# tbuckworth/train-procgen-pytorch

Hardware: AMD Instinct MI355X
Metric: env steps/sec (whole node), coinrun hard-500 IMPALA-CNN PPO (higher is better)
Workload: dtype bf16

## Files before the change

### scratch/ro_timeline4.py

```python
import csv, glob, sys, collections
f = glob.glob(sys.argv[1] + "/**/*kernel_trace.csv", recursive=True)[0]
rows = list(csv.DictReader(open(f)))
key = "Stream_Id" if "Stream_Id" in rows[0] else "Queue_Id"
by = collections.defaultdict(list)
for r in rows:
    by[r[key]].append(r)
streams = [(k, v) for k, v in by.items() if sum(1 for r in v if "heads_sample" in r["Kernel_Name"]) > 200]
print("streams with a rollout chain:", [(k, len(v)) for k, v in streams], "key", key)
k, v = streams[0]
v.sort(key=lambda r: int(r["Start_Timestamp"]))
idx = [i for i, r in enumerate(v) if "heads_sample" in r["Kernel_Name"]]
a, b = idx[-150], idx[-149]
base = int(v[a]["End_Timestamp"])
for r in v[a + 1:b + 1]:
    s, e = int(r["Start_Timestamp"]), int(r["End_Timestamp"])
    print(f"{(s - base) / 1e3:8.1f} us +{(e - s) / 1e3:7.1f}  {r['Kernel_Name'][:70]}")
dur, gap, cnt = collections.Counter(), collections.Counter(), collections.Counter()
for i in range(idx[-201] + 1, idx[-1] + 1):
    r, p = v[i], v[i - 1]
    n = r["Kernel_Name"][:40]
    dur[n] += (int(r["End_Timestamp"]) - int(r["Start_Timestamp"])) / 1e3
    gap[n] += (int(r["Start_Timestamp"]) - int(p["End_Timestamp"])) / 1e3
    cnt[n] += 1
print("kernel                                     n    avg_us   avg_gap_before_us")
for n in cnt:
    print(f"{n:40s} {cnt[n]:5d} {dur[n] / cnt[n]:8.1f} {gap[n] / cnt[n]:8.1f}")
print("step period us", (int(v[idx[-1]]["End_Timestamp"]) - int(v[idx[-201]]["End_Timestamp"])) / 200 / 1e3)
```

### train-procgen-pytorch_amd/csrc/common.h

```cpp
#pragma once
#include <hip/hip_runtime.h>
#include <stdint.h>
#include <stddef.h>

typedef float f32x4 __attribute__((ext_vector_type(4)));

struct ConvArgs {
    const void*    in;
    const int32_t* idx;
    long long      in_base;
    const float*   w;
    const float*   bias;
    const void*    res;
    const void*    mask;
    void*          out;
    const float*   lut;
    int            n;
    int            relu_in;
    int            bf16;
    const unsigned short* wbank;
    const unsigned short* lut16;
    const uint8_t* pool_arg;
    const void*    wg_in;
    float*         wg_partial;
};

struct WgradArgs {
    const void*    in;
    const int32_t* idx;
    long long      in_base;
    const void*    dout;
    float*         partial;
    const float*   lut;
    int            n;
    int            relu_in;
    int            bf16;
    const unsigned short* lut16;
    const uint8_t* pool_arg;
};

enum ConvShape {
    CS_3_16_64 = 0,
    CS_16_16_32,
    CS_16_32_32,
    CS_32_32_16,
    CS_32_32_8,
    CS_COUNT
};

void conv_shape_dims(ConvShape s, int* cin, int* cout, int* hw);
void launch_conv_fwd(ConvShape s, const ConvArgs& a, hipStream_t st);
void launch_conv_dgrad(ConvShape s, const ConvArgs& a, hipStream_t st);
int  wgrad_grid(ConvShape s, int n);
int  wgrad_grid_for(ConvShape s, int n, int bf16);
void launch_conv_wgrad(ConvShape s, const WgradArgs& a, hipStream_t st);

struct BankDesc { long long w_off, out_off; int rows, cin_pass, co_f, ci_f, transw, ws, nk; };
int  bank_ws(int cin_pass);
void launch_pack_banks(const float* params, unsigned short* banks, const BankDesc* d_desc, int n_desc, hipStream_t st);
int  wgrad_grid_bf16(ConvShape s, int n);
void launch_conv_wgrad_bf16(ConvShape s, const WgradArgs& a, hipStream_t st);
int  conv1_bank_elems();
void launch_repack_all(const float* params, unsigned short* banks, const BankDesc* d_desc, int n_desc, const float* c1_w, unsigned short* c1_bank ,
                       const float* fc_w, unsigned short* fc_wp, unsigned short* fc_wt, int H , hipStream_t st);
void launch_conv1_pool_fwd_bf16(const ConvArgs& a, const unsigned short* lut16, void* p_out, uint8_t* p_arg, hipStream_t st);
void launch_conv1_fwd_bf16(const ConvArgs& a, const unsigned short* lut16, hipStream_t st);
void launch_conv1_wgrad_bf16(const WgradArgs& a, const unsigned short* lut16, hipStream_t st);
void launch_conv_fwd_bf16(ConvShape s, const ConvArgs& a, hipStream_t st);
void launch_conv_dgrad_bf16(ConvShape s, const ConvArgs& a, hipStream_t st);
int  conv_bwd_fused_grid(ConvShape s, int n);

bool launch_conv_pool_fwd_bf16(ConvShape s, const ConvArgs& a, void* p_out, uint8_t* p_arg, hipStream_t st);

void launch_resblock_bf16(ConvShape s, const void* x, const float* b1, const float* b2, void* a_out, void* y_out, int n,
                          const unsigned short* bank1, const unsigned short* bank2, hipStream_t st);
void launch_resblock_bwd_bf16(ConvShape s, const void* dy, const void* a_fwd, const void* x_fwd, void* da_out, void* dx_out, int n,
                              const unsigned short* bank2_t, const unsigned short* bank1_t, hipStream_t st);
int  resblock_bwd_full_grid(int n);
void launch_resblock_bwd_full_bf16(const void* dy, const void* a_fwd, const void* x_fwd, void* dx_out, void* da_out, int n,
                                   const unsigned short* bank2_t, const unsigned short* bank1_t, float* slab2, float* slab1, hipStream_t st, hipEvent_t done_ev = nullptr );
int  resblock_bwd_full32_grid(ConvShape s, int n);
void launch_resblock_bwd_full32_bf16(ConvShape s, const void* dy, const void* a_fwd, const void* x_fwd, void* dx_out, void* da_out, int n,
                                     const unsigned short* bank2_t, const unsigned short* bank1_t, float* slab2, float* slab1, hipStream_t st);
void launch_resblock_pair_bf16(ConvShape s, const void* x, const float* const* b, void* a1_out, void* y1_out, void* a2_out, void* y2_out, int n,
                               const unsigned short* const* bank, hipStream_t st);

void launch_rollout_tail_bf16(const void* x, void* y, int n, const unsigned short* const* bank, const float* const* bias, hipStream_t st);

template <template <int> class F, typename... Args>
static inline bool fc_dispatch_width(int D, Args... args) {
    switch (D) {
    case 64: F<64>::run(args...); return true;
    case 128: F<128>::run(args...); return true;
    case 192: F<192>::run(args...); return true;
    case 256: F<256>::run(args...); return true;
    case 320: F<320>::run(args...); return true;
    case 384: F<384>::run(args...); return true;
    case 448: F<448>::run(args...); return true;
    case 512: F<512>::run(args...); return true;
    default: return false;
    }
}
void launch_fc_pack(const float* w, unsigned short* wp, unsigned short* wt, int N, int K, hipStream_t st);
void launch_fc_tn(const float* A, const unsigned short* B, float* gW, float* ws, size_t ws_floats, int M, int N, int K, hipStream_t st);
void launch_fc_fwd_bf16(const void* x_bf16, const unsigned short* wp, const float* bias, float* y, int n, int D, hipStream_t st);
void launch_fc_dgrad_bf16(const float* dy, const unsigned short* wt, const void* mask_bf16, void* dx_bf16, int n, int D, hipStream_t st);
void launch_fc_fwd_small_bf16(const void* X, const unsigned short* Wp, const float* bias, float* feat, int n, int D, hipStream_t st);

struct GemmArgs {
    const float* A; const float* B; float* C;
    int M, N, K;
    long long sam, sak, sbk, sbn, ldc;
    const float* bias;
    const float* mask;
    int relu_a, relu_b;
    int relu_out;
    int accumulate;
    int a_bf16, b_bf16, mask_bf16, c_bf16;
    float* ws; size_t ws_floats;
};
void launch_gemm(const GemmArgs& g, hipStream_t st);

void launch_maxpool_fwd(const float* in, float* out, uint8_t* arg, int n, int hw, int c, hipStream_t st);
void launch_maxpool_bwd(const float* dout, const uint8_t* arg, float* din, int n, int hw, int c, hipStream_t st);
void launch_maxpool_fwd_bf16(const void* in, void* out, uint8_t* arg, int n, int hw, int c, hipStream_t st);
void launch_maxpool_bwd_bf16(const void* dout, const uint8_t* arg, void* din, int n, int hw, int c, hipStream_t st);

struct SlabDesc { long long src_off, w_off, b_off; int nslab, slab_len, n_w; };
void launch_reduce_all_slabs(const float* ws, float* grads, const SlabDesc* d_desc, int n_desc, int max_slab_len, hipStream_t st);
void launch_reduce_slabs(const float* partial, int nslab, int slab_len, float* dst_w, int n_w, float* dst_b, int n_b,
                         hipStream_t st);
void launch_colsum_acc(const float* dY, int M, int N, int ld, float* db, float* col_ws , hipStream_t st);

void launch_heads_fwd(const float* feat, const float* Wh, const float* bh, float* hout, int n, int O , hipStream_t st);
void launch_heads_bwd(const float* dY, const float* feat, const float* Wh, int relu_mask, float* dfeat, float* gW, float* gb, float* ws ,
                      int n, int H, int O, hipStream_t st, bool with_reduce = true, hipEvent_t done_ev = nullptr);
void launch_heads_bwd_reduce(const float* ws, float* gW, float* gb, int n, int H, int O, hipStream_t st);
void launch_logp_all(const float* hout, int n, int A, float* lp_out, float* value_out, hipStream_t st, int value_from_logits = 0);
void launch_philox_debug(const uint32_t* in6, int n, uint32_t* out4, float* u_out, hipStream_t st);
void launch_heads_sample(const float* feat, const float* Wh, const float* bh, int n, int H, int A, const float* u,
                         unsigned long long seed, unsigned long long ctr, int32_t* act, float* logp, float* value, float* pack,
                         float* hout, const float* rd, float* rew_dst, float* done_dst, hipStream_t st,
                         unsigned* done_ctr = nullptr, unsigned* host_flag = nullptr, unsigned ticket = 0, int value_from_logits = 0);
void launch_sample(const float* hout, int n, int A, const float* u, unsigned long long seed, unsigned long long ctr,
                   int32_t* act, float* logp, float* value, hipStream_t st, int value_from_logits = 0);

struct LossHP { float eps_clip, value_coef, entropy_coef, x_entropy_coef, entropy_mult, fs_coef; };
struct LossArgs {
    const float* hout;
    const int32_t* idx;
    const int32_t* act; const float* old_logp; const float* old_value; const float* ret; const float* adv;
    float* dY;
    float* partial;
    float* stats;
    int n, A;
    float inv_n_global;
    LossHP hp;
    int value_from_logits;
};
constexpr int MI_MAX_SEG = 16;
constexpr int FS_PARTS = 8;
struct SegTab { int n_seg; int start[MI_MAX_SEG + 1]; };
int  loss_blocks(int n);
int  loss_blocks_seg(const SegTab& st);
void launch_loss_fwd_seg(const LossArgs& a, const SegTab& st, bool with_bwd, hipStream_t stream);
void launch_loss_fwd(const LossArgs& a, hipStream_t st);
void launch_loss_finalize_records(const LossArgs& a, int n_rec, float* stats_base, const float* fs_base, float* log_base, hipStream_t stream);
void launch_loss_finalize_seg(const LossArgs& a, const SegTab& st, int phase, float* stats_base, const double* fs_parts, int fs_d, float* fs_out,
                              float* log_base, hipStream_t stream);
void launch_loss_finalize(const LossArgs& a, int nblk, int phase, const float* fs_ptr, float* log_slot, hipStream_t st);
void launch_loss_bwd(const LossArgs& a, hipStream_t st);
int  fs_groups_per_segment(int n_seg);
void launch_fs_metric_seg(const void* flat_pre, int bf16, const SegTab& st, int d, float* colmax_scratch, double* fs_parts, hipStream_t stream);
int  fs_metric_groups();
void launch_fs_metric(const void* flat_pre, int bf16, int n, int d, float* colmax_scratch, float* fs_out, hipStream_t st);
void launch_fs_keys(const void* x, int bf16, int n, int d, const float* part, int G, const int32_t* gpos, float* colmax, int* arg,
                    long long* keys, long long* keys_local, hipStream_t st);
void launch_fs_apply_keys(void* Gd, int bf16, int d, const long long* keys, const long long* keys_local, const int* arg, float fs_coef, hipStream_t st);
void launch_fs_from_keys(const long long* keys, int d, float* fs_out, hipStream_t st);
void launch_fs_grad(const void* x, int bf16, int n, int d, const float* part, int G, void* Gd, float fs_coef, float* colmax, int* arg, hipStream_t st);

constexpr int IPL_SUMS = 8;
struct IplArgs {
    const float* hout;
    const int32_t* idx;
    const int32_t* act; const float* rew; const float* done;
    float* nv;
    float* dY;
    float* g_next;
    float *pred, *rew_out;
    double* partial;
    int n, A;
    float inv_n_global, gamma, alpha, entropy_coef;
    int entropy_modified, reward_incentive, adv_incentive, zero_obs_seed;
};
int  ipl_blocks(int n);
int  ipl_partial_cols(int A);
void launch_ipl_next_value(const IplArgs& a, const float* v_src, int v_stride, int v_off, hipStream_t st);
void launch_ipl_loss(const IplArgs& a, float* rec8, hipStream_t st);
void launch_ipl_next_seed(const float* g_next, float* dY, int n, int A, hipStream_t st);
void launch_ipl_shift_idx(const int32_t* idx, int32_t* idx2, int n, int shift, hipStream_t st);
void launch_ipl_greedy(const float* hout, int n, int A, int32_t* act, float* logp, float* value, hipStream_t st);

void launch_gae(const float* rew, const float* done, const float* value, float* adv, float* ret, int T, int E,
                float gamma, float lmbda, int use_gae, hipStream_t st);
void launch_advnorm_merge(const double* all, int R, double* stats3, hipStream_t st);
void launch_advnorm_stats(const float* adv, int n, double* stats3, hipStream_t st);
void launch_advnorm_apply(float* adv, int n, const double* stats3, hipStream_t st);

void launch_adam(float* p, float* g, float* m, float* v, long long n, const double* sumsq , int npart, float max_norm, float lr,
                 float beta1, float beta2, float eps, float step_size_scale, float bc2_sqrt, float* gnorm_out,
                 hipStream_t st);
void launch_sumsq_partials(const float* g, long long n, double* part , hipStream_t st);

void launch_mask_rows(const float* h, const float* done, float* out, int n, int H, hipStream_t st);
void launch_gru_value_bwd(const float* gi, const float* gh, const float* hm, const float* wv , float* dgates, int n, int H, hipStream_t st,
                          int row_seed = 0);
void launch_gru_gates(const float* gi, const float* gh, const float* hm, float* h_out, float* feat_out, int n, int H, hipStream_t st);
void launch_gru_step(const float* x, const float* h_in, const float* done, const float* w_ih, const float* w_hh, const float* b_ih,
                     const float* b_hh, float* h_out, float* h_copy, int n, int H, hipStream_t st);

void launch_gru_seq_mask(const float* done, const int32_t* idx, float* mask, int N, hipStream_t st);
bool gru_seq_width_ok(int H);
void launch_gru_seq_fwd(const float* gi, const float* h0, const float* mask, const float* w_hh, const float* b_hh, float* out_h, float* sv, int T, int n, int H,
                        hipStream_t st);
void launch_gru_seq_bwd(const float* dout, const float* out_h, const float* h0, const float* mask, const float* sv, const float* w_hh, float* dgi, float* dgh,
                        float* hm_out, int T, int n, int H, hipStream_t st);

void launch_value_seed(float* dY, int n, int A, hipStream_t st);
void launch_lse_value_seed(const float* hout, float* dY, int n, int A, hipStream_t st);
void launch_lse_hidden_seed(const float* hout, const float* Wh, float* seed, int n, int H, int A, hipStream_t st);
void launch_conv1_input_grad(const void* dC, int bf16, const float* W, float* dX, int n, hipStream_t st);

void mi_launch_fail(const char* msg);
const char* mi_launch_failed_take();
void launch_pull_bytes(const void* host_src , void* dst, size_t bytes , hipStream_t st);
void launch_pull_i32(const int32_t* host_src , int32_t* dst, int n, hipStream_t st);
void launch_gather_rows(const float* src, const int32_t* idx, long long base, float* dst, int n, int d, hipStream_t st);
void launch_fill(float* p, long long n, float v, hipStream_t st);
```

### train-procgen-pytorch_amd/csrc/conv_bf16.hip

```cpp
#include "common.h"
#include "device_util.h"
#include <mutex>
#include <type_traits>

static int c1_grid(int n);


template <int CH, int HO, int NPR>
struct PoolStage {
    static constexpr int NW = NPR * HO * (CH / 8), K = (NW + 255) / 256;
    static constexpr int PD_ELEMS = NPR * HO * CH;
    static constexpr size_t BYTES = (size_t)PD_ELEMS * 3;
    uint4 rd[K]; uint2 ra[K];
    __device__ __forceinline__ void load(const unsigned short* g_dp, const uint8_t* g_arg, long long img, int oyb) {
#pragma unroll
        for (int k = 0; k < K; ++k) {
            const int e = threadIdx.x + k * 256;
            rd[k] = (uint4){0u, 0u, 0u, 0u}; ra[k] = (uint2){0xffffffffu, 0xffffffffu};
            if (e < NW) {
                const int c8 = e % (CH / 8), ox = (e / (CH / 8)) % HO, oy = oyb + e / ((CH / 8) * HO);
                if (oy >= 0 && oy < HO) {
                    const long long o = ((img * HO + oy) * HO + ox) * CH + c8 * 8;
                    rd[k] = *(const uint4*)(g_dp + o); ra[k] = *(const uint2*)(g_arg + o);
                }
// ... 953 lines not shown
            for (int r = 0; r < 4; ++r) redb[wave * C::COUT + cb * 16 + kq * 4 + r] = accb[cb][r];
    }
    __syncthreads();
    float* slab = a.partial + (long long)blockIdx.x * C::SLAB;
    for (int e = tid; e < C::WLEN; e += 256) slab[e] = red[e];
    if (tid < C::COUT) slab[C::WLEN + tid] = (redb[tid] + redb[C::COUT + tid]) + (redb[2 * C::COUT + tid] + redb[3 * C::COUT + tid]);
}

using WT_16_16_32 = WbCfg<16, 16, 32,  8, 32, 1>;
using WT_16_32_32 = WbCfg<16, 32, 32,  8, 32, 1>;
using WT_32_32_16 = WbCfg<32, 32, 16, WG16_TH, 16, 1>;
using WT_32_32_8  = WbCfg<32, 32,  8,  8,  8, WG8_NIMG>;

template <class C>
static int wb_grid(int n) {
    int bpc = (int)((160 * 1024) / C::LDS_BYTES);
    bpc = bpc < 1 ? 1 : (bpc > 4 ? 4 : bpc);
    const int w = (C::NIMG > 1) ? (n + C::NIMG - 1) / C::NIMG : n * C::TPI;
    return w > 256 * bpc ? 256 * bpc : w;
}
template <class C, bool POOLED = false>
static void launch_wb_t(const WgradArgs& a, hipStream_t st) {
    static std::once_flag attr;
    constexpr size_t TILE = C::TILE_BYTES + (POOLED ? PoolStage<C::COUT, C::HW / 2, C::TH / 2 + 1>::BYTES : 0);
    constexpr size_t LDS = TILE > C::RED_BYTES ? TILE : C::RED_BYTES;
    std::call_once(attr, [] { hipFuncSetAttribute((const void*)conv3x3_wgrad_bf16_kernel<C, POOLED>, hipFuncAttributeMaxDynamicSharedMemorySize, (int)LDS); });
    const int grid = wb_grid<C>(a.n);
    if (grid < 1) return;
    hipLaunchKernelGGL((conv3x3_wgrad_bf16_kernel<C, POOLED>), dim3(grid), dim3(256), LDS, st, a);
}
int wgrad_grid_bf16(ConvShape s, int n) {
    switch (s) {
        case CS_16_16_32: return wb_grid<WT_16_16_32>(n);
        case CS_16_32_32: return wb_grid<WT_16_32_32>(n);
        case CS_32_32_16: return wb_grid<WT_32_32_16>(n);
        case CS_32_32_8:  return wb_grid<WT_32_32_8>(n);
        case CS_3_16_64:  return c1_grid(n);
        default: return -1;
    }
}
void launch_conv_wgrad_bf16(ConvShape s, const WgradArgs& a, hipStream_t st) {
    switch (s) {
        case CS_16_16_32: launch_wb_t<WT_16_16_32>(a, st); break;
        case CS_16_32_32: if (a.pool_arg) launch_wb_t<WT_16_32_32, true>(a, st); else launch_wb_t<WT_16_32_32>(a, st); break;
        case CS_32_32_16: if (a.pool_arg) launch_wb_t<WT_32_32_16, true>(a, st); else launch_wb_t<WT_32_32_16>(a, st); break;
        case CS_32_32_8:  launch_wb_t<WT_32_32_8>(a, st); break;
        default: break;
    }
}

template <int TH_>
struct C1T {
    static constexpr int HW = 64, TH = TH_, TW = 64, PH = TH + 2, PW = 66, NPIX = PH * PW, NT = TH * TW;
    static constexpr int NTASK = PH * 16, NLD = 3;
    static constexpr int TPI = HW / TH;
    static_assert(NTASK <= 256, "one staging task per thread");
};
using C1 = C1T<8>;
using C1W = C1T<4>;
__device__ __forceinline__ long long c1_frame(const int32_t* idx, long long in_base, int img) { return idx ? (long long)idx[img] : in_base + img; }
typedef const __attribute__((address_space(4))) int32_t* c1_const_i32p;
__device__ __forceinline__ int c1_frame_fetch(const int32_t* idx, const void* any_valid, int img) {
    const int32_t* p = idx ? idx + img : (const int32_t*)any_valid;
    return *(c1_const_i32p)p;
}
__device__ __forceinline__ long long c1_frame_of(const int32_t* idx, long long in_base, int fetched, int img) {
    return idx ? (long long)fetched : in_base + img;
}
template <class C1>
__device__ __forceinline__ void c1_load(uint32_t (&r)[C1::NLD], const uint8_t* frames, long long frame, int ty0) {
    const int e = threadIdx.x, row = (e >> 4) < C1::PH ? (e >> 4) : C1::PH - 1, g = e & 15, gy = ty0 + row - 1;
    const int gyc = gy < 0 ? 0 : (gy > C1::HW - 1 ? C1::HW - 1 : gy);
    const uint32_t* p = (const uint32_t*)(frames + frame * (C1::HW * C1::HW * 3) + gyc * (C1::HW * 3) + g * 12);
    r[0] = p[0]; r[1] = p[1]; r[2] = p[2];
}
template <class C1, bool ONE4 = false>
__device__ __forceinline__ void c1_store(const uint32_t (&r)[C1::NLD], unsigned short* s_in, int ty0) {
    const int e = threadIdx.x, row = e >> 4, g = e & 15, gy = ty0 + row - 1;
    if (e < C1::NTASK) {
        const bool in = gy >= 0 && gy < C1::HW;
        const uint32_t px[3] = {in ? r[0] : 0u, in ? r[1] : 0u, in ? r[2] : 0u};
        mi_f32x2 f[6];
#pragma unroll
        for (int b = 0; b < 6; ++b)
            f[b] = (mi_f32x2){(float)((px[(2 * b) >> 2] >> (8 * ((2 * b) & 3))) & 0xffu), (float)((px[(2 * b + 1) >> 2] >> (8 * ((2 * b + 1) & 3))) & 0xffu)}
                   * (mi_f32x2){1.0f / 255.0f, 1.0f / 255.0f};
        auto fv = [&](int b) { return (b & 1) ? f[b >> 1].y : f[b >> 1].x; };
#pragma unroll
        for (int j = 0; j < 4; ++j)
            *(uint2*)(s_in + (row * C1::PW + 1 + g * 4 + j) * 4) =
                (uint2){mi_pk_bf16(fv(3 * j), fv(3 * j + 1)), mi_pk_bf16(fv(3 * j + 2), ONE4 ? 1.f : 0.f)};
    }
}

constexpr int C1_WS = 80;
__global__ __launch_bounds__(256) void conv1_fwd_bf16_kernel(ConvArgs a, const unsigned short* lut16) {
    __shared__ __attribute__((aligned(16))) unsigned short s_in[C1::NPIX * 4];
    __shared__ __attribute__((aligned(16))) unsigned short s_w[16 * C1_WS];
    const int tid = threadIdx.x, lane = tid & 63, wave = tid >> 6, i = lane & 15, kq = lane >> 4;
    unsigned short* g_out = (unsigned short*)a.out;
    for (int e = tid; e < 16 * C1_WS; e += 256) {
        const int j = e / C1_WS, k = e % C1_WS, tap = k / 4, ci = k % 4;
        s_w[e] = f2bf((k < 36 && ci < 3) ? a.w[(j * 9 + tap) * 3 + ci] : 0.f);
    }
    for (int e = tid; e < C1::NPIX * 4; e += 256) s_in[e] = 0;
    const float bias = a.bias ? a.bias[i] : 0.f;
    int off0, off1;
    { const int t0 = 2 * kq, t1 = 2 * kq + 1; off0 = ((t0 / 3) * C1::PW + t0 % 3) * 4; off1 = ((t1 / 3) * C1::PW + t1 % 3) * 4; }
    constexpr int off8 = (2 * C1::PW + 2) * 4;
    const int nwork = a.n * C1::TPI;
    uint32_t regs[C1::NLD];
    auto item = [&](int w) { return w < nwork ? w : nwork - 1; };
    int frame_next = 0;
    if ((int)blockIdx.x < nwork) {
        c1_load<C1>(regs, (const uint8_t*)a.in, c1_frame(a.idx, a.in_base, blockIdx.x / C1::TPI), (blockIdx.x % C1::TPI) * C1::TH);
        frame_next = c1_frame_fetch(a.idx, a.in, item(blockIdx.x + gridDim.x) / C1::TPI);
    }
    for (int work = blockIdx.x; work < nwork; work += gridDim.x) {
        const int img = work / C1::TPI, ty0 = (work % C1::TPI) * C1::TH;
        __syncthreads();
        c1_store<C1>(regs, s_in, ty0);
        __syncthreads();
        { const int w2 = item(work + gridDim.x); c1_load<C1>(regs, (const uint8_t*)a.in, c1_frame_of(a.idx, a.in_base, frame_next, w2 / C1::TPI), (w2 % C1::TPI) * C1::TH);
          frame_next = c1_frame_fetch(a.idx, a.in, item(work + 2 * gridDim.x) / C1::TPI); }
        const bf16x8 bw1 = *(const bf16x8*)(s_w + i * C1_WS + kq * 8);
        const bf16x8 bw2 = *(const bf16x8*)(s_w + i * C1_WS + 32 + kq * 8);
#pragma unroll
        for (int mt = 0; mt < 8; ++mt) {
            const int pl = (wave * 8 + mt) * 16 + i, y = pl / C1::TW, x = pl % C1::TW;
            const unsigned short* p = s_in + (y * C1::PW + x) * 4;
            const uint2 lo = *(const uint2*)(p + off0), hi = *(const uint2*)(p + off1), t8 = *(const uint2*)(p + off8);
            const bf16x8 a1 = __builtin_bit_cast(bf16x8, (uint4){lo.x, lo.y, hi.x, hi.y});
            const bf16x8 a2 = __builtin_bit_cast(bf16x8, (uint4){t8.x, t8.y, 0u, 0u});
            f32x4 acc = {bias, bias, bias, bias};
            acc = MFMA_BF16(a1, bw1, acc);
            acc = MFMA_BF16(a2, bw2, acc);
#pragma unroll
            for (int r = 0; r < 4; ++r) {
                const int po = (wave * 8 + mt) * 16 + kq * 4 + r;
                g_out[(((long long)img * C1::HW + ty0 + po / C1::TW) * C1::HW + po % C1::TW) * 16 + i] = f2bf(acc[r]);
            }
        }
    }
}

using C1P = C1T<9>;
#ifndef C1P_SC
#define C1P_SC 24
#endif
int conv1_bank_elems() { return 16 * C1_WS; }
template <int D>
__global__ void repack_all_kernel(const float* __restrict__ params, unsigned short* __restrict__ banks, const BankDesc* __restrict__ desc, int n_desc,
                                  const float* __restrict__ c1_w, unsigned short* __restrict__ c1_bank,
                                  const float* __restrict__ fc_w, unsigned short* __restrict__ fc_wp, unsigned short* __restrict__ fc_wt) {
    constexpr int C1B = (16 * C1_WS + 255) / 256;
    int b = blockIdx.x;
    if (b < 8 * n_desc) {
        const BankDesc d = desc[b >> 3];
        const float* w = params + d.w_off;
        unsigned short* out = banks + d.out_off;
        for (int e = (b & 7) * 256 + threadIdx.x; e < d.rows * d.ws; e += 8 * 256) {
            const int j = e / d.ws, k = e % d.ws, tap = k / d.cin_pass, ci = k % d.cin_pass;
            float v = 0.f;
            if (k < d.nk * 32 && tap < 9) v = d.transw ? w[(ci * 9 + (8 - tap)) * d.ci_f + j] : w[(j * 9 + tap) * d.ci_f + ci];
            out[e] = f2bf(v);
        }
        return;
    }
    b -= 8 * n_desc;
    if (b < C1B) {
        const int e = b * 256 + threadIdx.x;
        if (c1_bank && e < 16 * C1_WS) {
            const int j = e / C1_WS, k = e % C1_WS, tap = k / 4, ci = k % 4;
            c1_bank[e] = f2bf((k < 36 && ci < 3) ? c1_w[(j * 9 + tap) * 3 + ci] : 0.f);
        }
        return;
    }
    b -= C1B;
    const int e = b * 256 + threadIdx.x;
    if (e < D * 2048) {
        const unsigned short h = f2bf(fc_w[e]);
        fc_wp[e] = h;
        fc_wt[(long long)(e % 2048) * D + e / 2048] = h;
    }
}
template <int D> struct RepackAll {
    static void run(const float* params, unsigned short* banks, const BankDesc* d_desc, int n_desc, const float* c1_w, unsigned short* c1_bank,
                    const float* fc_w, unsigned short* fc_wp, unsigned short* fc_wt, hipStream_t st) {
        const int blocks = 8 * n_desc + (16 * C1_WS + 255) / 256 + D * 2048 / 256;
        hipLaunchKernelGGL(repack_all_kernel<D>, dim3(blocks), dim3(256), 0, st, params, banks, d_desc, n_desc, c1_w, c1_bank, fc_w, fc_wp, fc_wt);
    }
};
void launch_repack_all(const float* params, unsigned short* banks, const BankDesc* d_desc, int n_desc, const float* c1_w, unsigned short* c1_bank,
                       const float* fc_w, unsigned short* fc_wp, unsigned short* fc_wt, int H, hipStream_t st) {
    if (!fc_dispatch_width<RepackAll>(H, params, banks, d_desc, n_desc, c1_w, c1_bank, fc_w, fc_wp, fc_wt, st))
        mi_launch_fail("repack_all: no fc image kernel for this output_dim");
}
__global__ __launch_bounds__(256, 4) void conv1_pool_fwd_bf16_kernel(ConvArgs a, const unsigned short* lut16, unsigned short* p_out, uint8_t* p_arg) {
    __shared__ __attribute__((aligned(16))) unsigned short s_in[C1P::NPIX * 4];
    __shared__ __attribute__((aligned(16))) unsigned short s_w[16 * C1_WS];
    __shared__ __attribute__((aligned(16))) unsigned short s_c[9 * 65 * C1P_SC];
    const int tid = threadIdx.x, lane = tid & 63, wave = tid >> 6, i = lane & 15, kq = lane >> 4;
#ifdef WG_TIMING
    long long tacc_[8] = {0, 0, 0, 0, 0, 0, 0, 0}, tlast_ = clock64();
#endif
    if (a.wbank) {
        if (tid < 16 * C1_WS / 8) ((uint4*)s_w)[tid] = ((const uint4*)a.wbank)[tid];
    } else {
        for (int e = tid; e < 16 * C1_WS; e += 256) {
            const int j = e / C1_WS, k = e % C1_WS, tap = k / 4, ci = k % 4;
            s_w[e] = f2bf((k < 36 && ci < 3) ? a.w[(j * 9 + tap) * 3 + ci] : 0.f);
        }
    }
    static_assert((C1P::NPIX * 4) % 8 == 0, "16-byte zero fill");
    for (int e = tid; e < C1P::NPIX * 4 / 8; e += 256) ((uint4*)s_in)[e] = (uint4){0u, 0u, 0u, 0u};
    if (tid < 9 * 8) ((unsigned*)s_c)[(tid >> 3) * 65 * (C1P_SC / 2) + (tid & 7)] = MI_KEY_MIN2;
    f32x4 bias4;
#pragma unroll
    for (int r = 0; r < 4; ++r) bias4[r] = a.bias ? a.bias[kq * 4 + r] : 0.f;
    int off0, off1;
    { const int t0 = 2 * kq, t1 = 2 * kq + 1; off0 = ((t0 / 3) * C1P::PW + t0 % 3) * 4; off1 = ((t1 / 3) * C1P::PW + t1 % 3) * 4; }
    constexpr int off8 = (2 * C1P::PW + 2) * 4;
    const int nwork = a.n * 8;
    uint32_t regs0[C1P::NLD], regs1[C1P::NLD];
    auto item = [&](int w) { return w < nwork ? w : nwork - 1; };
    const int G = gridDim.x;
    int frame_next = 0;
    if ((int)blockIdx.x < nwork) {
        const int w0 = blockIdx.x, w1 = item(w0 + G);
        c1_load<C1P>(regs0, (const uint8_t*)a.in, c1_frame(a.idx, a.in_base, w0 / 8), (w0 % 8) * 8 - 1);
        c1_load<C1P>(regs1, (const uint8_t*)a.in, c1_frame(a.idx, a.in_base, w1 / 8), (w1 % 8) * 8 - 1);
        frame_next = c1_frame_fetch(a.idx, a.in, item(w0 + 2 * G) / 8);
        asm volatile("s_waitcnt vmcnt(0)" ::: "memory");
    }
    auto step = [&](int work_, uint32_t (&regs)[C1P::NLD]) {
        const int work = __builtin_amdgcn_readfirstlane(work_);
        const int img = work / 8, oy0 = (work % 8) * 4, cy0 = 2 * oy0 - 1;
        TCK(0);
        __syncthreads();
        TCK(1);
        c1_store<C1P>(regs, s_in, cy0);
        TCK(2);
        __syncthreads();
        TCK(3);
        { const int w2 = item(work + 2 * G); c1_load<C1P>(regs, (const uint8_t*)a.in, c1_frame_of(a.idx, a.in_base, frame_next, w2 / 8), (w2 % 8) * 8 - 1);
          frame_next = c1_frame_fetch(a.idx, a.in, item(work + 3 * G) / 8); }
        TCK(4);
        const bf16x8 bw1 = *(const bf16x8*)(s_w + i * C1_WS + kq * 8);
        const bf16x8 bw2 = *(const bf16x8*)(s_w + i * C1_WS + 32 + kq * 8);
#ifndef C1P_GROUP
#define C1P_GROUP 3
#endif
#pragma unroll
        for (int g0 = 0; g0 < 9; g0 += C1P_GROUP) {
            f32x4 acc[C1P_GROUP];
#pragma unroll
            for (int m = 0; m < C1P_GROUP; ++m) {
                const int mt = g0 + m;
                const int pl = (wave * 9 + mt) * 16 + i, y = pl / 64, x = pl % 64;
                const unsigned short* p = s_in + (y * C1P::PW + x) * 4;
                const uint2 lo = *(const uint2*)(p + off0), hi = *(const uint2*)(p + off1), t8 = *(const uint2*)(p + off8);
                acc[m] = MFMA_BF16(bw1, __builtin_bit_cast(bf16x8, (uint4){lo.x, lo.y, hi.x, hi.y}), bias4);
                acc[m] = MFMA_BF16(bw2, __builtin_bit_cast(bf16x8, (uint4){t8.x, t8.y, 0u, 0u}), acc[m]);
            }
#pragma unroll
            for (int m = 0; m < C1P_GROUP; ++m) {
                const int t = wave * 9 + g0 + m;
                const unsigned k0 = mi_bf16x2_to_keys(mi_pk_bf16(acc[m][0], acc[m][1]));
                const unsigned k1 = mi_bf16x2_to_keys(mi_pk_bf16(acc[m][2], acc[m][3]));
                *(uint2*)(s_c + (t * 16 + i + (t >> 2) + 1) * C1P_SC + kq * 4) = (uint2){k0, k1};
            }
        }
        if (cy0 < 0 && wave == 0) {
            unsigned* q = (unsigned*)(s_c + (lane + 1) * C1P_SC);
#pragma unroll
            for (int w = 0; w < 8; ++w) q[w] = MI_KEY_MIN2;
        }
        TCK(5);
        __syncthreads();
        TCK(6);
        {
            const int c8 = tid & 1, ox = (tid >> 1) & 31, oyl = tid >> 6;
            uint4 u[9];
#pragma unroll
            for (int ky = 0; ky < 3; ++ky)
#pragma unroll
                for (int kx = 0; kx < 3; ++kx)
                    u[ky * 3 + kx] = *(const uint4*)(s_c + ((2 * oyl + ky) * 65 + 2 * ox + kx) * C1P_SC + c8 * 8);
            const size_t o = ((((size_t)img * 32 + oy0 + oyl) * 32 + ox) * 2 + c8) * 8;
            uint4 pk;
            uint2 ar;
            mi_pool9_keys(u, pk, ar);
            *(uint4*)(p_out + o) = pk;
            *(uint2*)(p_arg + o) = ar;
        }
        TCK(7);
    };
    int work = blockIdx.x;
    for (; work + G < nwork; work += 2 * G) { step(work, regs0); step(work + G, regs1); }
    if (work < nwork) step(work, regs0);
#ifdef WG_TIMING
    if (tid == 0) for (int k = 0; k < 8; ++k) atomicAdd(&g_wg_timing[k], (unsigned long long)tacc_[k]);
#endif
}
void launch_conv1_pool_fwd_bf16(const ConvArgs& a, const unsigned short* lut16, void* p_out, uint8_t* p_arg, hipStream_t st) {
    const int w = a.n * 8, grid = w > 1024 ? 1024 : w;
    if (grid < 1) return;
    hipLaunchKernelGGL(conv1_pool_fwd_bf16_kernel, dim3(grid), dim3(256), 0, st, a, lut16, (unsigned short*)p_out, p_arg);
}

__global__ __launch_bounds__(256) void conv1_wgrad_bf16_kernel(WgradArgs a, const unsigned short* lut16) {
    extern __shared__ __attribute__((aligned(16))) unsigned short smem_h[];
    unsigned short* s_in = smem_h;
    unsigned short* s_do = smem_h + ((C1W::NPIX * 4 + 7) / 8) * 8;
    const int tid = threadIdx.x, lane = tid & 63, wave = tid >> 6, i = lane & 15, kq = lane >> 4, rq = (lane & 15) >> 2, cp = lane & 3;
    const unsigned short* g_do = (const unsigned short*)a.dout;
#ifdef WG_TIMING
    long long tacc_[8] = {0, 0, 0, 0, 0, 0, 0, 0}, tlast_ = clock64();
#endif
    f32x4 acc[3] = {{0.f, 0.f, 0.f, 0.f}, {0.f, 0.f, 0.f, 0.f}, {0.f, 0.f, 0.f, 0.f}};
    for (int e = tid; e < C1W::NPIX * 4; e += 256) s_in[e] = 0;
    const int nwork = a.n * C1W::TPI;
    constexpr int NDO = C1W::NT * 2 / 256;
    struct Stage { uint32_t regs[C1W::NLD]; uint4 rdo[NDO]; };
    Stage S0, S1;
    auto load_do = [&](Stage& S, int img, int ty0) {
#pragma unroll
        for (int k = 0; k < NDO; ++k) {
            const int e = tid + k * 256, pl = e >> 1, c8 = e & 1;
            S.rdo[k] = *(const uint4*)(g_do + (((long long)img * C1W::HW + ty0 + pl / C1W::TW) * C1W::HW + pl % C1W::TW) * 16 + c8 * 8);
        }
    };
    auto item = [&](int w) { return w < nwork ? w : nwork - 1; };
    const int G = gridDim.x;
    int frame_next = 0;
    {
        const int w0 = blockIdx.x, w1 = item(w0 + G);
        c1_load<C1W>(S0.regs, (const uint8_t*)a.in, c1_frame(a.idx, a.in_base, w0 / C1W::TPI), (w0 % C1W::TPI) * C1W::TH); load_do(S0, w0 / C1W::TPI, (w0 % C1W::TPI) * C1W::TH);
        c1_load<C1W>(S1.regs, (const uint8_t*)a.in, c1_frame(a.idx, a.in_base, w1 / C1W::TPI), (w1 % C1W::TPI) * C1W::TH); load_do(S1, w1 / C1W::TPI, (w1 % C1W::TPI) * C1W::TH);
        frame_next = c1_frame_fetch(a.idx, a.in, item(w0 + 2 * G) / C1W::TPI);
        asm volatile("s_waitcnt vmcnt(0)" ::: "memory");
    }
    auto step = [&](int work, Stage& S) {
        TCK(0);
        __syncthreads();
        TCK(1);
        c1_store<C1W, true>(S.regs, s_in, (work % C1W::TPI) * C1W::TH);
#pragma unroll
// ... 312 lines not shown
```

### train-procgen-pytorch_amd/csrc/engine.hip

```cpp
#include "engine_ctx.h"
#include "lanes.h"

thread_local std::string g_err;
thread_local hipStream_t tl_stream = nullptr;
thread_local float* tl_ws = nullptr;
thread_local size_t tl_ws_floats = 0;
const char* mi_last_error(void) { return g_err.c_str(); }

static std::atomic<int64_t> g_live[3];
static int hip_dev_alloc(void** p, size_t bytes, bool zero) {
    hipError_t e = hipMalloc(p, bytes);
    if (e != hipSuccess) return e;
    if (zero && ((e = hipMemset(*p, 0, bytes)) != hipSuccess || (e = hipDeviceSynchronize()) != hipSuccess)) { hipFree(*p); return e; }
    ++g_live[0];
    return 0;
}
static void hip_dev_free(void* p) { hipFree(p); --g_live[0]; }
static int hip_pinned_alloc(void** p, size_t bytes, unsigned flags) { const hipError_t e = hipHostMalloc(p, bytes, flags); g_live[1] += e == hipSuccess; return e; }
static void hip_pinned_free(void* p) { hipHostFree(p); --g_live[1]; }
static int hip_event_create(void** ev, unsigned flags) { const hipError_t e = hipEventCreateWithFlags((hipEvent_t*)ev, flags); g_live[2] += e == hipSuccess; return e; }
static void hip_event_destroy(void* ev) { hipEventDestroy((hipEvent_t)ev); --g_live[2]; }
const DevPool::Backend* hip_pool() {
    static const DevPool::Backend be = {hip_dev_alloc, hip_dev_free, hip_pinned_alloc, hip_pinned_free, hip_event_create, hip_event_destroy};
    return &be;
// ... 128 lines not shown
        for (int o = 0; o < t.co; ++o)
            for (int ch = 0; ch < 32; ++ch)
                for (int p = 0; p < 64; ++p) dev[(int64_t)o * 2048 + p * 32 + ch] = ref[(int64_t)o * 2048 + ch * 64 + p];
    } else memcpy(dev, ref, t.n * sizeof(float));
}
void to_ref_layout(const TensorDesc& t, const float* dev, float* ref) {
    if (t.kind == K_CONVW) {
        for (int co = 0; co < t.co; ++co)
            for (int ci = 0; ci < t.ci; ++ci)
                for (int tap = 0; tap < 9; ++tap) ref[((int64_t)co * t.ci + ci) * 9 + tap] = dev[((int64_t)co * 9 + tap) * t.ci + ci];
    } else if (t.kind == K_FCW) {
        for (int o = 0; o < t.co; ++o)
            for (int ch = 0; ch < 32; ++ch)
                for (int p = 0; p < 64; ++p) ref[(int64_t)o * 2048 + ch * 64 + p] = dev[(int64_t)o * 2048 + p * 32 + ch];
    } else memcpy(ref, dev, t.n * sizeof(float));
}

static int upload_flat(mi_ctx* c, float* dbuf, const float* flat, int64_t n) {
    ARG(n == c->n_params, "flat vector length != mi_param_count"); JOIN(c);
    std::vector<float> tmp(n);
    for (auto& t : c->tensors) to_device_layout(t, flat + t.ref_off, tmp.data() + t.dev_off);
    HIPC(hipMemcpyAsync(dbuf, tmp.data(), n * sizeof(float), hipMemcpyHostToDevice, c->stream));
    HIPC(hipStreamSynchronize(c->stream));
    return 0;
}
static int download_flat(mi_ctx* c, const float* dbuf, float* flat, int64_t n) {
    ARG(n == c->n_params, "flat vector length != mi_param_count"); JOIN(c);
    std::vector<float> tmp(n);
    HIPC(hipMemcpyAsync(tmp.data(), dbuf, n * sizeof(float), hipMemcpyDeviceToHost, c->stream));
    HIPC(hipStreamSynchronize(c->stream));
    for (auto& t : c->tensors) to_ref_layout(t, tmp.data() + t.dev_off, flat + t.ref_off);
    return 0;
}

static int ctx_build(mi_ctx* c);
static void ctx_release(mi_ctx* c);
int mi_create(const mi_config* cfg, mi_ctx** out) {
    ARG(cfg && out, "null cfg/out");
    ARG(cfg->arch == MI_ARCH_IMPALA || cfg->arch == MI_ARCH_MLP, "arch");
    ARG(cfg->n_actions >= 1 && cfg->n_actions <= 16, "n_actions must be in [1,16]");
    ARG(cfg->n_steps >= 1 && cfg->n_envs >= 1 && cfg->max_batch >= 1, "n_steps/n_envs/max_batch");
    ARG(cfg->precision == 0 || cfg->precision == 1, "precision must be 0 (fp32) or 1 (bf16 activations)");
    ARG(cfg->value_from_logits == 0 || cfg->value_from_logits == 1, "value_from_logits must be 0 (fc_value head) or 1 (logsumexp of the logits)");
    if (cfg->arch == MI_ARCH_MLP) ARG(cfg->obs_dim >= 1 && cfg->mlp_depth >= 2 && cfg->mlp_width >= 1 && cfg->out_dim >= 1, "mlp dims");
    if (cfg->arch == MI_ARCH_IMPALA)
        ARG(cfg->out_dim == 0 || (cfg->out_dim >= 64 && cfg->out_dim <= 512 && cfg->out_dim % 64 == 0),
            "impala out_dim (output_dim) must be a multiple of 64 in [64, 512]");
    int ndev = 0;
    if (hipGetDeviceCount(&ndev) != hipSuccess || ndev == 0) return fail(-3, "no HIP device: the MI355X library has no CPU fallback");
    ARG(cfg->device >= 0 && cfg->device < ndev && cfg->device < MAX_LANE_DEVICES, "device");
    HIPC(hipSetDevice(cfg->device));
    mi_ctx* c = new mi_ctx();
    c->cfg = *cfg;
    if (int r = ctx_build(c)) { const std::string why = g_err; ctx_release(c); return fail(r, why); }
    *out = c;
    return 0;
}
static int ctx_build(mi_ctx* c) {
    const mi_config* cfg = &c->cfg;
    DevPool& m = c->pool;
    c->T = cfg->n_steps; c->E = cfg->n_envs; c->A = cfg->n_actions;
    c->H = (cfg->arch == MI_ARCH_IMPALA && cfg->out_dim == 0) ? 256 : cfg->out_dim;
    c->NB = cfg->max_batch < cfg->n_envs ? cfg->n_envs : cfg->max_batch;
    c->bf = (cfg->arch == MI_ARCH_IMPALA) && cfg->precision == 1;
    c->lse = cfg->value_from_logits;
    c->es = c->bf ? 2.0 : 4.0;
    if (cfg->stream) c->stream = (hipStream_t)cfg->stream;
    else { HIPC(hipStreamCreateWithFlags(&c->stream, hipStreamNonBlocking)); c->own_stream = true; }
    c->main_stream = c->stream;
    HIPC(m.event(&c->ev_side_fork, hipEventDisableTiming)); HIPC(m.event(&c->ev_side_join, hipEventDisableTiming));
    if (cfg->arch == MI_ARCH_IMPALA) build_impala_layout(c); else build_mlp_layout(c);
    if (cfg->arch == MI_ARCH_IMPALA && !impala_regions_ok(c)) return fail(-1, "internal: parameter layout does not split at embedder.fc.weight");

    const int64_t P = c->n_params, T = c->T, E = c->E, NB = c->NB;
    HIPC(m.dev(&c->params, P)); HIPC(m.dev(&c->grads, P)); HIPC(m.dev(&c->adam_m, P)); HIPC(m.dev(&c->adam_v, P));
    HIPC(m.dev(&c->rew, T * E)); HIPC(m.dev(&c->done, T * E)); HIPC(m.dev(&c->logp, T * E));
    HIPC(m.dev(&c->adv, T * E)); HIPC(m.dev(&c->ret, T * E)); HIPC(m.dev(&c->value, (T + 1) * E));
    HIPC(m.dev(&c->act, T * E)); HIPC(m.dev(&c->adv_stats, 4));
    if (cfg->arch == MI_ARCH_IMPALA) {
        c->obs_bytes_per_env = 64 * 64 * 3;
        HIPC(m.dev(&c->frames, (size_t)(T + 1) * E * c->obs_bytes_per_env));
        HIPC(m.dev(&c->stage_frames, (size_t)NB * c->obs_bytes_per_env));
        const int chan[4] = {3, 16, 32, 32};
        int hin = 64;
        for (int b = 0; b < 3; ++b) {
            Block& k = c->blk[b];
            k.cin = chan[b]; k.cout = chan[b + 1]; k.hin = hin;
            const size_t X = (size_t)NB * hin * hin * k.cout, p = X / 4;
            if (!c->bf) HIPC(m.dev(&k.C, X));
            HIPC(m.dev(&k.PI, p));
            HIPC(m.dev(&k.P0, p)); HIPC(m.dev(&k.A1, p)); HIPC(m.dev(&k.P1, p)); HIPC(m.dev(&k.A2, p)); HIPC(m.dev(&k.P2, p));
            hin /= 2;
        }
        if (!c->bf) HIPC(m.dev(&c->GC, (size_t)NB * 64 * 64 * 16));
        for (int k = 0; k < 3; ++k) HIPC(m.dev(&c->GP[k], (size_t)NB * 32 * 32 * 16));
        for (size_t l = 0; l < c->convs.size() && l < 15; ++l) {
            c->slab_off[l] = (long long)c->slab_floats;
            c->slab_floats += (size_t)1024 * (size_t)(c->convs[l].cout * 9 * c->convs[l].cin + c->convs[l].cout);
        }
        HIPC(m.dev(&c->slabs, c->slab_floats));
        HIPC(m.dev_raw(&c->d_slab_desc, sizeof(SlabDesc) * 15));
        HIPC(m.dev(&c->fs_scratch, (size_t)MI_MAX_SEG * 128 * 2048));
        HIPC(m.dev(&c->fs_colmax, (size_t)2048)); HIPC(m.dev(&c->fs_arg, (size_t)2048));
        HIPC(m.dev(&c->fs_keys, (size_t)2048)); HIPC(m.dev(&c->fs_keys_local, (size_t)2048)); HIPC(m.dev(&c->d_gpos, (size_t)NB));
        HIPC(m.pinned(&c->h_gpos, (size_t)NB * 4, hipHostMallocDefault));
    } else {
        c->obs_bytes_per_env = (size_t)cfg->obs_dim * sizeof(float);
        HIPC(m.dev(&c->obsf, (size_t)(T + 1) * E * cfg->obs_dim));
        HIPC(m.dev(&c->stage_obs, (size_t)NB * cfg->obs_dim));
        c->mlp_act.resize(c->mlp.size() + 1);
        HIPC(m.dev(&c->mlp_act[0], (size_t)NB * cfg->obs_dim));
        for (size_t l = 0; l < c->mlp.size(); ++l) HIPC(m.dev(&c->mlp_act[l + 1], (size_t)NB * c->mlp[l].out));
        const int wmax = cfg->mlp_width > c->H ? cfg->mlp_width : c->H;
        for (int k = 0; k < 2; ++k) HIPC(m.dev(&c->GP[k], (size_t)NB * wmax));
    }
    HIPC(m.dev(&c->feat, (size_t)NB * c->H)); HIPC(m.dev(&c->dfeat, (size_t)NB * c->H));
    HIPC(m.dev(&c->hout, (size_t)NB * (c->A + 1))); HIPC(m.dev(&c->dY, (size_t)NB * (c->A + 1)));
    if (c->lse) HIPC(m.dev(&c->d_val, (size_t)NB));
    HIPC(m.dev(&c->d_lp, (size_t)NB * c->A));
    const size_t gws = (size_t)8 << 20;
    HIPC(m.dev(&c->gemm_ws, gws)); c->gemm_ws_floats = gws;
    HIPC(m.dev(&c->col_ws, (size_t)64 * 4096));
    HIPC(m.dev(&c->fs_val, 4));
    {
        float h[256];
        for (int k = 0; k < 256; ++k) h[k] = (float)((double)k / 255.0);
        HIPC(m.dev(&c->lut, 256));
        HIPC(hipMemcpy(c->lut, h, sizeof(h), hipMemcpyHostToDevice));
        std::vector<uint16_t> b = host_to_bf16(h, 256);
        HIPC(m.dev(&c->lut16, 256));
        HIPC(hipMemcpy(c->lut16, b.data(), 512, hipMemcpyHostToDevice));
    }
    HIPC(m.dev(&c->d_idx, (size_t)NB));
    HIPC(m.dev(&c->loss_partial, (size_t)(loss_blocks(NB) + 1 + MI_MAX_SEG) * 32));
    HIPC(m.dev(&c->loss_stats, 64));
    HIPC(m.dev(&c->loss_log, (size_t)c->log_cap * 8));
    HIPC(m.dev(&c->stats_ring, (size_t)c->log_cap * 32)); HIPC(m.dev(&c->fs_ring, (size_t)c->log_cap)); HIPC(m.dev(&c->fs_parts, (size_t)MI_MAX_SEG * 8));
    HIPC(m.dev(&c->sumsq, 2 + 128)); HIPC(m.dev(&c->gnorm, 2));
    HIPC(m.dev(&c->d_u, (size_t)E));
    HIPC(m.dev(&c->d_pack, (size_t)3 * E)); HIPC(m.dev(&c->d_rd, (size_t)2 * E));
    const unsigned hflags = hipHostMallocCoherent | hipHostMallocMapped;
    HIPC(m.pinned(&c->h_pack, (size_t)3 * E * 4, hflags)); HIPC(m.pinned(&c->h_rd, (size_t)2 * E * 4, hflags));
    HIPC(m.dev(&c->d_done_ctr, (size_t)16)); HIPC(m.pinned(&c->h_flag, 64, hflags)); memset(c->h_flag, 0, 64);
    HIPC(m.dev(&c->s_act, (size_t)E)); HIPC(m.dev(&c->s_logp, (size_t)E)); HIPC(m.dev(&c->s_val, (size_t)E));
    for (int k = 0; k < mi_ctx::IDX_RING; ++k) {
        HIPC(m.pinned(&c->h_idx_ring[k], (size_t)NB * sizeof(int32_t), hflags));
        HIPC(m.event(&c->idx_ev[k], hipEventDisableTiming));
    }
    c->h_f_floats = (size_t)4 * (E > 64 ? E : 64);
    HIPC(m.pinned(&c->h_f, c->h_f_floats * sizeof(float), hipHostMallocDefault));
    HIPC(m.pinned(&c->h_i, (size_t)E * sizeof(int32_t), hipHostMallocDefault));
    if (getenv("MI355_COPY_GBPS")) c->copy_rate_bytes_per_us = atof(getenv("MI355_COPY_GBPS")) * 1000.0;
    if (c->bf) {
        HIPC(m.dev(&c->fc_wp, (size_t)c->H * 2048)); HIPC(m.dev(&c->fc_wt, (size_t)c->H * 2048));
        HIPC(m.dev(&c->c1_bank, (size_t)conv1_bank_elems()));
        std::vector<BankDesc> desc;
        long long off = 0;
        for (auto& L : c->convs) {
            if (L.cin == 3) continue;
            BankDesc f{L.w_off, off, L.cout, L.cin, L.cout, L.cin, 0, bank_ws(L.cin), L.cin == 32 ? 9 : 5};
            L.bank_f = off; off += (long long)f.rows * f.ws; desc.push_back(f);
            BankDesc d{L.w_off, off, L.cin, L.cout, L.cout, L.cin, 1, bank_ws(L.cout), L.cout == 32 ? 9 : 5};
            L.bank_d = off; off += (long long)d.rows * d.ws; desc.push_back(d);
        }
        c->n_banks = (int)desc.size();
        HIPC(m.dev(&c->banks, (size_t)off));
        HIPC(m.dev_raw(&c->d_bank_desc, desc.size() * sizeof(BankDesc)));
        HIPC(hipMemcpy(c->d_bank_desc, desc.data(), desc.size() * sizeof(BankDesc), hipMemcpyHostToDevice));
    }
    HIPC(hipDeviceSynchronize());
    return 0;
}

static void ctx_release(mi_ctx* c) {
    for (int g = 0; g < mi_ctx::MAX_GROUPS; ++g)
        if (c->gw[g]) {
            GroupWorker* w = c->gw[g];
            w->quit.store(true); { std::lock_guard<std::mutex> lk(w->mu); } w->cv.notify_one();
            w->th.join(); delete w; c->gw[g] = nullptr;
        }
    for (int g = 0; g < mi_ctx::MAX_GROUPS; ++g) if (c->gs[g]) hipStreamSynchronize(c->gs[g]);
    if (c->stream) hipStreamSynchronize(c->stream);
    prof_harvest(c);
    g_lanes[c->cfg.device].give_back(c, lane_drop);
    mi_comm_destroy(c);
    hipDeviceSynchronize();
    sae_release(c);
    c->pool.release_all();
    if (c->side_stream) hipStreamDestroy(c->side_stream);
    if (c->own_stream) hipStreamDestroy(c->stream);
    delete c;
}
int mi_destroy(mi_ctx* c) { if (c) ctx_release(c); return 0; }

void* mi_host_alloc(size_t bytes) {
    void* p = nullptr;
    if (hipHostMalloc(&p, bytes ? bytes : 1) != hipSuccess) { g_err = "hipHostMalloc failed"; return nullptr; }
    return p;
}
void mi_host_free(void* p) { if (p) hipHostFree(p); }
int mi_host_register(void* p, size_t bytes) {
    ARG(p && bytes, "null");
    if (hipHostRegister(p, bytes, hipHostRegisterDefault) != hipSuccess) { (void)hipGetLastError(); return fail(-2, "hipHostRegister refused the range"); }
    return 0;
}
int mi_host_unregister(void* p) {
    ARG(p, "null");
    if (hipHostUnregister(p) != hipSuccess) { (void)hipGetLastError(); return fail(-2, "hipHostUnregister failed"); }
    return 0;
}

int mi_sync(mi_ctx* c) { ARG(c, "ctx"); JOIN(c); HIPC(hipStreamSynchronize(c->stream)); return 0; }

int64_t mi_param_count(mi_ctx* c) { return c ? c->n_params : -1; }
int mi_set_params(mi_ctx* c, const float* flat, int64_t n) { ARG(c && flat, "null"); c->fc_packed_valid = false; return upload_flat(c, c->params, flat, n); }
int mi_get_params(mi_ctx* c, float* flat, int64_t n) { ARG(c && flat, "null"); return download_flat(c, c->params, flat, n); }
int mi_copy_params(mi_ctx* dst, mi_ctx* src) {
    ARG(dst && src && dst != src, "null / same context"); JOIN(src); JOIN(dst);
    ARG(dst->cfg.arch == src->cfg.arch && dst->n_params == src->n_params && dst->A == src->A && dst->H == src->H && dst->cfg.device == src->cfg.device,
        "contexts of different architecture / size / device");
    hipEvent_t ready = nullptr, done = nullptr;
    DevPool evs(hip_pool());
    HIPC(evs.event(&ready, hipEventDisableTiming)); HIPC(evs.event(&done, hipEventDisableTiming));
    HIPC(hipEventRecord(ready, src->stream));
    HIPC(hipStreamWaitEvent(dst->stream, ready, 0));
    HIPC(hipMemcpyAsync(dst->params, src->params, (size_t)src->n_params * 4, hipMemcpyDeviceToDevice, dst->stream));
    if (src->gru_train) {
        if (!dst->gru_on) return fail(-1, "invalid argument: the source trains its GRU but the destination has none (mi_set_gru)");
        const GruTensors from = gru_tensors(src), to = gru_tensors(dst);
        for (int k = 0; k < 4; ++k) HIPC(hipMemcpyAsync(to.t[k].p, from.t[k].p, from.t[k].len * 4, hipMemcpyDeviceToDevice, dst->stream));
    }
    HIPC(hipEventRecord(done, dst->stream));
    HIPC(hipStreamWaitEvent(src->stream, done, 0));
    dst->fc_packed_valid = false;
    return 0;
}
int mi_get_grads(mi_ctx* c, float* flat, int64_t n) { ARG(c && flat, "null"); return download_flat(c, c->grads, flat, n); }
int mi_set_adam_state(mi_ctx* c, const float* m, const float* v, int64_t n) {
    ARG(c && m && v, "null");
    int r = upload_flat(c, c->adam_m, m, n);
    return r ? r : upload_flat(c, c->adam_v, v, n);
}
int mi_get_adam_state(mi_ctx* c, float* m, float* v, int64_t n) {
    ARG(c && m && v, "null");
    int r = download_flat(c, c->adam_m, m, n);
    return r ? r : download_flat(c, c->adam_v, v, n);
}

int mi_put_obs(mi_ctx* c, int32_t t, const void* obs, size_t bytes) {
    ARG(c && obs, "null"); JOIN(c); ARG(t >= 0 && t <= c->T, "t out of range");
    const size_t want = (size_t)c->E * c->obs_bytes_per_env;
    ARG(bytes == want, "obs byte count != E * bytes_per_env");
    HIPC(hipMemcpyAsync(obs_ring(c) + (size_t)t * want, obs, bytes, hipMemcpyHostToDevice, c->stream));
    return 0;
}
int mi_get_obs(mi_ctx* c, int32_t t, void* obs, size_t bytes) {
    ARG(c && obs, "null"); JOIN(c); ARG(t >= 0 && t <= c->T, "t out of range");
    const size_t want = (size_t)c->E * c->obs_bytes_per_env;
    ARG(bytes == want, "obs byte count != E * bytes_per_env");
    HIPC(hipMemcpyAsync(obs, obs_ring(c) + (size_t)t * want, bytes, hipMemcpyDeviceToHost, c->stream));
    HIPC(hipStreamSynchronize(c->stream));
    return 0;
}
int mi_put_step(mi_ctx* c, int32_t t, const float* rew, const float* done) {
    ARG(c && rew && done, "null"); JOIN(c); ARG(t >= 0 && t < c->T, "t out of range");
    const size_t b = (size_t)c->E * sizeof(float);
    HIPC(hipMemcpyAsync(c->rew + (size_t)t * c->E, rew, b, hipMemcpyHostToDevice, c->stream));
    HIPC(hipMemcpyAsync(c->done + (size_t)t * c->E, done, b, hipMemcpyHostToDevice, c->stream));
    return 0;
}
int mi_put_policy_outputs(mi_ctx* c, int32_t t, const int32_t* act, const float* logp, const float* value) {
    ARG(c, "null"); JOIN(c); ARG(t >= 0 && t <= c->T, "t out of range");
    const size_t E = c->E;
    if (act) { ARG(t < c->T, "act at t==T"); HIPC(hipMemcpyAsync(c->act + t * E, act, E * 4, hipMemcpyHostToDevice, c->stream)); }
    if (logp) { ARG(t < c->T, "logp at t==T"); HIPC(hipMemcpyAsync(c->logp + t * E, logp, E * 4, hipMemcpyHostToDevice, c->stream)); }
    if (value) HIPC(hipMemcpyAsync(c->value + t * E, value, E * 4, hipMemcpyHostToDevice, c->stream));
    HIPC(hipStreamSynchronize(c->stream));
    return 0;
}
static float* field_ptr(mi_ctx* c, int f, int64_t* n) {
    const int64_t TE = (int64_t)c->T * c->E;
    *n = TE;
    switch (f) {
        case MI_F_REW: return c->rew; case MI_F_DONE: return c->done; case MI_F_LOGP: return c->logp;
        case MI_F_ADV: return c->adv; case MI_F_RET: return c->ret;
        case MI_F_VALUE: *n = TE + c->E; return c->value;
        default: return nullptr;
    }
}
int mi_read_field(mi_ctx* c, int32_t f, float* out, int64_t n) {
    ARG(c && out, "null"); JOIN(c);
    if (f == MI_F_ACT) {
        ARG(n == (int64_t)c->T * c->E, "length");
        std::vector<int32_t> tmp(n);
        HIPC(hipMemcpyAsync(tmp.data(), c->act, n * 4, hipMemcpyDeviceToHost, c->stream));
        HIPC(hipStreamSynchronize(c->stream));
        for (int64_t k = 0; k < n; ++k) out[k] = (float)tmp[k];
        return 0;
    }
    int64_t want; float* p = field_ptr(c, f, &want);
    ARG(p, "field"); ARG(n == want, "length");
    HIPC(hipMemcpyAsync(out, p, n * 4, hipMemcpyDeviceToHost, c->stream));
    HIPC(hipStreamSynchronize(c->stream));
    return 0;
}
int mi_write_field(mi_ctx* c, int32_t f, const float* in, int64_t n) {
    ARG(c && in, "null"); JOIN(c);
// ... 40 lines not shown
        p.a = prof_event(c); p.b = prof_event(c); p.cls = cls; p.phase = c->prof.phase; p.units = units; p.bytes = bytes; p.flops = flops;
        hipEventRecord(p.a, c->stream);
    }
    ~ProfScope() {
        if (!live) return;
        hipEventRecord(p.b, c->stream);
        c->prof.pend.push_back(p);
        if (c->prof.pend.size() >= 4096) prof_harvest(c);
    }
};
int mi_profile_enable(mi_ctx* c, int32_t enabled) {
    ARG(c, "null");
    if (!enabled) prof_harvest(c);
    c->prof.on = (enabled & 0xff) != 0; c->prof.all_phases = (enabled & 0xff) == 2;
    c->prof.period = (enabled >> 8) > 0 ? (enabled >> 8) : 1; c->prof.mb_count = 0; c->prof.sample_now = true;
    return 0;
}
const char* mi_profile_class_name(int32_t id) { return (id >= 0 && id < PC_COUNT) ? kProfNames[id] : ""; }
int mi_profile_read(mi_ctx* c, double* rows, int32_t max_rows, int32_t* n_rows, int32_t reset) {
    ARG(c && rows && n_rows, "null"); JOIN(c);
    prof_harvest(c);
    int n = 0;
    for (int ph = 0; ph < 2; ++ph)
        for (int k = 0; k < PC_COUNT; ++k)
            if (c->prof.launches[ph][k] > 0 && n < max_rows) {
                double* r = rows + (size_t)n * 7;
                r[0] = k; r[1] = ph; r[2] = (double)c->prof.launches[ph][k]; r[3] = c->prof.ms[ph][k]; r[4] = (double)c->prof.units[ph][k];
                r[5] = c->prof.bytes[ph][k]; r[6] = c->prof.flops[ph][k];
                ++n;
            }
    *n_rows = n;
    if (reset) { memset(c->prof.ms, 0, sizeof(c->prof.ms)); memset(c->prof.launches, 0, sizeof(c->prof.launches)); memset(c->prof.units, 0, sizeof(c->prof.units));
                 memset(c->prof.bytes, 0, sizeof(c->prof.bytes)); memset(c->prof.flops, 0, sizeof(c->prof.flops)); }
    return 0;
}

static void conv_fwd(mi_ctx* c, const ConvLayer& L, const void* in, const InputSrc* src, int relu_in, const float* res, float* out, int n) {
    ConvArgs a{};
    a.in = src ? src->base : in; a.idx = src ? src->idx : nullptr; a.in_base = src ? src->first : 0;
    a.w = c->params + L.w_off; a.bias = c->params + L.b_off; a.res = res; a.mask = nullptr; a.out = out;
    a.lut = c->lut; a.n = n; a.relu_in = relu_in; a.bf16 = c->bf;
    a.wbank = (c->bf && L.bank_f >= 0) ? c->banks + L.bank_f : nullptr;
    a.lut16 = c->bf ? c->lut16 : nullptr;
    const double px = (double)n * L.hw * L.hw, es = c->es;
    ProfScope ps(c, PC_CONV_FWD + (int)L.shape, n, px * ((L.cin == 3 ? 3.0 : es * L.cin) + es * L.cout * (res ? 2 : 1)), px * 18.0 * L.cin * L.cout);
    launch_conv_fwd(L.shape, a, CUR(c));
}
static void conv_dgrad(mi_ctx* c, const ConvLayer& L, const float* dout, const float* mask, const float* res, float* din, int n, const uint8_t* pool_arg = nullptr) {
    ConvArgs a{};
    a.pool_arg = pool_arg;
    a.in = dout; a.w = c->params + L.w_off; a.bias = nullptr; a.res = res; a.mask = mask; a.out = din;
    a.lut = c->lut; a.n = n; a.relu_in = 0; a.bf16 = c->bf;
    a.wbank = (c->bf && L.bank_d >= 0) ? c->banks + L.bank_d : nullptr;
    const double px = (double)n * L.hw * L.hw;
    const double pool_b = pool_arg ? c->es * (px / 4 * L.cout + 2.0 * px * L.cout) : 0.0;
    ProfScope ps(c, PC_CONV_DGRAD + (int)L.shape, n, px * c->es * (L.cout + L.cin * (1 + (mask ? 1 : 0) + (res ? 1 : 0))) + pool_b, px * 18.0 * L.cin * L.cout);
    launch_conv_dgrad(L.shape, a, CUR(c));
}
static inline void push_slab(mi_ctx* c, int layer, int grid) {
    const ConvLayer& L = c->convs[layer];
    const int wlen = L.cout * 9 * L.cin;
    c->h_slab_desc[c->slab_desc_n++] = SlabDesc{c->slab_off[layer], (long long)L.w_off, (long long)L.b_off, grid, wlen + L.cout, wlen};
}
static void conv_wgrad(mi_ctx* c, const ConvLayer& L, const void* in, const InputSrc* src, int relu_in, const float* dout, int n, const uint8_t* pool_arg = nullptr) {
    WgradArgs a{};
    a.pool_arg = pool_arg;
    a.in = src ? src->base : in; a.idx = src ? src->idx : nullptr; a.in_base = src ? src->first : 0;
    const int layer = (int)(&L - c->convs.data());
    a.dout = dout; a.partial = c->slabs + c->slab_off[layer]; a.lut = c->lut; a.n = n; a.relu_in = relu_in; a.bf16 = c->bf;
    a.lut16 = c->bf ? c->lut16 : nullptr;
    const int grid = wgrad_grid_for(L.shape, n, c->bf);
    if (grid < 1) return;
    if (grid > 1024) { net_err_set(c, "weight-gradient launch needs more than the 1024 slabs a layer owns"); return; }
    const double px = (double)n * L.hw * L.hw;
    {
      const double pool_b = (pool_arg && L.cin == 3) ? c->es * (px / 4 * L.cout + 2.0 * px * L.cout) : 0.0;
      ProfScope ps(c, PC_CONV_WGRAD + (int)L.shape, n, px * ((L.cin == 3 ? 3.0 : c->es * L.cin) + c->es * L.cout) + pool_b, px * 18.0 * L.cin * L.cout);
      launch_conv_wgrad(L.shape, a, CUR(c)); }
    push_slab(c, layer, grid);
}
static void issue_grad_allreduce(mi_ctx* c, int64_t off, int64_t n, bool last) {
    if (!c->ar_armed || !c->comm || n <= 0) return;
    hipEventRecord(c->ev_ar_ready, CUR(c));
    hipStreamWaitEvent(c->comm_stream, c->ev_ar_ready, 0);
    ncclResult_t r = ncclAllReduce(c->grads + off, c->grads + off, (size_t)n, ncclFloat, ncclSum, c->comm_grad, c->comm_stream);
    if (r != ncclSuccess) { net_err_set(c, std::string("ncclAllReduce (gradients): ") + ncclGetErrorString(r)); return; }
    if (last) { hipEventRecord(c->ev_ar_done, c->comm_stream); c->ar_armed = false; c->ar_issued = true; c->ar_inflight = true; }
}

static void conv_wgrad_reduce_all(mi_ctx* c, int n, int first = 0) {
    if (c->slab_desc_n <= 0) return;
    int max_len = 0; double bytes = 0;
    for (int k = first; k < c->slab_desc_n; ++k) { max_len = std::max(max_len, c->h_slab_desc[k].slab_len); bytes += 4.0 * c->h_slab_desc[k].nslab * c->h_slab_desc[k].slab_len; }
    if (c->slab_desc_cached_n != n) {
        hipMemcpyAsync(c->d_slab_desc, c->h_slab_desc, sizeof(SlabDesc) * c->slab_desc_n, hipMemcpyHostToDevice, CUR(c));
        c->slab_desc_cached_n = n;
    }
    { ProfScope ps(c, PC_SLAB_REDUCE, n, bytes, 0.0);
      launch_reduce_all_slabs(c->slabs, c->grads, c->d_slab_desc + first, c->slab_desc_n - first, max_len, CUR(c)); }
    c->slab_desc_n = 0;
}

void linear_fwd(mi_ctx* c, const float* X, int relu_x, const float* W, const float* b, float* Y, int n, int in, int out, int relu_out, int x_bf16) {
    GemmArgs g{};
    const GemmWs ws = gemm_ws(c); g.ws = ws.p; g.ws_floats = ws.floats;
    g.a_bf16 = x_bf16;
    g.A = X; g.B = W; g.C = Y; g.M = n; g.N = out; g.K = in;
    g.sam = in; g.sak = 1; g.sbk = 1; g.sbn = in; g.ldc = out;
    g.bias = b; g.relu_a = relu_x; g.relu_out = relu_out;
    ProfScope ps(c, PC_GEMM, n, 4.0 * ((double)n * in + (double)in * out + (double)n * out), 2.0 * n * in * out);
    launch_gemm(g, CUR(c));
}
void linear_dgrad(mi_ctx* c, const float* dY, const float* W, const float* mask, float* dX, int n, int in, int out, int x_bf16) {
    GemmArgs g{};
    const GemmWs ws = gemm_ws(c); g.ws = ws.p; g.ws_floats = ws.floats;
    g.mask_bf16 = x_bf16; g.c_bf16 = x_bf16;
    g.A = dY; g.B = W; g.C = dX; g.M = n; g.N = in; g.K = out;
    g.sam = out; g.sak = 1; g.sbk = in; g.sbn = 1; g.ldc = in; g.mask = mask;
    ProfScope ps(c, PC_GEMM, n, 4.0 * ((double)n * out + (double)in * out + (double)n * in * (mask ? 2 : 1)), 2.0 * n * in * out);
    launch_gemm(g, CUR(c));
}
void linear_wgrad(mi_ctx* c, const float* dY, const float* X, int relu_x, float* gW, float* gb, int n, int in, int out, int x_bf16) {
    GemmArgs g{};
    const GemmWs ws = gemm_ws(c); g.ws = ws.p; g.ws_floats = ws.floats;
    g.b_bf16 = x_bf16;
    g.A = dY; g.B = X; g.C = gW; g.M = out; g.N = in; g.K = n;
    g.sam = 1; g.sak = out; g.sbk = in; g.sbn = 1; g.ldc = in; g.relu_b = relu_x; g.accumulate = 1;
    ProfScope ps(c, PC_GEMM, n, 4.0 * ((double)n * out + (double)n * in + (double)in * out), 2.0 * n * in * out);
    launch_gemm(g, CUR(c));
    launch_colsum_acc(dY, n, out, out, gb, c->col_ws, CUR(c));
}

static void net_heads(mi_ctx* c, int n, int soff = 0) {
    if (c->H == 256 && c->A + 1 <= 16 && n >= 1024) {
        ProfScope ps(c, PC_GEMM, n, 4.0 * ((double)n * c->H + (double)n * (c->A + 1) + (double)c->H * (c->A + 1)), 2.0 * n * c->H * (c->A + 1));
        launch_heads_fwd(c->feat + (size_t)soff * c->H, c->params + c->wh_off, c->params + c->bh_off, c->hout + (size_t)soff * (c->A + 1), n, c->A + 1, CUR(c));
        return;
    }
    linear_fwd(c, c->feat + (size_t)soff * c->H, 0, c->params + c->wh_off, c->params + c->bh_off, c->hout + (size_t)soff * (c->A + 1), n, c->H, c->A + 1, 0);
}
static void net_gru(mi_ctx* c, int n, int soff = 0) {
    const int H = c->H;
    const size_t o = (size_t)soff * H;
    launch_mask_rows(c->h_state + o, c->d_done + soff, c->h_masked + o, n, H, CUR(c));
    linear_fwd(c, c->feat + o, 0, c->gru_wih, c->gru_bih, c->gru_gi + 3 * o, n, H, 3 * H, 0);
    linear_fwd(c, c->h_masked + o, 0, c->gru_whh, c->gru_bhh, c->gru_gh + 3 * o, n, H, 3 * H, 0);
    if (c->sal_keep_x) hipMemcpyAsync(c->gru_x + o, c->feat + o, (size_t)n * H * 4, hipMemcpyDeviceToDevice, CUR(c));
    launch_gru_gates(c->gru_gi + 3 * o, c->gru_gh + 3 * o, c->h_masked + o, c->h_state + o, c->feat + o, n, H, CUR(c));
}

static void fc_refresh(mi_ctx* c) {
    if (c->bf && !c->fc_packed_valid) {
        launch_repack_all(c->params, c->banks, c->d_bank_desc, c->n_banks, c->convs.empty() ? nullptr : c->params + c->convs[0].w_off,
                          c->convs.empty() ? nullptr : c->c1_bank, c->params + c->fc.w_off, c->fc_wp, c->fc_wt, c->H, CUR(c));
        c->fc_packed_valid = true;
    }
}

static Block block_view(const mi_ctx* c, int b, int soff) {
    Block k = c->blk[b];
    if (soff) {
        const size_t pe = (size_t)(k.hin / 2) * (k.hin / 2) * k.cout, po = (size_t)soff * pe * (size_t)c->es;
        auto sh = [&](float* q, size_t bytes) { return q ? (float*)((char*)q + bytes) : q; };
        k.C = sh(k.C, po * 4); k.P0 = sh(k.P0, po); k.A1 = sh(k.A1, po); k.P1 = sh(k.P1, po); k.A2 = sh(k.A2, po); k.P2 = sh(k.P2, po);
        k.PI += (size_t)soff * pe;
    }
    return k;
}

static void forward_mlp(mi_ctx* c, const InputSrc& src, int n, int soff, float* feat) {
    float* x0 = c->mlp_act[0] + (size_t)soff * c->cfg.obs_dim;
    launch_gather_rows((const float*)src.base, src.idx, src.first, x0, n, c->cfg.obs_dim, CUR(c));
    const size_t L = c->mlp.size();
    const float* x = x0;
    for (size_t l = 0; l < L; ++l) {
        float* y = (l + 1 == L) ? feat : c->mlp_act[l + 1] + (size_t)soff * c->mlp[l].out;
        linear_fwd(c, x, 0, c->params + c->mlp[l].w_off, c->params + c->mlp[l].b_off, y, n, c->mlp[l].in, c->mlp[l].out, l + 1 < L);
        x = y;
    }
}

static void forward_impala_fp32(mi_ctx* c, const InputSrc& src, int n, int soff, float* feat) {
    const float* prev = nullptr;
    for (int b = 0; b < 3; ++b) {
        const Block k = block_view(c, b, soff);
        const ConvLayer* L = &c->convs[b * 5];
        if (b == 0) conv_fwd(c, L[0], nullptr, &src, 0, nullptr, k.C, n);
        else conv_fwd(c, L[0], prev, nullptr, 0, nullptr, k.C, n);
        { ProfScope ps(c, PC_POOL_FWD, n, (double)n * k.hin * k.hin * k.cout * (c->es * 1.25 + 0.25), 0.0);
          launch_maxpool_fwd(k.C, k.P0, k.PI, n, k.hin, k.cout, CUR(c)); }
        conv_fwd(c, L[1], k.P0, nullptr, 1, nullptr, k.A1, n);
        conv_fwd(c, L[2], k.A1, nullptr, 1, k.P0, k.P1, n);
        conv_fwd(c, L[3], k.P1, nullptr, 1, nullptr, k.A2, n);
        conv_fwd(c, L[4], k.A2, nullptr, 1, k.P1, k.P2, n);
        prev = k.P2;
    }
    linear_fwd(c, prev, 1, c->params + c->fc.w_off, c->params + c->fc.b_off, feat, n, 2048, c->H, 1, 0);
}

static bool forward_impala_bf16(mi_ctx* c, const InputSrc& src, int n, int soff, float* feat, bool train) {
    const bool fused_tail = !train && n <= 256 && c->rollout_tail;
    const float* prev = nullptr;
    for (int b = 0; b < 3; ++b) {
        const Block k = block_view(c, b, soff);
        const ConvLayer* L = &c->convs[b * 5];
        if (fused_tail && b == 1) {
            const unsigned short* bk[10]; const float* bb[10];
            for (int q = 0; q < 10; ++q) { bk[q] = c->banks + c->convs[5 + q].bank_f; bb[q] = c->params + c->convs[5 + q].b_off; }
            const Block k3 = block_view(c, 2, soff);
            { const double px2 = (double)n * 32 * 32, px3 = (double)n * 16 * 16;
              ProfScope ps(c, PC_RESBLOCK + (int)CS_32_32_16, n, 2.0 * (px2 * 16 + px3 / 4 * 32), px2 * 18.0 * 16 * 32 + 5.0 * px3 * 18.0 * 32 * 32 + 4.0 * (px3 / 4) * 18.0 * 32 * 32);
              launch_rollout_tail_bf16(prev, k3.P2, n, bk, bb, CUR(c)); }
            prev = k3.P2;
            break;
        }
        if (b == 0) {
            ConvArgs a{};
            a.in = src.base; a.idx = src.idx; a.in_base = src.first; a.w = c->params + L[0].w_off; a.bias = c->params + L[0].b_off;
            a.n = n; a.bf16 = 1; a.lut16 = c->lut16; a.wbank = c->c1_bank;
            const double px = (double)n * 64 * 64;
            ProfScope ps(c, PC_CONV_FWD + (int)L[0].shape, n, px * 3.0 + 2.0 * (2.0 * px * 16 + px / 4 * 16), px * 18.0 * 3 * 16);
            launch_conv1_pool_fwd_bf16(a, c->lut16, k.P0, k.PI, CUR(c));
        } else {
            ConvArgs a{};
            a.in = prev; a.bias = c->params + L[0].b_off; a.n = n; a.bf16 = 1; a.wbank = c->banks + L[0].bank_f;
            const double px = (double)n * L[0].hw * L[0].hw;
            ProfScope ps(c, PC_CONV_FWD + (int)L[0].shape, n, 2.0 * (px * L[0].cin + 2.0 * px * L[0].cout + px / 4 * L[0].cout), px * 18.0 * L[0].cin * L[0].cout);
            if (!launch_conv_pool_fwd_bf16(L[0].shape, a, k.P0, k.PI, CUR(c))) { net_err_set(c, "no fused conv+pool kernel for this conv shape"); return false; }
        }
        {
            const double px = (double)n * L[1].hw * L[1].hw, ch = L[1].cout;
            const float* bb[4] = {c->params + L[1].b_off, c->params + L[2].b_off, c->params + L[3].b_off, c->params + L[4].b_off};
            const unsigned short* bk[4] = {c->banks + L[1].bank_f, c->banks + L[2].bank_f, c->banks + L[3].bank_f, c->banks + L[4].bank_f};
            ProfScope ps(c, PC_RESBLOCK + (int)L[1].shape, n, px * ch * 2.0 * 10, 4.0 * px * 18.0 * ch * ch);
            launch_resblock_pair_bf16(L[1].shape, k.P0, bb, train ? k.A1 : nullptr, train ? k.P1 : nullptr, train ? k.A2 : nullptr, k.P2, n, bk, CUR(c));
        }
        prev = k.P2;
    }
    {
        const double H = c->H;
        ProfScope ps(c, PC_GEMM, n, 2.0 * n * 2048 + 2.0 * 2048 * H + 4.0 * n * H, 2.0 * n * 2048 * H);
        if (n >= 1024) launch_fc_fwd_bf16(prev, c->fc_wp, c->params + c->fc.b_off, feat, n, c->H, CUR(c));
        else launch_fc_fwd_small_bf16(prev, c->fc_wp, c->params + c->fc.b_off, feat, n, c->H, CUR(c));
    }
    return true;
}

void net_forward(mi_ctx* c, const InputSrc& src, int n, const FwdOpts& o) {
    fc_refresh(c);
    float* const feat = c->feat + (size_t)o.soff * c->H;
    if (c->cfg.arch != MI_ARCH_IMPALA) forward_mlp(c, src, n, o.soff, feat);
    else if (!c->bf) forward_impala_fp32(c, src, n, o.soff, feat);
    else if (!forward_impala_bf16(c, src, n, o.soff, feat, o.train)) return;
    if (o.recurrent && c->gru_on) net_gru(c, n, o.soff);
    if (o.heads) net_heads(c, n, o.soff);
}

static void heads_backward(mi_ctx* c, int n, int relu_mask, bool fused, bool prof, hipStream_t st, bool with_reduce = true, hipEvent_t done_ev = nullptr) {
    if (fused) {
        ProfScope ps(c, PC_GEMM, n, 4.0 * ((double)n * (c->A + 1) + 2.0 * n * c->H + (double)c->H * (c->A + 1)), 4.0 * n * c->H * (c->A + 1), prof);
        launch_heads_bwd(c->dY, c->feat, c->params + c->wh_off, relu_mask, c->dfeat, c->grads + c->wh_off, c->grads + c->bh_off, c->gemm_ws, n, c->H, c->A + 1, st, with_reduce, done_ev);
        return;
    }
    linear_wgrad(c, c->dY, c->feat, 0, c->grads + c->wh_off, c->grads + c->bh_off, n, c->H, c->A + 1);
    linear_dgrad(c, c->dY, c->params + c->wh_off, relu_mask ? c->feat : nullptr, c->dfeat, n, c->H, c->A + 1);
}

static void backward_mlp(mi_ctx* c, int n) {
    const size_t L = c->mlp.size();
    const float* dy = c->dfeat;
    for (size_t l = L; l-- > 0;) {
        linear_wgrad(c, dy, c->mlp_act[l], 0, c->grads + c->mlp[l].w_off, c->grads + c->mlp[l].b_off, n, c->mlp[l].in, c->mlp[l].out);
        if (l == 0) { c->sal_src = dy; break; }
        float* dx = c->GP[l & 1];
        linear_dgrad(c, dy, c->params + c->mlp[l].w_off, c->mlp_act[l], dx, n, c->mlp[l].in, c->mlp[l].out);
        dy = dx;
    }
    issue_grad_allreduce(c, 0, c->n_params, true);
}

static void fs_gradient(mi_ctx* c, int n, float* G) {
    if (c->fs_grad_coef == 0.f) return;
    if (c->fs_global_apply) { if (n > 0) launch_fs_apply_keys(G, c->bf, 2048, c->fs_keys, c->fs_keys_local, c->fs_arg, c->fs_grad_coef, CUR(c)); }
    else launch_fs_grad(c->blk[2].P2, c->bf, n, 2048, c->fs_scratch, c->fs_G, G, c->fs_grad_coef, c->fs_colmax, c->fs_arg, CUR(c));
}

static void backward_impala_fp32(mi_ctx* c, const InputSrc& src, int n) {
    linear_wgrad(c, c->dfeat, c->blk[2].P2, 1, c->grads + c->fc.w_off, c->grads + c->fc.b_off, n, 2048, c->H, 0);
    issue_grad_allreduce(c, c->fc.w_off, c->n_params - c->fc.w_off, false);
    float *Gout = c->GP[0], *Ga = c->GP[1], *Gb = c->GP[2];
    linear_dgrad(c, c->dfeat, c->params + c->fc.w_off, c->blk[2].P2, Gout, n, 2048, c->H, 0);
    fs_gradient(c, n, Gout);
    for (int b = 2; b >= 0; --b) {
        Block& k = c->blk[b];
        const ConvLayer* L = &c->convs[b * 5];
        conv_wgrad(c, L[4], k.A2, nullptr, 1, Gout, n);
        conv_dgrad(c, L[4], Gout, k.A2, nullptr, Ga, n);
        conv_wgrad(c, L[3], k.P1, nullptr, 1, Ga, n);
        conv_dgrad(c, L[3], Ga, k.P1, Gout, Gb, n);
        conv_wgrad(c, L[2], k.A1, nullptr, 1, Gb, n);
        conv_dgrad(c, L[2], Gb, k.A1, nullptr, Ga, n);
        conv_wgrad(c, L[1], k.P0, nullptr, 1, Ga, n);
        conv_dgrad(c, L[1], Ga, k.P0, Gb, Gout, n);
        { ProfScope ps(c, PC_POOL_BWD, n, (double)n * k.hin * k.hin * k.cout * (c->es * 1.25 + 0.25), 0.0);
          launch_maxpool_bwd(Gout, k.PI, c->GC, n, k.hin, k.cout, CUR(c)); }
        if (b == 0) { c->sal_src = c->GC; conv_wgrad(c, L[0], nullptr, &src, 0, c->GC, n); }
        else {
            conv_wgrad(c, L[0], c->blk[b - 1].P2, nullptr, 0, c->GC, n);
            conv_dgrad(c, L[0], c->GC, nullptr, nullptr, Gout, n);
        }
    }
    conv_wgrad_reduce_all(c, n);
    issue_grad_allreduce(c, 0, c->fc.w_off, true);
}

static void fork_stats_and_fc(mi_ctx* c, int n) {
    fc_refresh(c);
    const mi_ctx::SideJob& j = c->side;
    hipStream_t ss = side_stream(c);
    hipStreamWaitEvent(ss, c->ev_side_fork, 0);
    if (c->idx_ev_deferred >= 0) { hipEventRecord(c->idx_ev[c->idx_ev_deferred], ss); c->idx_ev_deferred = -1; }
    tl_stream = ss;
    launch_heads_bwd_reduce(c->gemm_ws, c->grads + c->wh_off, c->grads + c->bh_off, n, c->H, c->A + 1, ss);
    launch_fs_metric_seg(c->blk[2].P2, c->bf, j.st, 2048, c->fs_scratch, c->fs_parts, ss);
    launch_loss_finalize_seg(j.a, j.st, j.mode, j.ring, c->fs_parts, 2048, j.fsr, j.log, ss);
    launch_fc_tn(c->dfeat, (const unsigned short*)c->blk[2].P2, c->grads + c->fc.w_off, c->gemm_ws, (size_t)8 << 20, c->H, 2048, n, ss);
    launch_colsum_acc(c->dfeat, n, c->H, c->H, c->grads + c->fc.b_off, c->col_ws, ss);
    tl_stream = nullptr;
    hipEventRecord(c->ev_side_join, ss);
    c->side.armed = false;
}
static int fork_slab_sums(mi_ctx* c, bool fork_recorded) {
    hipStream_t ss = side_stream(c);
    int max_len = 0;
    for (int q = 0; q < c->slab_desc_n; ++q) max_len = std::max(max_len, c->h_slab_desc[q].slab_len);
    if (!fork_recorded) hipEventRecord(c->ev_side_fork, c->stream);
    hipStreamWaitEvent(ss, c->ev_side_fork, 0);
    launch_reduce_all_slabs(c->slabs, c->grads, c->d_slab_desc, c->slab_desc_n, max_len, ss);
    hipEventRecord(c->ev_side_join, ss);
    return c->slab_desc_n;
}

static bool backward_residual_pair(mi_ctx* c, int b, int n, float* G, float* Ga, float* Gb, hipEvent_t done_ev) {
    const Block& k = c->blk[b];
    const ConvShape s = c->convs[b * 5 + 1].shape;
    const double px = (double)n * c->convs[b * 5 + 1].hw * c->convs[b * 5 + 1].hw, ch = c->convs[b * 5 + 1].cout;
    bool ev_taken = false;
    auto residual = [&](int i1, const float* dy, const float* a_fwd, const float* x_fwd, float* dx, hipEvent_t ev) {
        const int i2 = i1 + 1;
        const ConvLayer &l1 = c->convs[i1], &l2 = c->convs[i2];
        const unsigned short *bank2 = c->banks + l2.bank_d, *bank1 = c->banks + l1.bank_d;
        if (s == CS_16_16_32 || s == CS_32_32_16 || s == CS_32_32_8) {
            const bool c16 = s == CS_16_16_32;
            const int grid = c16 ? resblock_bwd_full_grid(n) : resblock_bwd_full32_grid(s, n);
            float *slab2 = c->slabs + c->slab_off[i2], *slab1 = c->slabs + c->slab_off[i1];
            { ProfScope ps(c, PC_RESBLOCK_BWD + (int)s, n, px * ch * 2.0 * 7, 4.0 * px * 18.0 * ch * ch);
              if (c16) launch_resblock_bwd_full_bf16(dy, a_fwd, x_fwd, dx, nullptr, n, bank2, bank1, slab2, slab1, CUR(c), ev);
              else launch_resblock_bwd_full32_bf16(s, dy, a_fwd, x_fwd, dx, nullptr, n, bank2, bank1, slab2, slab1, CUR(c)); }
            push_slab(c, i2, grid); push_slab(c, i1, grid);
            ev_taken = c16 && ev != nullptr;
        } else {
            { ProfScope ps(c, PC_RESBLOCK_BWD + (int)s, n, px * ch * 2.0 * 5, 2.0 * px * 18.0 * ch * ch);
              launch_resblock_bwd_bf16(s, dy, a_fwd, x_fwd, Ga, dx, n, bank2, bank1, CUR(c)); }
            conv_wgrad(c, l2, a_fwd, nullptr, 1, dy, n);
            conv_wgrad(c, l1, x_fwd, nullptr, 1, Ga, n);
        }
    };
    residual(b * 5 + 3, G, k.A2, k.P1, Gb, nullptr);
    residual(b * 5 + 1, Gb, k.A1, k.P0, G, done_ev);
    return ev_taken;
}
static void backward_conv_pool_bf16(mi_ctx* c, int b, int n, const float* G, float* Gin) {
    const Block& k = c->blk[b];
    const int layer = b * 5;
    const ConvLayer& L = c->convs[layer];
    const int fgrid = conv_bwd_fused_grid(L.shape, n);
    if (fgrid > 0) {
        ConvArgs a{};
        a.in = G; a.pool_arg = k.PI; a.out = Gin; a.n = n; a.bf16 = 1; a.wbank = c->banks + L.bank_d;
        a.wg_in = c->blk[b - 1].P2; a.wg_partial = c->slabs + c->slab_off[layer];
        const double px = (double)n * L.hw * L.hw;
        { ProfScope ps(c, PC_CONV_DGRAD + (int)L.shape, n, 2.0 * (px / 4 * L.cout + 3.0 * px * L.cout + 2.0 * px * L.cin), 2.0 * px * 18.0 * L.cin * L.cout);
          launch_conv_dgrad(L.shape, a, CUR(c)); }
        push_slab(c, layer, fgrid);
    } else {
        conv_wgrad(c, L, c->blk[b - 1].P2, nullptr, 0, G, n, k.PI);
        conv_dgrad(c, L, G, nullptr, nullptr, Gin, n, k.PI);
    }
}

static void backward_impala_bf16(mi_ctx* c, const InputSrc& src, int n) {
    const bool fc16 = n >= 1024;
    const bool fork1 = fc16 && c->side.armed && !tl_stream;
    const bool fork2 = c->side_on && !tl_stream && n >= 1024 && c->slab_desc_cached_n == n;
    float *Gout = c->GP[0], *Ga = c->GP[1], *Gb = c->GP[2];
    if (fork1) fork_stats_and_fc(c, n);
    else if (fc16) {
        fc_refresh(c);
        { const double H = c->H;
          ProfScope ps(c, PC_GEMM, n, 2.0 * n * 2048 + 4.0 * n * H + 4.0 * 2048 * H, 2.0 * n * 2048 * H);
          launch_fc_tn(c->dfeat, (const unsigned short*)c->blk[2].P2, c->grads + c->fc.w_off, c->gemm_ws, (size_t)8 << 20, c->H, 2048, n, CUR(c)); }
        launch_colsum_acc(c->dfeat, n, c->H, c->H, c->grads + c->fc.b_off, c->col_ws, CUR(c));
    } else
        linear_wgrad(c, c->dfeat, c->blk[2].P2, 1, c->grads + c->fc.w_off, c->grads + c->fc.b_off, n, 2048, c->H, 1);
    issue_grad_allreduce(c, c->fc.w_off, c->n_params - c->fc.w_off, false);
    if (fc16) {
        const double H = c->H;
        ProfScope ps(c, PC_GEMM, n, 4.0 * n * H + 2.0 * 2048 * H + 2.0 * 2.0 * n * 2048, 2.0 * n * 2048 * H);
        launch_fc_dgrad_bf16(c->dfeat, c->fc_wt, c->blk[2].P2, Gout, n, c->H, CUR(c));
    } else
        linear_dgrad(c, c->dfeat, c->params + c->fc.w_off, c->blk[2].P2, Gout, n, 2048, c->H, 1);
    fs_gradient(c, n, Gout);
    for (int b = 2; b >= 1; --b) {
        backward_residual_pair(c, b, n, Gout, Ga, Gb, nullptr);
        backward_conv_pool_bf16(c, b, n, Gout, Ga);
        std::swap(Gout, Ga);
    }
    const bool fork2_on_launch = backward_residual_pair(c, 0, n, Gout, Ga, Gb, fork2 ? c->ev_side_fork : nullptr);
    c->sal_src = Gout;
    int slabs_done = 0;
    if (fork2 && c->slab_desc_n >= 1) slabs_done = fork_slab_sums(c, fork2_on_launch);
    conv_wgrad(c, c->convs[0], nullptr, &src, 0, Gout, n, c->blk[0].PI);
    if (fork1 || slabs_done) hipStreamWaitEvent(c->stream, c->ev_side_join, 0);
    conv_wgrad_reduce_all(c, n, slabs_done);
    issue_grad_allreduce(c, 0, c->fc.w_off, true);
}

static void net_backward(mi_ctx* c, const InputSrc& src, int n) {
    const bool impala = c->cfg.arch == MI_ARCH_IMPALA;
    if (!c->bwd_from_dfeat) {
        const bool to_side = c->side.armed && !tl_stream;
        heads_backward(c, n, impala ? 1 : 0, c->H <= 256 && c->A + 1 <= 16 && !tl_ws, true, CUR(c), !to_side, to_side ? c->ev_side_fork : nullptr);
    }
    if (!impala) backward_mlp(c, n);
    else if (!c->bf) backward_impala_fp32(c, src, n);
    else backward_impala_bf16(c, src, n);
}

static int upload_u(mi_ctx* c, const float* u, hipStream_t st, int row0, int rows, const float** du) {
    *du = nullptr;
    if (u) { HIPC(hipMemcpyAsync(c->d_u + row0, u, (size_t)rows * 4, hipMemcpyHostToDevice, st)); *du = c->d_u + row0; }
    return 0;
}
static int read_back_staged(mi_ctx* c, const int32_t* d_act, const float* d_logp, const float* d_val, int64_t* act_out, float* logp_out, float* value_out, void* extra_out = nullptr, const void* d_extra = nullptr, size_t extra_bytes = 0) {
    const size_t E = c->E;
    if (d_act) HIPC(hipMemcpyAsync(c->h_i, d_act, E * 4, hipMemcpyDeviceToHost, c->stream));
    if (d_logp) HIPC(hipMemcpyAsync(c->h_f, d_logp, E * 4, hipMemcpyDeviceToHost, c->stream));
    if (d_val) HIPC(hipMemcpyAsync(c->h_f + E, d_val, E * 4, hipMemcpyDeviceToHost, c->stream));
    if (extra_out) HIPC(hipMemcpyAsync(extra_out, d_extra, extra_bytes, hipMemcpyDeviceToHost, c->stream));
    HIPC(hipStreamSynchronize(c->stream));
    if (d_act && act_out) for (size_t e = 0; e < E; ++e) act_out[e] = c->h_i[e];
    if (d_logp && logp_out) memcpy(logp_out, c->h_f, E * 4);
    if (d_val && value_out) memcpy(value_out, c->h_f + E, E * 4);
    return 0;
}
static inline void unpack_step(const float* pk, int n, bool last, int64_t* act_out, float* logp_out, float* value_out) {
    for (int e = 0; e < n; ++e) {
        if (act_out && !last) act_out[e] = (int64_t)pk[3 * e];
        if (logp_out && !last) logp_out[e] = pk[3 * e + 1];
        if (value_out) value_out[e] = pk[3 * e + 2];
    }
}
template <typename Gone>
static inline bool wait_ticket(const volatile unsigned* flag, unsigned want, Gone gone) {
    for (unsigned long long spin = 0; spin < (1ull << 34); ++spin) {
        if (__atomic_load_n(flag, __ATOMIC_ACQUIRE) == want) return true;
        __builtin_ia32_pause();
        if ((spin & 0xfffff) == 0xfffff && gone()) break;
    }
    return false;
}

int mi_policy_step(mi_ctx* c, int32_t t, uint64_t seed, const float* u, int64_t* act_out, float* logp_out, float* value_out) {
    ARG(c, "null"); JOIN(c); ARG(t >= 0 && t <= c->T, "t out of range");
    const int E = c->E;
    InputSrc src{obs_ring(c), nullptr, (long long)t * E};
    const float* du;
    if (int r = upload_u(c, u, c->stream, 0, E, &du)) return r;
    c->prof.phase = 0;
    net_forward(c, src, E, {.recurrent = true});
    const bool last = (t == c->T);
    launch_sample(c->hout, E, c->A, du, seed, (unsigned long long)t * E, last ? nullptr : c->act + (size_t)t * E,
                  last ? nullptr : c->logp + (size_t)t * E, c->value + (size_t)t * E, c->stream, c->lse);
    HIPC(hipGetLastError()); NETCHK(c);
    if (!act_out && !logp_out && !value_out) { if (u) HIPC(hipStreamSynchronize(c->stream)); return 0; }
    const size_t o = (size_t)t * E;
    return read_back_staged(c, (act_out && !last) ? c->act + o : nullptr, (logp_out && !last) ? c->logp + o : nullptr, value_out ? c->value + o : nullptr, act_out, logp_out, value_out);
}

int mi_rollout_step(mi_ctx* c, int32_t t, const float* rew_prev, const float* done_prev, uint64_t seed, const float* u,
                    int64_t* act_out, float* logp_out, float* value_out) {
    ARG(c, "null"); JOIN(c); ARG(t >= 0 && t <= c->T, "t out of range");
    const int E = c->E;
    if (rew_prev || done_prev) {
        ARG(rew_prev && done_prev && t >= 1, "rew_prev/done_prev come together and belong to step t-1");
        memcpy(c->h_rd, rew_prev, (size_t)E * 4); memcpy(c->h_rd + E, done_prev, (size_t)E * 4);
        if (c->gru_on) HIPC(hipMemcpyAsync(c->d_done, c->h_rd + E, (size_t)E * 4, hipMemcpyHostToDevice, c->stream));
    }
    const bool have_rd = rew_prev != nullptr;
    InputSrc src{obs_ring(c), nullptr, (long long)t * E};
    const float* du;
    if (int r = upload_u(c, u, c->stream, 0, E, &du)) return r;
    c->prof.phase = 0;
    net_forward(c, src, E, {.recurrent = true, .heads = false});
    const bool last = (t == c->T);
    launch_heads_sample(c->feat, c->params + c->wh_off, c->params + c->bh_off, E, c->H, c->A, du, seed, (unsigned long long)t * E,
                        last ? nullptr : c->act + (size_t)t * E, last ? nullptr : c->logp + (size_t)t * E, c->value + (size_t)t * E,
                        c->h_pack, nullptr, have_rd ? c->h_rd : nullptr, have_rd ? c->rew + (size_t)(t - 1) * E : nullptr,
                        have_rd ? c->done + (size_t)(t - 1) * E : nullptr, c->stream, c->d_done_ctr, c->h_flag, ++c->roll_ticket, c->lse);
    HIPC(hipGetLastError()); NETCHK(c);
    if (!wait_ticket(c->h_flag, c->roll_ticket, [&] { return hipStreamQuery(c->stream) != hipErrorNotReady; })) HIPC(hipStreamSynchronize(c->stream));
    unpack_step(c->h_pack, E, last, act_out, logp_out, value_out);
    return 0;
}

static void worker_drain(GroupWorker* w) {
    if (!w) return;
    while (w->done.load(std::memory_order_acquire) != w->posted.load(std::memory_order_acquire)) __builtin_ia32_pause();
}
int join_groups(mi_ctx* c) {
    for (int g = 0; g < c->n_groups; ++g) {
        if (!c->gs[g]) continue;
        worker_drain(c->gw[g]);
        if (c->g_dirty[g]) {
            HIPC(hipEventRecord(c->ev_join[g], c->gs[g]));
            HIPC(hipStreamWaitEvent(c->main_stream, c->ev_join[g], 0));
            c->g_dirty[g] = false;
        }
        c->g_forked[g] = false;
    }
    c->groups_live = false;
    return 0;
}

static int group_issue(mi_ctx* c, int g, const GroupJob& j) {
    const int E = c->E, ng = E / c->n_groups, e0 = g * ng;
    hipStream_t st = tl_stream;
    if (j.frames) {
        char* dst = obs_ring(c) + ((size_t)j.t * E + e0) * c->obs_bytes_per_env;
        if (c->copy_rate_bytes_per_us > 0) {
            const int64_t gap = (int64_t)((double)j.bytes * 1000.0 / c->copy_rate_bytes_per_us);
            const auto clk = [] { return (int64_t)std::chrono::duration_cast<std::chrono::nanoseconds>(std::chrono::steady_clock::now().time_since_epoch()).count(); };
            int64_t slot = c->copy_slot_ns.load(), start;
            do { const int64_t now = clk(); start = now > slot ? now : slot; } while (!c->copy_slot_ns.compare_exchange_weak(slot, start + gap));
            while (clk() < start) __builtin_ia32_pause();
        }
        if (j.pull) launch_pull_bytes(j.frames, dst, j.bytes, st);
        else HIPC(hipMemcpyAsync(dst, j.frames, j.bytes, hipMemcpyHostToDevice, st));
    }
    float* h_rd = c->h_rd + 2 * e0;
    if (j.have_rd && c->gru_on) HIPC(hipMemcpyAsync(c->d_done + e0, h_rd + ng, (size_t)ng * 4, hipMemcpyHostToDevice, st));
    const float* du;
    if (int r = upload_u(c, j.u, st, e0, ng, &du)) return r;
    InputSrc src{obs_ring(c), nullptr, (long long)j.t * E + e0};
    net_forward(c, src, ng, {.heads = false, .soff = e0});
    const float* hin = c->feat + (size_t)e0 * c->H;
    if (c->gru_on) {
        const size_t H = c->H;
        float* slot = c->h_ring + ((size_t)j.t * E + e0) * H;
        launch_gru_step(c->feat + (size_t)e0 * H, slot, c->d_done + e0, c->gru_wih, c->gru_whh, c->gru_bih, c->gru_bhh, c->h_state + (size_t)e0 * H,
                        j.last ? nullptr : slot + (size_t)E * H, ng, c->H, st);
        hin = c->h_state + (size_t)e0 * H;
    }
    const size_t o = (size_t)j.t * E + e0;
    launch_heads_sample(hin, c->params + c->wh_off, c->params + c->bh_off, ng, c->H, c->A, du, j.seed, (unsigned long long)j.t * E + e0,
                        j.last ? nullptr : c->act + o, j.last ? nullptr : c->logp + o, c->value + o, c->h_pack + 3 * e0, nullptr,
                        j.have_rd ? h_rd : nullptr, j.have_rd ? c->rew + o - E : nullptr, j.have_rd ? c->done + o - E : nullptr, st,
                        c->d_done_ctr + 1 + g, c->h_flag + 1 + g, j.ticket, c->lse);
    HIPC(hipGetLastError());
    if (const char* lf = mi_launch_failed_take()) return fail(-4, lf);
    return 0;
}
static void group_worker_main(mi_ctx* c, int g) {
    GroupWorker* w = c->gw[g];
    hipSetDevice(c->cfg.device);
    tl_stream = c->gs[g];
    tl_ws_floats = c->gemm_ws_floats / mi_ctx::MAX_GROUPS; tl_ws = c->gemm_ws + (size_t)g * tl_ws_floats;
    unsigned seen = 0;
    for (;;) {
        int spins = 0;
        while (w->posted.load(std::memory_order_acquire) == seen && !w->quit.load()) {
            if (++spins < 40000) __builtin_ia32_pause();
            else {
                std::unique_lock<std::mutex> lk(w->mu);
                w->sleeping.store(true);
                w->cv.wait_for(lk, std::chrono::milliseconds(50), [&] { return w->posted.load() != seen || w->quit.load(); });
                w->sleeping.store(false);
                spins = 0;
            }
        }
        if (w->quit.load()) return;
        seen = w->posted.load(std::memory_order_acquire);
        w->rc = group_issue(c, g, w->job);
        if (w->rc) w->err = g_err;
        w->done.store(seen, std::memory_order_release);
    }
}

int mi_rollout_groups(mi_ctx* c, int32_t n_groups) {
    ARG(c, "null"); ARG(n_groups >= 1 && n_groups <= mi_ctx::MAX_GROUPS, "1 .. 4 groups");
    ARG(c->E % n_groups == 0, "n_envs must be divisible by the number of groups");
    for (int g = 0; g < c->n_groups; ++g) ARG(!c->g_busy[g], "a group step is still in flight: mi_rollout_wait it first");
    JOIN(c);
    void* lane[mi_ctx::MAX_GROUPS]; int prio[mi_ctx::MAX_GROUPS];
    const int have = [&] { int k = 0; while (k < mi_ctx::MAX_GROUPS && c->gs[k]) ++k; return k; }();
    if (n_groups > have && !g_lanes[c->cfg.device].borrow(c, n_groups, c->cfg.device, lane_make, lane, prio))
        return fail(-2, "no stream for an env group (hipStreamCreateWithPriority failed)");
    for (int g = 0; g < n_groups; ++g)
        if (!c->gs[g]) {
            DevPool::Group both(c->pool);
            HIPC(c->pool.event(&c->ev_fork[g], hipEventDisableTiming));
            HIPC(c->pool.event(&c->ev_join[g], hipEventDisableTiming));
            both.keep = true;
            c->gs[g] = (hipStream_t)lane[g]; c->gs_prio[g] = prio[g];
            c->gw[g] = new GroupWorker();
            c->gw[g]->th = std::thread(group_worker_main, c, g);
        }
    c->n_groups = n_groups;
    return 0;
}

int mi_rollout_lane_info(mi_ctx* c, int32_t* n, int32_t* prio, uint64_t* stream_id) {
    ARG(c && n && prio && stream_id, "null");
    *n = 0;
    for (int g = 0; g < c->n_groups && c->gs[g]; ++g) { prio[g] = c->gs_prio[g]; stream_id[g] = (uint64_t)(uintptr_t)c->gs[g]; *n = g + 1; }
    return 0;
}

int mi_rollout_submit(mi_ctx* c, int32_t t, int32_t g, const void* frames, size_t bytes, const float* rew_prev, const float* done_prev,
                      uint64_t seed, const float* u) {
    ARG(c, "null"); ARG(t >= 0 && t <= c->T, "t out of range"); ARG(g >= 0 && g < c->n_groups, "group out of range");
    ARG(c->gs[g], "call mi_rollout_groups first"); ARG(!c->g_busy[g], "this group's previous step has not been waited for");
    ARG(c->pending_n < 0, "a multirank minibatch is pending");
    const int E = c->E, ng = E / c->n_groups, e0 = g * ng;
    ARG(!frames || bytes == (size_t)ng * c->obs_bytes_per_env, "frames byte count != (E / groups) * bytes_per_env");
    if (rew_prev || done_prev) ARG(rew_prev && done_prev && t >= 1, "rew_prev/done_prev come together and belong to step t-1");
    if (c->gru_on) {
        ARG(c->h_ring && (t > 0 || c->g_rec_ok[g]), "recurrent rollout: call mi_rec_begin before the groups' first step (t == 0) of every rollout");
        if (t == 0) c->g_rec_ok[g] = false;
    }
    GroupWorker* w = c->gw[g];
    worker_drain(w);
    if (!c->g_forked[g]) {
        fc_refresh(c);
        HIPC(hipEventRecord(c->ev_fork[g], c->main_stream));
        HIPC(hipStreamWaitEvent(c->gs[g], c->ev_fork[g], 0));
        c->g_forked[g] = true;
    }
    c->groups_live = true; c->g_dirty[g] = true;
    const bool have_rd = rew_prev != nullptr;
    if (have_rd) { float* h_rd = c->h_rd + 2 * e0; memcpy(h_rd, rew_prev, (size_t)ng * 4); memcpy(h_rd + ng, done_prev, (size_t)ng * 4); }
    const bool last = (t == c->T);
    bool pull = false;
    if (frames && !c->no_pull && bytes <= (512u << 10) && (bytes & 15) == 0 && ((uintptr_t)frames & 15) == 0) {
        auto it = c->pull_ok.find(frames);
        if (it == c->pull_ok.end()) {
            hipPointerAttribute_t at{};
            const bool ok = hipPointerGetAttributes(&at, frames) == hipSuccess && at.type == hipMemoryTypeHost && at.devicePointer == frames;
            if (!ok) (void)hipGetLastError();
            if (c->pull_ok.size() > 64) c->pull_ok.clear();
            it = c->pull_ok.emplace(frames, ok).first;
        }
        pull = it->second;
    }
    w->job = GroupJob{t, frames, bytes, pull, have_rd, last, u, seed, ++c->g_ticket[g]};
    w->posted.fetch_add(1, std::memory_order_seq_cst);
    if (w->sleeping.load()) { { std::lock_guard<std::mutex> lk(w->mu); } w->cv.notify_one(); }
    c->g_busy[g] = true; c->g_last[g] = last;
    return 0;
}

int mi_rollout_wait(mi_ctx* c, int32_t g, int64_t* act_out, float* logp_out, float* value_out) {
    ARG(c, "null"); ARG(g >= 0 && g < c->n_groups, "group out of range"); ARG(c->g_busy[g], "nothing submitted for this group");
    const int ng = c->E / c->n_groups, e0 = g * ng;
    const unsigned want = c->g_ticket[g];
    GroupWorker* w = c->gw[g];
    const bool seen = wait_ticket(c->h_flag + 1 + g, want, [&] { return w->done.load() == w->posted.load() && hipStreamQuery(c->gs[g]) != hipErrorNotReady; });
    worker_drain(w);
    c->g_busy[g] = false;
    if (w->rc) { const int rc = w->rc; w->rc = 0; return fail(rc, "group worker: " + w->err); }
    if (!seen) HIPC(hipStreamSynchronize(c->gs[g]));
    NETCHK(c);
    unpack_step(c->h_pack + 3 * e0, ng, c->g_last[g], act_out, logp_out, value_out);
    return 0;
}

int mi_predict_staged(mi_ctx* c, const void* obs, size_t bytes, uint64_t seed, uint64_t counter, const float* u,
                      int64_t* act_out, float* logp_out, float* value_out) {
    ARG(c && obs, "null"); JOIN(c);
    const int E = c->E;
    ARG(bytes == (size_t)E * c->obs_bytes_per_env, "obs byte count != E * bytes_per_env");
    void* stage = obs_stage(c);
    HIPC(hipMemcpyAsync(stage, obs, bytes, hipMemcpyHostToDevice, c->stream));
    const float* du;
    if (int r = upload_u(c, u, c->stream, 0, E, &du)) return r;
    InputSrc src{stage, nullptr, 0};
    net_forward(c, src, E, {.recurrent = true});
    launch_sample(c->hout, E, c->A, du, seed, counter, c->s_act, c->s_logp, c->s_val, c->stream, c->lse);
    HIPC(hipGetLastError()); NETCHK(c);
    if (int r = read_back_staged(c, c->s_act, c->s_logp, c->s_val, act_out, logp_out, value_out)) return r;
    c->staged_valid = true;
    return 0;
}

int mi_predict_greedy(mi_ctx* c, const void* obs, size_t bytes, int64_t* act_out, float* logp_out, float* value_out) {
    ARG(c && obs, "null"); JOIN(c);
    ARG(!c->gru_on, "mi_predict_greedy: a recurrent context (mi_set_gru) is not supported"); ARG(!c->lse, "mi_predict_greedy: value_from_logits is not supported");
    const int E = c->E;
    ARG(bytes == (size_t)E * c->obs_bytes_per_env, "obs byte count != E * bytes_per_env");
    void* stage = obs_stage(c);
    HIPC(hipMemcpyAsync(stage, obs, bytes, hipMemcpyHostToDevice, c->stream));
    InputSrc src{stage, nullptr, 0};
    net_forward(c, src, E, {});
    launch_ipl_greedy(c->hout, E, c->A, c->s_act, c->s_logp, c->s_val, c->stream);
    HIPC(hipGetLastError()); NETCHK(c);
    if (int r = read_back_staged(c, c->s_act, c->s_logp, c->s_val, act_out, logp_out, value_out)) return r;
    c->staged_valid = true;
    return 0;
}

int mi_value_saliency(mi_ctx* c, const void* obs, size_t bytes, uint64_t seed, uint64_t counter, const float* u,
// ... 460 lines not shown
}

int mi_minibatch_rec(mi_ctx* c, const int64_t* env_idx, int32_t n_env, const float* h0, int32_t n_global, const mi_hparams* hp) {
    ARG(c && hp && env_idx && h0, "null"); JOIN(c);
    ARG(c->gru_train, "GRU training is off: call mi_gru_train first");
    ARG(!c->lse, "value_from_logits with a trained GRU (recurrent ppo-pure) is not supported");
    ARG(hp->fs_coef == 0.f, "algo ppo-pure has no feature-sparsity term: fs_coef must be 0");
    ARG(c->multirank == 0 && !c->ar_armed && !c->comm, "GRU training runs on a single rank: multirank modes 1 / 2 and the in-library gradient exchange are refused");
    ARG(n_env >= 1 && n_global >= 1, "n_env / n_global");
    ARG((int64_t)n_env * c->T <= c->NB, "n_env * T must not exceed max_batch");
    ARG(c->log_count + 1 <= c->log_cap, "loss log full: call mi_loss_log_read(reset=1)");
    ARG(c->pending_n < 0, "previous multirank minibatch not finished");
    for (int i = 0; i < n_env; ++i) ARG(env_idx[i] >= 0 && env_idx[i] < c->E, "env index out of range");
    const int T = c->T, E = c->E, H = c->H, n = n_env, N = n_env * T;
    if (int r = stage_indices(c, N, [&](int32_t* h) { for (int t = 0; t < T; ++t) for (int i = 0; i < n; ++i) h[t * n + i] = (int32_t)(t * E + env_idx[i]); }, false)) return r;
    HIPC(hipMemcpyAsync(c->rec_h0, h0, (size_t)n * H * 4, hipMemcpyHostToDevice, c->stream));
    InputSrc src = minibatch_src(c);
    c->prof.phase = 1;
    c->prof.sample_now = (c->prof.mb_count++ % c->prof.period) == 0;
    const bool impala = c->cfg.arch == MI_ARCH_IMPALA;
    net_forward(c, src, N, {.heads = false, .train = true});
    HIPC(hipMemcpyAsync(c->rec_x, c->feat, (size_t)N * H * 4, hipMemcpyDeviceToDevice, c->stream));
    launch_gru_seq_mask(c->done, c->d_idx, c->rec_mask, N, c->stream);
    linear_fwd(c, c->rec_x, 0, c->gru_wih, c->gru_bih, c->rec_gi, N, H, 3 * H, 0);
    launch_gru_seq_fwd(c->rec_gi, c->rec_h0, c->rec_mask, c->gru_whh, c->gru_bhh, c->feat, c->rec_sv, T, n, H, c->stream);
    net_heads(c, N);
    LossArgs a = loss_args(c, N, n_global, hp);
    a.hp.fs_coef = 0.f;
    const bool batch_terms = hp->x_entropy_coef != 0.f;
    SegTab st{};
    st.n_seg = 1; st.start[1] = N;
    float* ring = c->stats_ring + (size_t)c->log_count * 32;
    a.stats = ring;
    loss_and_records(c, a, st, !batch_terms, 3, ring, c->fs_ring + c->log_count, c->loss_log + (size_t)c->log_count * 8);
    c->ring_args = a;
    c->log_count += 1;
    if (batch_terms) launch_loss_bwd(a, c->stream);
    heads_backward(c, N, 0, H <= 256 && c->A + 1 <= 16, false, c->stream);
    launch_gru_seq_bwd(c->dfeat, c->feat, c->rec_h0, c->rec_mask, c->rec_sv, c->gru_whh, c->rec_dgi, c->rec_dgh, c->rec_hm, T, n, H, c->stream);
    const size_t W = (size_t)3 * H * H, B = (size_t)3 * H;
    linear_wgrad(c, c->rec_dgi, c->rec_x, 0, c->gru_g, c->gru_g + 2 * W, N, H, 3 * H);
    linear_wgrad(c, c->rec_dgh, c->rec_hm, 0, c->gru_g + W, c->gru_g + 2 * W + B, N, H, 3 * H);
    linear_dgrad(c, c->rec_dgi, c->gru_wih, impala ? c->rec_x : nullptr, c->dfeat, N, H, 3 * H);
    c->bwd_from_dfeat = true;
    net_backward(c, src, N);
    c->bwd_from_dfeat = false;
    c->rec_last = true;
    HIPC(hipGetLastError()); NETCHK(c);
    return 0;
}

int mi_loss_log_read(mi_ctx* c, float* out, int32_t max_records, int32_t* n_records, int32_t reset) {
    ARG(c && n_records, "null"); JOIN(c);
    const int n = c->log_count < max_records ? c->log_count : max_records;
    if (out && n > 0) {
        HIPC(hipMemcpyAsync(out, c->loss_log, (size_t)n * 8 * 4, hipMemcpyDeviceToHost, c->stream));
        HIPC(hipStreamSynchronize(c->stream));
    }
    *n_records = n;
    if (reset) c->log_count = 0;
    return 0;
}

int mi_comm_unique_id(void* out, size_t bytes) {
    ARG(out && bytes >= sizeof(ncclUniqueId), "need a 128-byte buffer");
    ncclUniqueId id;
    NCCLC(ncclGetUniqueId(&id));
    memcpy(out, &id, sizeof id);
    return 0;
}
int mi_comm_init(mi_ctx* c, const void* id_bytes, size_t bytes, int32_t rank, int32_t world) {
    ARG(c && id_bytes && bytes >= sizeof(ncclUniqueId), "null / short id"); ARG(world >= 1 && rank >= 0 && rank < world, "rank / world");
    ARG(!c->comm, "communicator already initialised");
    JOIN(c);
    HIPC(hipSetDevice(c->cfg.device));
    ncclUniqueId id;
    memcpy(&id, id_bytes, sizeof id);
    struct Undo { mi_ctx* c; bool keep = false; ~Undo() { if (!keep) mi_comm_destroy(c); } } undo{c};
    NCCLC(ncclCommInitRank(&c->comm, world, id, rank));
    NCCLC(ncclCommSplit(c->comm, 0, rank, &c->comm_grad, nullptr));
    c->comm_world = world; c->comm_rank = rank;
    HIPC(hipStreamCreateWithFlags(&c->comm_stream, hipStreamNonBlocking));
    HIPC(c->comm_pool.event(&c->ev_ar_ready, hipEventDisableTiming));
    HIPC(c->comm_pool.event(&c->ev_ar_done, hipEventDisableTiming));
    HIPC(c->comm_pool.dev(&c->adv_all, (size_t)3 * world + 4));
    undo.keep = true;
    return 0;
}
int mi_comm_destroy(mi_ctx* c) {
    if (!c || !c->comm) return 0;
    if (c->comm_stream) hipStreamSynchronize(c->comm_stream);
    hipStreamSynchronize(c->stream);
    if (c->comm_grad) { ncclCommDestroy(c->comm_grad); c->comm_grad = nullptr; }
    ncclCommDestroy(c->comm); c->comm = nullptr;
    c->comm_pool.release_all();
    if (c->comm_stream) { hipStreamDestroy(c->comm_stream); c->comm_stream = nullptr; }
    c->comm_world = 1; c->comm_rank = 0;
    c->ar_armed = c->ar_issued = c->ar_inflight = false;
    return 0;
}
int mi_allreduce_arm(mi_ctx* c) {
    ARG(c, "null"); ARG(c->comm, "no communicator: call mi_comm_init first"); ARG(!c->ar_inflight, "a gradient all-reduce is already in flight");
    c->ar_armed = true;
    return 0;
}
int mi_allreduce_grads(mi_ctx* c) {
    ARG(c, "null"); ARG(c->comm, "no communicator: call mi_comm_init first"); JOIN(c);
    if (c->ar_issued) return 0;
    c->ar_armed = true;
    issue_grad_allreduce(c, 0, c->n_params, true);
    NETCHK(c);
    return 0;
}
int mi_allreduce_buffer(mi_ctx* c, int32_t which, int64_t n) {
    ARG(c, "null"); ARG(c->comm, "no communicator: call mi_comm_init first"); JOIN(c);
    if (which == MI_PTR_FS_KEYS) {
        ARG(c->fs_keys && n == 2048, "MI_PTR_FS_KEYS: the 2048 keys of an IMPALA context");
        NCCLC(ncclAllReduce(c->fs_keys, c->fs_keys, 2048, ncclInt64, ncclMax, c->comm, c->stream));
        return 0;
    }
    float* p = nullptr; int64_t cap = 0;
    switch (which) {
        case MI_PTR_LOSS_STATS: p = c->loss_stats; cap = 32; break;
        case MI_PTR_STATS_RING: p = c->stats_ring; cap = (int64_t)c->log_cap * 32; break;
        case MI_PTR_GRADS: p = c->grads; cap = c->n_params; break;
        default: return fail(-1, "mi_allreduce_buffer: unknown buffer id");
    }
    ARG(n >= 1 && n <= cap, "count");
    NCCLC(ncclAllReduce(p, p, (size_t)n, ncclFloat, ncclSum, c->comm, c->stream));
    return 0;
}
int mi_adv_normalize_global(mi_ctx* c) {
    ARG(c, "null"); ARG(c->comm, "no communicator: call mi_comm_init first"); JOIN(c);
    launch_advnorm_stats(c->adv, c->T * c->E, c->adv_stats, c->stream);
    NCCLC(ncclAllGather(c->adv_stats, c->adv_all, 3, ncclDouble, c->comm, c->stream));
    launch_advnorm_merge(c->adv_all, c->comm_world, c->adv_stats, c->stream);
    launch_advnorm_apply(c->adv, c->T * c->E, c->adv_stats, c->stream);
    HIPC(hipGetLastError());
    return 0;
}

int mi_device_ptr(mi_ctx* c, int32_t which, void** ptr, int64_t* n) {
    ARG(c && ptr && n, "null"); JOIN(c);
    switch (which) {
        case MI_PTR_GRADS: *ptr = c->grads; *n = c->n_params; return 0;
        case MI_PTR_LOSS_STATS: *ptr = c->loss_stats; *n = 32; return 0;
        case MI_PTR_PARAMS: *ptr = c->params; *n = c->n_params; return 0;
        case MI_PTR_STATS_RING: *ptr = c->stats_ring; *n = (int64_t)c->log_cap * 32; return 0;
        case MI_PTR_FS_KEYS: ARG(c->fs_keys, "IMPALA contexts only"); *ptr = c->fs_keys; *n = 2048; return 0;
        default: return fail(-1, "unknown pointer id");
    }
}

int mi_debug_flags(mi_ctx* c, int32_t flags) { ARG(c, "null"); JOIN(c); c->rollout_tail = !(flags & 1); c->no_pull = (flags & 4) != 0; c->side_on = !(flags & 16); return 0; }
```

### train-procgen-pytorch_amd/csrc/engine_ctx.h

```cpp
#pragma once
#include "common.h"
#include "devpool.h"
#include "../../include/mi355ppo.h"
#include <rccl/rccl.h>
#include <math.h>
#include <stdio.h>
#include <string.h>
#include <string>
#include <unordered_map>
#include <vector>
#include <atomic>
#include <chrono>
#include <condition_variable>
#include <deque>
#include <mutex>
#include <thread>

#pragma clang diagnostic ignored "-Wc++20-designator"
#define MI_INTERNAL __attribute__((visibility("hidden")))

MI_INTERNAL extern thread_local std::string g_err;
MI_INTERNAL extern thread_local hipStream_t tl_stream;
MI_INTERNAL extern thread_local float* tl_ws;
MI_INTERNAL extern thread_local size_t tl_ws_floats;
#define CUR(c) (tl_stream ? tl_stream : (c)->stream)
static inline int fail(int code, const std::string& msg) { g_err = msg; return code; }

#define HIPC(x)                                                                                          \
    do {                                                                                                 \
        hipError_t e_ = (hipError_t)(x);       \
        if (e_ != hipSuccess)                                                                            \
            return fail(-2, std::string(#x) + ": " + hipGetErrorString(e_) + " @" + std::to_string(__LINE__)); \
    } while (0)
#define ARG(c, msg) do { if (!(c)) return fail(-1, std::string("invalid argument: ") + msg); } while (0)
#define NETCHK(c) do { if (const char* lf_ = mi_launch_failed_take()) return fail(-4, lf_);                                   \
                       std::string m_ = net_err_take(c); if (!m_.empty()) return fail(-4, m_); } while (0)
#define JOIN(c) do { if ((c)->groups_live) { int r_ = join_groups(c); if (r_) return r_; } } while (0)


enum TKind { K_PLAIN = 0, K_CONVW, K_FCW };
struct TensorDesc {
    std::string name;
    int64_t ref_off, dev_off, n;
    int kind, co, ci;
};

struct ConvLayer { ConvShape shape; int64_t w_off, b_off; int cin, cout, hw; long long bank_f = -1, bank_d = -1; };
struct Block { float *C = nullptr, *P0 = nullptr, *A1 = nullptr, *P1 = nullptr, *A2 = nullptr, *P2 = nullptr; uint8_t* PI = nullptr; int cin = 0, cout = 0, hin = 0; };
struct Linear { int64_t w_off, b_off; int in, out; };

enum ProfClass { PC_CONV_FWD = 0, PC_CONV_DGRAD = 5, PC_CONV_WGRAD = 10, PC_POOL_FWD = 15, PC_POOL_BWD, PC_GEMM, PC_SLAB_REDUCE, PC_RESBLOCK, PC_RESBLOCK_BWD = PC_RESBLOCK + 5, PC_COUNT = PC_RESBLOCK_BWD + 5 };
struct ProfPending { hipEvent_t a, b; int cls, phase; long long units; double bytes, flops; };
struct Profiler {
    bool on = false;
    bool all_phases = false;
    int phase = 0;
    int period = 1, mb_count = 0;
    bool sample_now = true;
    std::vector<ProfPending> pend;
    std::vector<hipEvent_t> pool;
    std::deque<hipEvent_t> made;
    double ms[2][PC_COUNT] = {};
    long long launches[2][PC_COUNT] = {}, units[2][PC_COUNT] = {};
    double bytes[2][PC_COUNT] = {}, flops[2][PC_COUNT] = {};
};

MI_INTERNAL const DevPool::Backend* hip_pool();
struct mi_ctx {
    Profiler prof;
    mi_config cfg = {};
    hipStream_t stream = nullptr;
    bool own_stream = false;
    int T = 0, E = 0, A = 0, H = 0, NB = 0;
    bool bf = false;
    double es = 4.0;
    int64_t n_params = 0;
    std::vector<TensorDesc> tensors;
    float *params = nullptr, *grads = nullptr, *adam_m = nullptr, *adam_v = nullptr;
    uint8_t* frames = nullptr;
    float* obsf = nullptr;
    size_t obs_bytes_per_env = 0;
    float *rew = nullptr, *done = nullptr, *logp = nullptr, *adv = nullptr, *ret = nullptr, *value = nullptr;
    int32_t* act = nullptr;
    double* adv_stats = nullptr;
    std::vector<ConvLayer> convs;
    Block blk[3];
    Linear fc = {};
    std::vector<Linear> mlp;
    std::vector<float*> mlp_act;
    int64_t wh_off = 0, bh_off = 0;
    float *feat = nullptr, *hout = nullptr, *dY = nullptr, *dfeat = nullptr, *GC = nullptr, *GP[3] = {};
    int lse = 0; float* d_val = nullptr;
    float* slabs = nullptr; size_t slab_floats = 0;
    void* sal_dc = nullptr; float* sal_dx = nullptr; const float* sal_src = nullptr;
    long long slab_off[15] = {}; SlabDesc h_slab_desc[15] = {}; SlabDesc* d_slab_desc = nullptr; int slab_desc_n = 0, slab_desc_cached_n = -1;
    float *gemm_ws = nullptr, *col_ws = nullptr, *fs_scratch = nullptr, *fs_val = nullptr; size_t gemm_ws_floats = 0;
    float* lut = nullptr;
    unsigned short* lut16 = nullptr;
    uint8_t* stage_frames = nullptr; float* stage_obs = nullptr;
    int32_t* d_idx = nullptr;
    float *loss_partial = nullptr, *loss_stats = nullptr, *loss_log = nullptr; int log_count = 0, log_cap = 4096;
    double* fs_parts = nullptr;
    float *stats_ring = nullptr, *fs_ring = nullptr; LossArgs ring_args = {};
    double* sumsq = nullptr; float* gnorm = nullptr;
    float* d_u = nullptr; float* d_lp = nullptr;
    unsigned short* banks = nullptr; BankDesc* d_bank_desc = nullptr; int n_banks = 0;
    unsigned short* c1_bank = nullptr;
    unsigned short *fc_wp = nullptr, *fc_wt = nullptr;
    bool fc_packed_valid = false;
    float *d_pack = nullptr, *h_pack = nullptr, *h_rd = nullptr, *d_rd = nullptr;
    unsigned *d_done_ctr = nullptr, *h_flag = nullptr, roll_ticket = 0;
    int32_t* s_act = nullptr; float *s_logp = nullptr, *s_val = nullptr; bool staged_valid = false;
    bool gru_on = false; float *gru_wih = nullptr, *gru_whh = nullptr, *gru_bih = nullptr, *gru_bhh = nullptr, *h_state = nullptr, *h_masked = nullptr, *gru_gi = nullptr, *gru_gh = nullptr, *d_done = nullptr;
    float *gru_x = nullptr, *gru_dg = nullptr; bool sal_keep_x = false, bwd_from_dfeat = false;
    static constexpr int IDX_RING = 32;
    int32_t* h_idx_ring[IDX_RING] = {}; hipEvent_t idx_ev[IDX_RING] = {}; bool idx_used[IDX_RING] = {}; int idx_next = 0, idx_ev_deferred = -1;
    float* h_f = nullptr; int32_t* h_i = nullptr; size_t h_f_floats = 0;
    int multirank = 0;
    LossArgs pending = {}; int pending_n = -1;
    static constexpr int MAX_GROUPS = 4;
    int n_groups = 1; hipStream_t main_stream = nullptr, gs[MAX_GROUPS] = {}; int gs_prio[MAX_GROUPS] = {}; hipEvent_t ev_fork[MAX_GROUPS] = {}, ev_join[MAX_GROUPS] = {};
    bool g_forked[MAX_GROUPS] = {}, g_busy[MAX_GROUPS] = {}, g_last[MAX_GROUPS] = {}, g_dirty[MAX_GROUPS] = {}; unsigned g_ticket[MAX_GROUPS] = {}; bool groups_live = false;
    struct GroupWorker* gw[MAX_GROUPS] = {};
    std::atomic<int64_t> copy_slot_ns{0}; double copy_rate_bytes_per_us = 40000.0;
    std::unordered_map<const void*, bool> pull_ok; bool no_pull = false;
    hipStream_t side_stream = nullptr; hipEvent_t ev_side_fork = nullptr, ev_side_join = nullptr;
    bool side_on = true;
    struct SideJob { bool armed; LossArgs a; SegTab st; int mode; float* ring; float* fsr; float* log; } side = {};
    bool rollout_tail = true;
    float *fs_colmax = nullptr, fs_grad_coef = 0.f; int *fs_arg = nullptr, fs_G = 0;
    long long *fs_keys = nullptr, *fs_keys_local = nullptr; int32_t *d_gpos = nullptr, *h_gpos = nullptr; int gpos_n = -1; bool fs_global_pending = false, fs_global_apply = false;
    ncclComm_t comm = nullptr, comm_grad = nullptr; int comm_world = 1, comm_rank = 0; hipStream_t comm_stream = nullptr; hipEvent_t ev_ar_ready = nullptr, ev_ar_done = nullptr;
    bool ar_armed = false, ar_issued = false, ar_inflight = false; double* adv_all = nullptr;
    std::string net_err; std::mutex net_err_mu;
    float *h_ring = nullptr, *h_rec_stage = nullptr; hipEvent_t ev_rec = nullptr; bool g_rec_ok[MAX_GROUPS] = {};
    bool gru_train = false, rec_last = false; float *gru_g = nullptr, *gru_m = nullptr, *gru_v = nullptr; double* gru_sumsq = nullptr;
    float *rec_x = nullptr, *rec_gi = nullptr, *rec_sv = nullptr, *rec_dgi = nullptr, *rec_dgh = nullptr, *rec_hm = nullptr, *rec_mask = nullptr, *rec_h0 = nullptr;
    int32_t* ipl_idx2 = nullptr; float *ipl_nv = nullptr, *ipl_gnext = nullptr, *ipl_pred = nullptr, *ipl_rew = nullptr; double* ipl_partial = nullptr;
    int ipl_last_n = 0;
    struct mi_sae* sae = nullptr;
    DevPool pool{hip_pool()}, comm_pool{hip_pool()};
};

static inline char* obs_ring(mi_ctx* c) { return c->frames ? (char*)c->frames : (char*)c->obsf; }

MI_INTERNAL std::string net_err_take(mi_ctx* c);
MI_INTERNAL void net_err_set(mi_ctx* c, const std::string& m);
MI_INTERNAL void sae_release(mi_ctx* c);
MI_INTERNAL int join_groups(mi_ctx* c);
MI_INTERNAL void to_device_layout(const TensorDesc& t, const float* ref, float* dev);
MI_INTERNAL void to_ref_layout(const TensorDesc& t, const float* dev, float* ref);
MI_INTERNAL std::vector<uint16_t> host_to_bf16(const float* x, size_t n);
struct InputSrc { const void* base; const int32_t* idx; long long first; };
struct FwdOpts { bool recurrent = false; bool heads = true; bool train = false; int soff = 0; };
MI_INTERNAL void net_forward(mi_ctx* c, const InputSrc& src, int n, const FwdOpts& o);
MI_INTERNAL void linear_fwd(mi_ctx* c, const float* X, int relu_x, const float* W, const float* b, float* Y, int n, int in, int out, int relu_out, int x_bf16 = 0);
MI_INTERNAL void linear_dgrad(mi_ctx* c, const float* dY, const float* W, const float* mask, float* dX, int n, int in, int out, int x_bf16 = 0);
MI_INTERNAL void linear_wgrad(mi_ctx* c, const float* dY, const float* X, int relu_x, float* gW, float* gb, int n, int in, int out, int x_bf16 = 0);
```

### train-procgen-pytorch_amd/csrc/heads.hip

```cpp
#include "common.h"
#include "policy_math.h"
#include <hip/hip_ext.h>
#include <math.h>

__global__ __launch_bounds__(256) void heads_fwd_kernel(const float* __restrict__ feat, const float* __restrict__ Wh, const float* __restrict__ bh,
                                                        float* __restrict__ hout, int n, int O) {
    __shared__ __attribute__((aligned(16))) float s_f[16 * 260];
    __shared__ __attribute__((aligned(16))) float s_w[16 * 260];
    const int tid = threadIdx.x, e0 = blockIdx.x * 16, el = tid >> 4, o = tid & 15;
    f32x4 rf[4], rw[4];
#pragma unroll
    for (int j = 0; j < 4; ++j) {
        const int k = tid + j * 256, r = k >> 6, kk = (k & 63) * 4;
        const int rr = e0 + r < n ? e0 + r : n - 1;
        rf[j] = *(const f32x4*)(feat + (long long)rr * 256 + kk);
        rw[j] = *(const f32x4*)(Wh + (long long)(r < O ? r : O - 1) * 256 + kk);
    }
#pragma unroll
    for (int j = 0; j < 4; ++j) { const int k = tid + j * 256; *(f32x4*)(s_f + (k >> 6) * 260 + (k & 63) * 4) = rf[j]; *(f32x4*)(s_w + (k >> 6) * 260 + (k & 63) * 4) = rw[j]; }
    __syncthreads();
    const float* w = s_w + o * 260;
    const float* f = s_f + el * 260;
    float acc = 0.f;
#pragma unroll 8
// ... 54 lines not shown
    if (k < O) sl[(long long)O * H + k] = gb;
}
static int heads_bwd_grid(int n) { const int g = (n + 15) / 16; return g > 512 ? 512 : g; }
void launch_heads_bwd_reduce(const float* ws, float* gW, float* gb, int n, int H, int O, hipStream_t st) {
    if (n <= 0) return;
    launch_reduce_slabs(ws, heads_bwd_grid(n), O * H + O, gW, O * H, gb, O, st);
}
void launch_heads_bwd(const float* dY, const float* feat, const float* Wh, int relu_mask, float* dfeat, float* gW, float* gb, float* ws,
                      int n, int H, int O, hipStream_t st, bool with_reduce, hipEvent_t done_ev) {
    if (n <= 0) return;
    if (done_ev) hipExtLaunchKernelGGL(heads_bwd_kernel, dim3(heads_bwd_grid(n)), dim3(256), 0, st, nullptr, done_ev, 0, dY, feat, Wh, relu_mask, dfeat, ws, n, H, O);
    else
    hipLaunchKernelGGL(heads_bwd_kernel, dim3(heads_bwd_grid(n)), dim3(256), 0, st, dY, feat, Wh, relu_mask, dfeat, ws, n, H, O);
    if (with_reduce) launch_heads_bwd_reduce(ws, gW, gb, n, H, O, st);
}

template <bool LSE>
__global__ void sample_kernel(const float* hout, int n, int A, const float* u, unsigned long long seed,
                              unsigned long long ctr, int32_t* act, float* logp, float* value) {
    const int e = blockIdx.x * blockDim.x + threadIdx.x;
    if (e >= n) return;
    const float* h = hout + (long long)e * (A + 1);
    float z[MAXA], lp[MAXA], p[MAXA];
    for (int k = 0; k < A; ++k) z[k] = h[k];
    float lse = 0.f, q1[MAXA];
    log_softmax_twice_t<LSE>(z, A, lp, p, lse, q1);
    const float uu = u ? u[e] : philox_uniform(seed, ctr + e);
    float cdf = 0.f;
    int a_sel = 0;
    for (int k = 0; k < A; ++k) { cdf += expf(lp[k]); if (cdf <= uu) a_sel = k + 1; }
    if (a_sel > A - 1) a_sel = A - 1;
    if (act) act[e] = a_sel;
    if (logp) logp[e] = lp[a_sel];
    if (value) value[e] = LSE ? lse : h[A];
}
template <bool LSE>
__global__ void logp_all_kernel(const float* hout, int n, int A, float* lp_out, float* value_out) {
    const int e = blockIdx.x * blockDim.x + threadIdx.x;
    if (e >= n) return;
    const float* h = hout + (long long)e * (A + 1);
    float z[MAXA], lp[MAXA], p[MAXA];
    for (int k = 0; k < A; ++k) z[k] = h[k];
    float lse = 0.f, q1[MAXA];
    log_softmax_twice_t<LSE>(z, A, lp, p, lse, q1);
    if (lp_out) for (int k = 0; k < A; ++k) lp_out[(long long)e * A + k] = lp[k];
    if (value_out) value_out[e] = LSE ? lse : h[A];
}
void launch_logp_all(const float* hout, int n, int A, float* lp_out, float* value_out, hipStream_t st, int value_from_logits) {
    if (n <= 0) return;
    if (value_from_logits) hipLaunchKernelGGL(logp_all_kernel<true>, dim3((n + 63) / 64), dim3(64), 0, st, hout, n, A, lp_out, value_out);
    else hipLaunchKernelGGL(logp_all_kernel<false>, dim3((n + 63) / 64), dim3(64), 0, st, hout, n, A, lp_out, value_out);
}
__global__ void philox_debug_kernel(const uint32_t* in6, int n, uint32_t* out4, float* u_out) {
    const int i = blockIdx.x * blockDim.x + threadIdx.x;
    if (i >= n) return;
    uint32_t c[4] = {in6[6 * i], in6[6 * i + 1], in6[6 * i + 2], in6[6 * i + 3]};
    uint32_t k[2] = {in6[6 * i + 4], in6[6 * i + 5]};
    philox4x32_10(c, k);
    for (int j = 0; j < 4; ++j) out4[4 * i + j] = c[j];
    u_out[i] = philox_uniform((unsigned long long)in6[6 * i + 4] | ((unsigned long long)in6[6 * i + 5] << 32),
                              (unsigned long long)in6[6 * i] | ((unsigned long long)in6[6 * i + 1] << 32));
}
void launch_philox_debug(const uint32_t* in6, int n, uint32_t* out4, float* u_out, hipStream_t st) {
    if (n <= 0) return;
    hipLaunchKernelGGL(philox_debug_kernel, dim3((n + 255) / 256), dim3(256), 0, st, in6, n, out4, u_out);
}
template <bool WIDE, bool LSE>
__global__ __launch_bounds__(256) void heads_sample_kernel(const float* __restrict__ feat, const float* __restrict__ Wh,
                                                           const float* __restrict__ bh, int n, int H, int A, const float* u,
                                                           unsigned long long seed, unsigned long long ctr, int32_t* act,
                                                           float* logp, float* value, float* pack, float* hout,
                                                           const float* rd, float* rew_dst, float* done_dst,
                                                           unsigned* done_ctr, unsigned* host_flag, unsigned ticket) {
    __shared__ __attribute__((aligned(16))) float s_f[16 * 260];
    __shared__ __attribute__((aligned(16))) float s_w[17 * 260];
    __shared__ float s_z[16 * 17];
    const int tid = threadIdx.x, e0 = blockIdx.x * 16;
    const int el = tid >> 4, o = tid & 15, e = e0 + el;
    float rwd = 0.f, dn = 0.f;
    if (rd && o == 0 && e < n) { rwd = rd[e]; dn = rd[n + e]; }
    if constexpr (WIDE) {
        float acc0 = 0.f, acc1 = 0.f;
        for (int c0 = 0; c0 < H; c0 += 256) {
            const int HC = H - c0 < 256 ? H - c0 : 256;
            __syncthreads();
            if ((H & 3) == 0) {
                const int H4 = HC >> 2;
                for (int k = tid; k < 16 * H4; k += 256) {
                    const int r = k / H4, kk = (k % H4) * 4;
                    *(f32x4*)(s_f + r * 260 + kk) = (e0 + r < n) ? *(const f32x4*)(feat + (long long)(e0 + r) * H + c0 + kk) : (f32x4){0.f, 0.f, 0.f, 0.f};
                }
                for (int k = tid; k < (A + 1) * H4; k += 256) {
                    const int r = k / H4, kk = (k % H4) * 4;
                    *(f32x4*)(s_w + r * 260 + kk) = *(const f32x4*)(Wh + (long long)r * H + c0 + kk);
                }
            } else {
                for (int k = tid; k < 16 * HC; k += 256) { const int r = k / HC, kk = k % HC; s_f[r * 260 + kk] = (e0 + r < n) ? feat[(long long)(e0 + r) * H + c0 + kk] : 0.f; }
                for (int k = tid; k < (A + 1) * HC; k += 256) { const int r = k / HC, kk = k % HC; s_w[r * 260 + kk] = Wh[(long long)r * H + c0 + kk]; }
            }
            __syncthreads();
            auto dot = [&](int oo, float acc) {
                const float* w = s_w + oo * 260;
                const float* f = s_f + el * 260;
                int k = 0;
                for (; k + 4 <= HC; k += 4) {
                    const f32x4 fv = *(const f32x4*)(f + k), ww = *(const f32x4*)(w + k);
                    acc += fv.x * ww.x + fv.y * ww.y + fv.z * ww.z + fv.w * ww.w;
                }
                for (; k < HC; ++k) acc += f[k] * w[k];
                return acc;
            };
            if (o <= A) acc0 = dot(o, acc0);
            if (o + 16 <= A) acc1 = dot(o + 16, acc1);
        }
        if (o <= A) s_z[el * 17 + o] = acc0 + bh[o];
        if (o + 16 <= A) s_z[el * 17 + o + 16] = acc1 + bh[o + 16];
    } else {
    if (H == 256) {
        f32x4 rf[4], rw[5];
#pragma unroll
        for (int j = 0; j < 4; ++j) {
            const int k = tid + j * 256, r = k >> 6, kk = (k & 63) * 4;
            rf[j] = (e0 + r < n) ? *(const f32x4*)(feat + (long long)(e0 + r) * 256 + kk) : (f32x4){0.f, 0.f, 0.f, 0.f};
        }
#pragma unroll
        for (int j = 0; j < 5; ++j) {
            const int k = tid + j * 256, r = k >> 6, kk = (k & 63) * 4;
            rw[j] = (r <= A) ? *(const f32x4*)(Wh + (long long)r * 256 + kk) : (f32x4){0.f, 0.f, 0.f, 0.f};
        }
#pragma unroll
        for (int j = 0; j < 4; ++j) { const int k = tid + j * 256; *(f32x4*)(s_f + (k >> 6) * 260 + (k & 63) * 4) = rf[j]; }
#pragma unroll
        for (int j = 0; j < 5; ++j) { const int k = tid + j * 256; if ((k >> 6) <= A) *(f32x4*)(s_w + (k >> 6) * 260 + (k & 63) * 4) = rw[j]; }
    } else if ((H & 3) == 0) {
        const int H4 = H >> 2;
        for (int k = tid; k < 16 * H4; k += 256) {
            const int r = k / H4, kk = (k % H4) * 4;
            *(f32x4*)(s_f + r * 260 + kk) = (e0 + r < n) ? *(const f32x4*)(feat + (long long)(e0 + r) * H + kk) : (f32x4){0.f, 0.f, 0.f, 0.f};
        }
        for (int k = tid; k < (A + 1) * H4; k += 256) {
            const int r = k / H4, kk = (k % H4) * 4;
            *(f32x4*)(s_w + r * 260 + kk) = *(const f32x4*)(Wh + (long long)r * H + kk);
        }
    } else {
        for (int k = tid; k < 16 * H; k += 256) { const int r = k / H, kk = k % H; s_f[r * 260 + kk] = (e0 + r < n) ? feat[(long long)(e0 + r) * H + kk] : 0.f; }
        for (int k = tid; k < (A + 1) * H; k += 256) { const int r = k / H, kk = k % H; s_w[r * 260 + kk] = Wh[(long long)r * H + kk]; }
    }
    __syncthreads();
    for (int oo = o; oo <= A; oo += 16) {
        const float* w = s_w + oo * 260;
        const float* f = s_f + el * 260;
        float acc = 0.f;
        int k = 0;
        if (H == 256) {
#pragma unroll 8
            for (; k < 256; k += 4) {
                const f32x4 fv = *(const f32x4*)(f + k), ww = *(const f32x4*)(w + k);
                acc += fv.x * ww.x + fv.y * ww.y + fv.z * ww.z + fv.w * ww.w;
            }
        }
        for (; k + 4 <= H; k += 4) {
            const f32x4 fv = *(const f32x4*)(f + k), ww = *(const f32x4*)(w + k);
            acc += fv.x * ww.x + fv.y * ww.y + fv.z * ww.z + fv.w * ww.w;
        }
        for (; k < H; ++k) acc += f[k] * w[k];
        s_z[el * 17 + oo] = acc + bh[oo];
    }
    }
    __syncthreads();
    __shared__ __attribute__((aligned(16))) float s_t[16 * 16];
    const bool lane_on = o < A;
    auto row = [&](float term, float (&v)[16]) {
        __builtin_amdgcn_wave_barrier();
        s_t[el * 16 + o] = term;
        __builtin_amdgcn_wave_barrier();
        const f32x4 a0 = *(const f32x4*)(s_t + el * 16), a1 = *(const f32x4*)(s_t + el * 16 + 4);
        const f32x4 a2 = *(const f32x4*)(s_t + el * 16 + 8), a3 = *(const f32x4*)(s_t + el * 16 + 12);
        v[0] = a0.x; v[1] = a0.y; v[2] = a0.z; v[3] = a0.w; v[4] = a1.x; v[5] = a1.y; v[6] = a1.z; v[7] = a1.w;
        v[8] = a2.x; v[9] = a2.y; v[10] = a2.z; v[11] = a2.w; v[12] = a3.x; v[13] = a3.y; v[14] = a3.z; v[15] = a3.w;
    };
    auto group_sum = [&](float term) {
        float v[16];
        row(term, v);
        float t = 0.f;
#pragma unroll
        for (int k = 0; k < 16; ++k) if (k < A) t += v[k];
        return t;
    };
    const float z = lane_on ? s_z[el * 17 + o] : 0.f;
    float mx;
    {
        float v[16];
        row(z, v);
        mx = v[0];
#pragma unroll
        for (int k = 1; k < 16; ++k) if (k < A) mx = fmaxf(mx, v[k]);
    }
    const float s1 = group_sum(lane_on ? expf(z - mx) : 0.f);
    const float lse1 = mx + logf(s1);
    float lp = z - lse1;
    const float s2 = group_sum(lane_on ? expf(lp) : 0.f);
    lp -= logf(s2);
    const float pr = lane_on ? expf(lp) : 0.f;
    float cdf = 0.f;
    {
        float v[16];
        row(pr, v);
#pragma unroll
        for (int k = 0; k < 16; ++k) if (k < A) cdf += (k <= o) ? v[k] : 0.f;
    }
    const float uu = (e < n) ? (u ? u[e] : philox_uniform(seed, ctr + e)) : 0.f;
    const float mark = (lane_on && cdf <= uu) ? (float)(o + 1) : 0.f;
    float sel = 0.f;
    {
        float v[16];
        row(mark, v);
#pragma unroll
        for (int k = 0; k < 16; ++k) if (k < A) sel = fmaxf(sel, v[k]);
    }
    int a_sel = (int)sel;
    if (a_sel > A - 1) a_sel = A - 1;
    float lp_pick;
    {
        float v[16];
        row(lp, v);
        lp_pick = v[0];
#pragma unroll
        for (int k = 1; k < 16; ++k) lp_pick = (k == a_sel) ? v[k] : lp_pick;
    }
    if (o == 0 && e < n) {
        const float lp_sel = lp_pick, val = LSE ? lse1 : s_z[el * 17 + A];
        if (rd) { rew_dst[e] = rwd; done_dst[e] = dn; }
        if (act) act[e] = a_sel;
        if (logp) logp[e] = lp_sel;
        if (value) value[e] = val;
        if (pack) { pack[e * 3] = (float)a_sel; pack[e * 3 + 1] = lp_sel; pack[e * 3 + 2] = val; }
        if (hout) for (int k = 0; k <= A; ++k) hout[(long long)e * (A + 1) + k] = s_z[el * 17 + k];
    }
    if (host_flag) {
        __threadfence_system();
        __syncthreads();
        if (threadIdx.x == 0) {
            const unsigned old = atomicAdd(done_ctr, 1u);
            if (old == gridDim.x - 1) {
                *done_ctr = 0;
                __threadfence_system();
                __hip_atomic_store(host_flag, ticket, __ATOMIC_RELEASE, __HIP_MEMORY_SCOPE_SYSTEM);
            }
        }
    }
}
void launch_heads_sample(const float* feat, const float* Wh, const float* bh, int n, int H, int A, const float* u,
                         unsigned long long seed, unsigned long long ctr, int32_t* act, float* logp, float* value, float* pack,
                         float* hout, const float* rd, float* rew_dst, float* done_dst, hipStream_t st,
                         unsigned* done_ctr, unsigned* host_flag, unsigned ticket, int value_from_logits) {
    if (n <= 0) return;
    auto go = [&](auto kernel) {
        hipLaunchKernelGGL(kernel, dim3((n + 15) / 16), dim3(256), 0, st, feat, Wh, bh, n, H, A, u, seed, ctr, act, logp, value, pack, hout,
                           rd, rew_dst, done_dst, done_ctr, host_flag, ticket);
    };
    if (value_from_logits) { if (H > 256) go(heads_sample_kernel<true, true>); else go(heads_sample_kernel<false, true>); }
    else if (H > 256) go(heads_sample_kernel<true, false>);
    else go(heads_sample_kernel<false, false>);
}
void launch_sample(const float* hout, int n, int A, const float* u, unsigned long long seed, unsigned long long ctr,
                   int32_t* act, float* logp, float* value, hipStream_t st, int value_from_logits) {
    if (n <= 0) return;
    if (value_from_logits) hipLaunchKernelGGL(sample_kernel<true>, dim3((n + 63) / 64), dim3(64), 0, st, hout, n, A, u, seed, ctr, act, logp, value);
    else hipLaunchKernelGGL(sample_kernel<false>, dim3((n + 63) / 64), dim3(64), 0, st, hout, n, A, u, seed, ctr, act, logp, value);
}
```

### train-procgen-pytorch_amd/csrc/policy_math.h

```cpp
#pragma once
#include <hip/hip_runtime.h>
#include <stdint.h>
#include <math.h>

#define MAXA 16
template <bool LSE>
__device__ __forceinline__ void log_softmax_twice_t(const float* z, int A, float* lp, float* p, float& lse_out, float* q1) {
    float mx = z[0];
#pragma unroll
    for (int a = 1; a < MAXA; ++a) if (a < A) mx = fmaxf(mx, z[a]);
    float s = 0.f;
#pragma unroll
    for (int a = 0; a < MAXA; ++a) if (a < A) s += expf(z[a] - mx);
    const float lse = mx + logf(s);
    float s2 = 0.f;
#pragma unroll
    for (int a = 0; a < MAXA; ++a) if (a < A) { lp[a] = z[a] - lse; const float e1 = expf(lp[a]); s2 += e1; if (LSE) q1[a] = e1; }
    if (LSE) lse_out = lse;
    const float lse2 = logf(s2);
    float s3 = 0.f;
#pragma unroll
    for (int a = 0; a < MAXA; ++a) if (a < A) { lp[a] -= lse2; p[a] = expf(lp[a]); s3 += p[a]; }
#pragma unroll
    for (int a = 0; a < MAXA; ++a) if (a < A) p[a] /= s3;
}

__device__ __forceinline__ void philox_round(uint32_t* c, uint32_t* k) {
    const uint32_t M0 = 0xD2511F53u, M1 = 0xCD9E8D57u;
    const uint32_t hi0 = __umulhi(M0, c[0]), lo0 = M0 * c[0];
    const uint32_t hi1 = __umulhi(M1, c[2]), lo1 = M1 * c[2];
    const uint32_t n0 = hi1 ^ c[1] ^ k[0], n2 = hi0 ^ c[3] ^ k[1];
    c[0] = n0; c[1] = lo1; c[2] = n2; c[3] = lo0;
    k[0] += 0x9E3779B9u; k[1] += 0xBB67AE85u;
}
__device__ __forceinline__ void philox4x32_10(uint32_t* c, uint32_t* k) {
#pragma unroll
    for (int r = 0; r < 10; ++r) philox_round(c, k);
}
__device__ __forceinline__ float philox_uniform(unsigned long long seed, unsigned long long ctr) {
    uint32_t c[4] = {(uint32_t)ctr, (uint32_t)(ctr >> 32), 0u, 0u};
    uint32_t k[2] = {(uint32_t)seed, (uint32_t)(seed >> 32)};
    philox4x32_10(c, k);
    return (float)(c[0] >> 8) * (1.0f / 16777216.0f);
}
```

### train-procgen-pytorch_amd/csrc/rollout_bf16.hip

```cpp
#include "common.h"
#include "device_util.h"
#include <mutex>

__device__ __forceinline__ unsigned rt_relu2(unsigned w) { const unsigned neg = (w >> 15) & 0x00010001u; return w & ~(neg * 0xFFFFu); }

#ifndef RT_NT
#define RT_NT 512
#endif
namespace rt {
constexpr int NT = RT_NT, NW = NT / 64;
constexpr int S16 = 16, S32 = 48, SCS = 48;
constexpr int P32 = 34, P16 = 18, P8 = 10;
constexpr int IN_ELEMS = P32 * P32 * S16;
constexpr int X16_ELEMS = P16 * P16 * S32;
constexpr int X8_ELEMS = P8 * P8 * S32;
constexpr int KB2_ELEMS = 9 * 33 * SCS;
constexpr int KB3_ELEMS = 17 * 17 * SCS;
constexpr int WS16 = 5 * 32 + 16, WS32 = 9 * 32 + 16;
constexpr int W_ELEMS = 32 * WS32;
constexpr int R_IN = 0, R_X = R_IN + IN_ELEMS, R_Y = R_X + X16_ELEMS, R_W = R_Y + X16_ELEMS, R_B = R_W + 2 * W_ELEMS;
constexpr int LDS_ELEMS = R_B + 10 * 32 * 2;
static_assert(KB2_ELEMS <= X16_ELEMS && KB3_ELEMS <= IN_ELEMS && 2 * X8_ELEMS <= X16_ELEMS, "region reuse");
static_assert(LDS_ELEMS * 2 <= 160 * 1024, "LDS");
constexpr int KW = (W_ELEMS / 8 + NT - 1) / NT;
}

struct RolloutTailArgs {
    const unsigned short* x;
    unsigned short* y;
    int n;
    const unsigned short* bank[10];
    const float* bias[10];
};

struct KoffTab { int v[5]; __device__ __forceinline__ int operator()(int m) const { return v[m]; } };
template <int P> struct KoffC { __device__ __forceinline__ constexpr int operator()(int m) const { return ((m / 3) * P + (m % 3)) * 48; } };
template <int NK, int WS, bool RELU_A, int MTC, class KO>
__device__ __forceinline__ void rt_conv(const unsigned short* s_src, const unsigned short* s_w, const KO koff, const int (&abase)[MTC],
                                        int bbase, f32x4 (&acc)[MTC][2], int nmt = MTC) {
#pragma unroll
    for (int mt = 0; mt < MTC; ++mt) { acc[mt][0] = (f32x4){0.f, 0.f, 0.f, 0.f}; acc[mt][1] = (f32x4){0.f, 0.f, 0.f, 0.f}; }
#pragma unroll
    for (int m = 0; m < NK; ++m) {
        bf16x8 av[MTC];
#pragma unroll
        for (int mt = 0; mt < MTC; ++mt) {
            if (mt >= nmt) continue;
            av[mt] = *(const bf16x8*)(s_src + abase[mt] + koff(m));
            if (RELU_A) {
                const uint4 u = __builtin_bit_cast(uint4, av[mt]);
                av[mt] = __builtin_bit_cast(bf16x8, (uint4){mi_relu_bf16x2(u.x), mi_relu_bf16x2(u.y), mi_relu_bf16x2(u.z), mi_relu_bf16x2(u.w)});
            }
        }
        const bf16x8 b0 = *(const bf16x8*)(s_w + bbase + m * 32), b1 = *(const bf16x8*)(s_w + bbase + 16 * WS + m * 32);
#pragma unroll
        for (int mt = 0; mt < MTC; ++mt)
            if (mt < nmt) { acc[mt][0] = MFMA_BF16(b0, av[mt], acc[mt][0]); acc[mt][1] = MFMA_BF16(b1, av[mt], acc[mt][1]); }
    }
}
template <bool RELU_A>
__device__ __forceinline__ f32x4 rt_conv1(const unsigned short* s_src, const unsigned short* s_w, int abase, int bbase) {
    f32x4 acc = {0.f, 0.f, 0.f, 0.f};
    constexpr KoffC<10> koff;
#pragma unroll
    for (int m = 0; m < 9; ++m) {
        bf16x8 av = *(const bf16x8*)(s_src + abase + koff(m));
        if (RELU_A) {
            const uint4 u = __builtin_bit_cast(uint4, av);
            av = __builtin_bit_cast(bf16x8, (uint4){mi_relu_bf16x2(u.x), mi_relu_bf16x2(u.y), mi_relu_bf16x2(u.z), mi_relu_bf16x2(u.w)});
        }
        acc = MFMA_BF16(*(const bf16x8*)(s_w + bbase + m * 32), av, acc);
    }
    return acc;
}

__global__ __launch_bounds__(rt::NT) void rollout_tail_bf16_kernel(RolloutTailArgs a) {
    using namespace rt;
    extern __shared__ __attribute__((aligned(16))) unsigned short smem_h[];
    unsigned short* s_in = smem_h + R_IN;
    unsigned short* s_x = smem_h + R_X;
    unsigned short* s_y = smem_h + R_Y;
    unsigned short* s_w[2] = {smem_h + R_W, smem_h + R_W + W_ELEMS};
    float* s_b = (float*)(smem_h + R_B);
    const int tid = threadIdx.x, lane = tid & 63, wave = tid >> 6, i = lane & 15, kq = lane >> 4;

    KoffTab koff2;
#pragma unroll
    for (int m = 0; m < 5; ++m) { int tap = 2 * m + (kq >> 1); const int chunk = kq & 1; if (tap > 8) tap = 8; koff2.v[m] = ((tap / 3) * P32 + (tap % 3)) * S16 + chunk * 8; }
    static_assert(S32 == 48, "KoffC assumes the 32-channel pixel stride");
    const int bb16 = i * WS16 + kq * 8, bb32 = i * WS32 + kq * 8;

    typedef unsigned rt_u32x4 __attribute__((ext_vector_type(4)));
    rt_u32x4 wreg[2][KW];
    auto bank_fetch = [&](int k) {
        const int words = (k == 0 ? 32 * WS16 : W_ELEMS) / 8;
#pragma unroll
        for (int q = 0; q < KW; ++q) { const int e = tid + q * NT; wreg[k & 1][q] = e < words ? ((const rt_u32x4*)a.bank[k])[e] : (rt_u32x4){0u, 0u, 0u, 0u}; }
    };
    auto bank_commit = [&](int k) {
        const int words = (k == 0 ? 32 * WS16 : W_ELEMS) / 8;
#pragma unroll
        for (int q = 0; q < KW; ++q) { const int e = tid + q * NT; if (e < words) ((rt_u32x4*)s_w[k & 1])[e] = wreg[k & 1][q]; }
    };
    auto bank_step = [&](int c) { bank_commit(c + 1); if (c + 3 <= 9) bank_fetch(c + 3); };

    for (int img = blockIdx.x; img < a.n; img += gridDim.x) {
        rt_u32x4 xin[2048 / NT];
        {
            const rt_u32x4* g = (const rt_u32x4*)(a.x + (long long)img * 32 * 32 * 16);
#pragma unroll
            for (int q = 0; q < 2048 / NT; ++q) xin[q] = g[tid + q * NT];
        }
        bank_fetch(0); bank_fetch(1);
        const float bias_v = tid < 320 ? a.bias[tid >> 5][tid & 31] : 0.f;
        __syncthreads();
        for (int e = tid; e < (IN_ELEMS + X16_ELEMS) / 8; e += NT) ((uint4*)smem_h)[e] = (uint4){0u, 0u, 0u, 0u};
        for (int e = tid; e < 9 * 16; e += NT) ((unsigned*)s_y)[(e >> 4) * 33 * (SCS / 2) + (e & 15)] = MI_KEY_MIN2;
        if (tid < 320) s_b[tid] = bias_v;
        bank_commit(0);
        bank_fetch(2);
        __syncthreads();
#pragma unroll
        for (int q = 0; q < 2048 / NT; ++q) {
            const int e = tid + q * NT, c8 = e & 1, px = (e >> 1) & 31, r = e >> 6;
            *(rt_u32x4*)(s_in + ((r + 1) * P32 + px + 1) * S16 + c8 * 8) = xin[q];
        }
        __syncthreads();

        for (int band = 0; band < 4; ++band) {
            const int cy0 = 8 * band - 1;
            constexpr int MTB = (18 + NW - 1) / NW;
            const int nmtb = (18 - __builtin_amdgcn_readfirstlane(wave) + NW - 1) / NW;
            f32x4 acc[MTB][2];
            int abase[MTB], cbase[MTB];
            bool dead[MTB];
#pragma unroll
            for (int mt = 0; mt < MTB; ++mt) {
                int t = wave + NW * mt;
                const bool live = t < 18;
                t = live ? t : 17;
                const int pl = t * 16 + i, y = pl >> 5, x = pl & 31, cy = cy0 + y;
                dead[mt] = cy < 0;
                abase[mt] = ((cy < 0 ? 0 : cy) * P32 + x) * S16;
                cbase[mt] = live ? (y * 33 + x + 1) * SCS + kq * 4 : -1;
            }
            rt_conv<5, WS16, false, MTB, KoffTab>(s_in, s_w[0], koff2, abase, bb16, acc, nmtb);
#pragma unroll
            for (int mt = 0; mt < MTB; ++mt) {
                if (cbase[mt] < 0) continue;
#pragma unroll
                for (int nb = 0; nb < 2; ++nb) {
                    const f32x4 bq = *(const f32x4*)(s_b + nb * 16 + kq * 4);
                    const unsigned k0 = mi_bf16x2_to_keys(mi_pk_bf16(acc[mt][nb][0] + bq[0], acc[mt][nb][1] + bq[1]));
                    const unsigned k1 = mi_bf16x2_to_keys(mi_pk_bf16(acc[mt][nb][2] + bq[2], acc[mt][nb][3] + bq[3]));
                    *(uint2*)(s_y + cbase[mt] + nb * 16) = (uint2){dead[mt] ? MI_KEY_MIN2 : k0, dead[mt] ? MI_KEY_MIN2 : k1};
                }
            }
            if (band == 0) { bank_commit(1); bank_fetch(3); }
            __syncthreads();
            if (tid < 256) {
                const int c8 = tid & 3, ox = (tid >> 2) & 15, oyl = tid >> 6;
                uint4 u[9];
#pragma unroll
                for (int ky = 0; ky < 3; ++ky)
#pragma unroll
                    for (int kx = 0; kx < 3; ++kx) u[ky * 3 + kx] = *(const uint4*)(s_y + ((2 * oyl + ky) * 33 + 2 * ox + kx) * SCS + c8 * 8);
                uint4 pk; uint2 ar;
                mi_pool9_keys(u, pk, ar);
                *(uint4*)(s_x + ((4 * band + oyl + 1) * P16 + ox + 1) * S32 + c8 * 8) = pk;
            }
            __syncthreads();
        }
        for (int e = tid; e < X16_ELEMS / 8; e += NT) ((uint4*)s_y)[e] = (uint4){0u, 0u, 0u, 0u};
        __syncthreads();

        constexpr int MT16 = 16 / NW;
        {
            int abase[MT16], cen[MT16];
#pragma unroll
            for (int mt = 0; mt < MT16; ++mt) { const int pl = (wave + NW * mt) * 16 + i, y = pl >> 4, x = pl & 15; abase[mt] = (y * P16 + x) * S32 + kq * 8; cen[mt] = (y * P16 + x) * S32 + (P16 + 1) * S32 + kq * 4; }
#pragma unroll
            for (int st = 0; st < 2; ++st) {
                const int k1 = 1 + 2 * st, k2 = k1 + 1;
                f32x4 acc[MT16][2];
                rt_conv<9, WS32, true, MT16, KoffC<P16>>(s_x, s_w[k1 & 1], KoffC<P16>(), abase, bb32, acc);
#pragma unroll
                for (int mt = 0; mt < MT16; ++mt)
#pragma unroll
                    for (int nb = 0; nb < 2; ++nb) {
                        const f32x4 bq = *(const f32x4*)(s_b + k1 * 32 + nb * 16 + kq * 4);
                        float v[4];
#pragma unroll
                        for (int r = 0; r < 4; ++r) v[r] = acc[mt][nb][r] + bq[r];
                        const uint2 raw = mi_pk_bf16x4(v);
                        *(uint2*)(s_y + cen[mt] + nb * 16) = (uint2){rt_relu2(raw.x), rt_relu2(raw.y)};
                    }
                bank_step(k1);
                __syncthreads();
                rt_conv<9, WS32, false, MT16, KoffC<P16>>(s_y, s_w[k2 & 1], KoffC<P16>(), abase, bb32, acc);
#pragma unroll
                for (int mt = 0; mt < MT16; ++mt)
#pragma unroll
                    for (int nb = 0; nb < 2; ++nb) {
                        const f32x4 bq = *(const f32x4*)(s_b + k2 * 32 + nb * 16 + kq * 4);
                        const uint2 sk = *(const uint2*)(s_x + cen[mt] + nb * 16);
                        float v[4];
#pragma unroll
                        for (int r = 0; r < 4; ++r) v[r] = acc[mt][nb][r] + bq[r] + mi_bf16x4_lane(sk, r);
                        *(uint2*)(s_x + cen[mt] + nb * 16) = mi_pk_bf16x4(v);
                    }
                bank_step(k2);
                __syncthreads();
            }
        }

        unsigned short* s_k3 = s_in;
        unsigned short* s_x8 = s_y;
        unsigned short* s_y8 = s_x;
        {
            for (int e = tid; e < 17 * 16; e += NT) {
                const int cell = e >> 4, d = e & 15;
                ((unsigned*)s_k3)[cell * (SCS / 2) + d] = MI_KEY_MIN2;
                if (cell >= 1) ((unsigned*)s_k3)[cell * 17 * (SCS / 2) + d] = MI_KEY_MIN2;
            }
            for (int e = tid; e < X8_ELEMS / 8; e += NT) ((uint4*)s_x8)[e] = (uint4){0u, 0u, 0u, 0u};
            int abase[MT16], cbase[MT16];
#pragma unroll
            for (int mt = 0; mt < MT16; ++mt) { const int pl = (wave + NW * mt) * 16 + i, y = pl >> 4, x = pl & 15; abase[mt] = (y * P16 + x) * S32 + kq * 8; cbase[mt] = ((y + 1) * 17 + x + 1) * SCS + kq * 4; }
            f32x4 acc[MT16][2];
            rt_conv<9, WS32, false, MT16, KoffC<P16>>(s_x, s_w[5 & 1], KoffC<P16>(), abase, bb32, acc);
#pragma unroll
            for (int mt = 0; mt < MT16; ++mt)
#pragma unroll
                for (int nb = 0; nb < 2; ++nb) {
                    const f32x4 bq = *(const f32x4*)(s_b + 5 * 32 + nb * 16 + kq * 4);
                    const unsigned k0 = mi_bf16x2_to_keys(mi_pk_bf16(acc[mt][nb][0] + bq[0], acc[mt][nb][1] + bq[1]));
                    const unsigned k1 = mi_bf16x2_to_keys(mi_pk_bf16(acc[mt][nb][2] + bq[2], acc[mt][nb][3] + bq[3]));
                    *(uint2*)(s_k3 + cbase[mt] + nb * 16) = (uint2){k0, k1};
                }
            bank_step(5);
            __syncthreads();
            for (int e = tid; e < X8_ELEMS / 8; e += NT) ((uint4*)s_y8)[e] = (uint4){0u, 0u, 0u, 0u};
            if (tid < 256) {
                const int c8 = tid & 3, ox = (tid >> 2) & 7, oy = tid >> 5;
                uint4 u[9];
#pragma unroll
                for (int ky = 0; ky < 3; ++ky)
#pragma unroll
                    for (int kx = 0; kx < 3; ++kx) u[ky * 3 + kx] = *(const uint4*)(s_k3 + ((2 * oy + ky) * 17 + 2 * ox + kx) * SCS + c8 * 8);
                uint4 pk; uint2 ar;
                mi_pool9_keys(u, pk, ar);
                *(uint4*)(s_x8 + ((oy + 1) * P8 + ox + 1) * S32 + c8 * 8) = pk;
            }
            __syncthreads();
        }

        {
            const bool on = wave < 8;
            const int tile = (wave & 7) >> 1, nb = wave & 1;
            const int pl = tile * 16 + i, y = pl >> 3, x = pl & 7;
            const int abase = (y * P8 + x) * S32 + kq * 8, cen = (y * P8 + x) * S32 + (P8 + 1) * S32 + kq * 4 + nb * 16;
            const int bbn = bb32 + nb * 16 * WS32;
#pragma unroll
            for (int st = 0; st < 2; ++st) {
                const int k1 = 6 + 2 * st, k2 = k1 + 1;
                f32x4 acc = {0.f, 0.f, 0.f, 0.f};
                if (on) acc = rt_conv1<true>(s_x8, s_w[k1 & 1], abase, bbn);
                if (on) {
                    const f32x4 bq = *(const f32x4*)(s_b + k1 * 32 + nb * 16 + kq * 4);
                    float v[4];
#pragma unroll
                    for (int r = 0; r < 4; ++r) v[r] = acc[r] + bq[r];
                    const uint2 raw = mi_pk_bf16x4(v);
                    *(uint2*)(s_y8 + cen) = (uint2){rt_relu2(raw.x), rt_relu2(raw.y)};
                }
                bank_step(k1);
                __syncthreads();
                if (on) acc = rt_conv1<false>(s_y8, s_w[k2 & 1], abase, bbn);
                if (on) {
                    const f32x4 bq = *(const f32x4*)(s_b + k2 * 32 + nb * 16 + kq * 4);
                    const uint2 sk = *(const uint2*)(s_x8 + cen);
                    float v[4];
#pragma unroll
                    for (int r = 0; r < 4; ++r) v[r] = acc[r] + bq[r] + mi_bf16x4_lane(sk, r);
                    const uint2 raw = mi_pk_bf16x4(v);
                    if (k2 < 9) *(uint2*)(s_x8 + cen) = raw;
                    else *(uint2*)(a.y + ((long long)img * 64 + pl) * 32 + nb * 16 + kq * 4) = raw;
                }
                if (k2 < 9) bank_step(k2);
                __syncthreads();
            }
        }
    }
}

void launch_rollout_tail_bf16(const void* x, void* y, int n, const unsigned short* const* bank, const float* const* bias, hipStream_t st) {
    if (n <= 0) return;
    static std::once_flag attr;
    std::call_once(attr, [] { hipFuncSetAttribute((const void*)rollout_tail_bf16_kernel, hipFuncAttributeMaxDynamicSharedMemorySize, rt::LDS_ELEMS * 2); });
    RolloutTailArgs a{};
    a.x = (const unsigned short*)x; a.y = (unsigned short*)y; a.n = n;
    for (int k = 0; k < 10; ++k) { a.bank[k] = bank[k]; a.bias[k] = bias[k]; }
    hipLaunchKernelGGL(rollout_tail_bf16_kernel, dim3(n < 256 ? n : 256), dim3(rt::NT), rt::LDS_ELEMS * 2, st, a);
}
```

Baseline: 724,700.

## Fuse FC layer and policy head sampling into rollout tail kernel

Adds a rollout_step kernel that continues the fused resblock tail with the 2048x256 FC layer as MFMA, using a new pre-packed fc_wf weight layout. It then computes the policy/value heads, samples the action, and signals the host flag, all within one launch per image. This removes the separate FC and heads_sample launches, along with their inter-kernel gaps and feature round-trips, from the latency-bound rollout step. In exchange, each block redundantly streams the full FC weight matrix, and the grid is now n blocks instead of at most 256.

Measured after the change: 730,300 (median of 6 runs). Within noise of the previous version (+0.8%).

```diff
diff --git a/scratch/ro_timeline4.py b/scratch/ro_timeline4.py
--- a/scratch/ro_timeline4.py
+++ b/scratch/ro_timeline4.py
@@ -5,11 +5,12 @@
 by = collections.defaultdict(list)
 for r in rows:
     by[r[key]].append(r)
-streams = [(k, v) for k, v in by.items() if sum(1 for r in v if "heads_sample" in r["Kernel_Name"]) > 200]
+last = lambda r: "heads_sample" in r["Kernel_Name"] or "rollout_step_bf16" in r["Kernel_Name"]
+streams = [(k, v) for k, v in by.items() if sum(1 for r in v if last(r)) > 200]
 print("streams with a rollout chain:", [(k, len(v)) for k, v in streams], "key", key)
 k, v = streams[0]
 v.sort(key=lambda r: int(r["Start_Timestamp"]))
-idx = [i for i, r in enumerate(v) if "heads_sample" in r["Kernel_Name"]]
+idx = [i for i, r in enumerate(v) if last(r)]
 a, b = idx[-150], idx[-149]
 base = int(v[a]["End_Timestamp"])
 for r in v[a + 1:b + 1]:
diff --git a/train-procgen-pytorch_amd/csrc/common.h b/train-procgen-pytorch_amd/csrc/common.h
--- a/train-procgen-pytorch_amd/csrc/common.h
+++ b/train-procgen-pytorch_amd/csrc/common.h
@@ -62,7 +62,7 @@
 void launch_conv_wgrad_bf16(ConvShape s, const WgradArgs& a, hipStream_t st);
 int  conv1_bank_elems();
 void launch_repack_all(const float* params, unsigned short* banks, const BankDesc* d_desc, int n_desc, const float* c1_w, unsigned short* c1_bank ,
-                       const float* fc_w, unsigned short* fc_wp, unsigned short* fc_wt, int H , hipStream_t st);
+                       const float* fc_w, unsigned short* fc_wp, unsigned short* fc_wt, unsigned short* fc_wf, int H , hipStream_t st);
 void launch_conv1_pool_fwd_bf16(const ConvArgs& a, const unsigned short* lut16, void* p_out, uint8_t* p_arg, hipStream_t st);
 void launch_conv1_fwd_bf16(const ConvArgs& a, const unsigned short* lut16, hipStream_t st);
 void launch_conv1_wgrad_bf16(const WgradArgs& a, const unsigned short* lut16, hipStream_t st);
@@ -86,6 +86,15 @@
                                const unsigned short* const* bank, hipStream_t st);
 
 void launch_rollout_tail_bf16(const void* x, void* y, int n, const unsigned short* const* bank, const float* const* bias, hipStream_t st);
+struct StepHead {
+    const float* u; unsigned long long seed, ctr;
+    int32_t* act; float *logp, *value, *pack, *hout;
+    const float* rd; float *rew_dst, *done_dst;
+    unsigned *done_ctr, *host_flag; unsigned ticket;
+};
+void launch_rollout_step_bf16(const void* x, void* y, int n, const unsigned short* const* bank, const float* const* bias,
+                              const unsigned short* fc_wf, const float* fc_b, float* feat, const float* Wh, const float* bh, int A,
+                              int value_from_logits, const StepHead& s, hipStream_t st);
 
 template <template <int> class F, typename... Args>
 static inline bool fc_dispatch_width(int D, Args... args) {
diff --git a/train-procgen-pytorch_amd/csrc/conv_bf16.hip b/train-procgen-pytorch_amd/csrc/conv_bf16.hip
--- a/train-procgen-pytorch_amd/csrc/conv_bf16.hip
+++ b/train-procgen-pytorch_amd/csrc/conv_bf16.hip
@@ -1129,7 +1129,8 @@
 template <int D>
 __global__ void repack_all_kernel(const float* __restrict__ params, unsigned short* __restrict__ banks, const BankDesc* __restrict__ desc, int n_desc,
                                   const float* __restrict__ c1_w, unsigned short* __restrict__ c1_bank,
-                                  const float* __restrict__ fc_w, unsigned short* __restrict__ fc_wp, unsigned short* __restrict__ fc_wt) {
+                                  const float* __restrict__ fc_w, unsigned short* __restrict__ fc_wp, unsigned short* __restrict__ fc_wt,
+                                  unsigned short* __restrict__ fc_wf) {
     constexpr int C1B = (16 * C1_WS + 255) / 256;
     int b = blockIdx.x;
     if (b < 8 * n_desc) {
@@ -1159,18 +1160,20 @@
         const unsigned short h = f2bf(fc_w[e]);
         fc_wp[e] = h;
         fc_wt[(long long)(e % 2048) * D + e / 2048] = h;
+        const int n = e / 2048, k = e % 2048;
+        fc_wf[(((n >> 4) * 64 + (k >> 5)) * 64 + ((k >> 3) & 3) * 16 + (n & 15)) * 8 + (k & 7)] = h;
     }
 }
 template <int D> struct RepackAll {
     static void run(const float* params, unsigned short* banks, const BankDesc* d_desc, int n_desc, const float* c1_w, unsigned short* c1_bank,
-                    const float* fc_w, unsigned short* fc_wp, unsigned short* fc_wt, hipStream_t st) {
+                    const float* fc_w, unsigned short* fc_wp, unsigned short* fc_wt, unsigned short* fc_wf, hipStream_t st) {
         const int blocks = 8 * n_desc + (16 * C1_WS + 255) / 256 + D * 2048 / 256;
-        hipLaunchKernelGGL(repack_all_kernel<D>, dim3(blocks), dim3(256), 0, st, params, banks, d_desc, n_desc, c1_w, c1_bank, fc_w, fc_wp, fc_wt);
+        hipLaunchKernelGGL(repack_all_kernel<D>, dim3(blocks), dim3(256), 0, st, params, banks, d_desc, n_desc, c1_w, c1_bank, fc_w, fc_wp, fc_wt, fc_wf);
     }
 };
 void launch_repack_all(const float* params, unsigned short* banks, const BankDesc* d_desc, int n_desc, const float* c1_w, unsigned short* c1_bank,
-                       const float* fc_w, unsigned short* fc_wp, unsigned short* fc_wt, int H, hipStream_t st) {
-    if (!fc_dispatch_width<RepackAll>(H, params, banks, d_desc, n_desc, c1_w, c1_bank, fc_w, fc_wp, fc_wt, st))
+                       const float* fc_w, unsigned short* fc_wp, unsigned short* fc_wt, unsigned short* fc_wf, int H, hipStream_t st) {
+    if (!fc_dispatch_width<RepackAll>(H, params, banks, d_desc, n_desc, c1_w, c1_bank, fc_w, fc_wp, fc_wt, fc_wf, st))
         mi_launch_fail("repack_all: no fc image kernel for this output_dim");
 }
 __global__ __launch_bounds__(256, 4) void conv1_pool_fwd_bf16_kernel(ConvArgs a, const unsigned short* lut16, unsigned short* p_out, uint8_t* p_arg) {
diff --git a/train-procgen-pytorch_amd/csrc/engine.hip b/train-procgen-pytorch_amd/csrc/engine.hip
--- a/train-procgen-pytorch_amd/csrc/engine.hip
+++ b/train-procgen-pytorch_amd/csrc/engine.hip
@@ -304,7 +304,7 @@
     HIPC(m.pinned(&c->h_i, (size_t)E * sizeof(int32_t), hipHostMallocDefault));
     if (getenv("MI355_COPY_GBPS")) c->copy_rate_bytes_per_us = atof(getenv("MI355_COPY_GBPS")) * 1000.0;
     if (c->bf) {
-        HIPC(m.dev(&c->fc_wp, (size_t)c->H * 2048)); HIPC(m.dev(&c->fc_wt, (size_t)c->H * 2048));
+        HIPC(m.dev(&c->fc_wp, (size_t)c->H * 2048)); HIPC(m.dev(&c->fc_wt, (size_t)c->H * 2048)); HIPC(m.dev(&c->fc_wf, (size_t)c->H * 2048));
         HIPC(m.dev(&c->c1_bank, (size_t)conv1_bank_elems()));
         std::vector<BankDesc> desc;
         long long off = 0;
@@ -651,7 +651,7 @@
 static void fc_refresh(mi_ctx* c) {
     if (c->bf && !c->fc_packed_valid) {
         launch_repack_all(c->params, c->banks, c->d_bank_desc, c->n_banks, c->convs.empty() ? nullptr : c->params + c->convs[0].w_off,
-                          c->convs.empty() ? nullptr : c->c1_bank, c->params + c->fc.w_off, c->fc_wp, c->fc_wt, c->H, CUR(c));
+                          c->convs.empty() ? nullptr : c->c1_bank, c->params + c->fc.w_off, c->fc_wp, c->fc_wt, c->fc_wf, c->H, CUR(c));
         c->fc_packed_valid = true;
     }
 }
@@ -697,8 +697,10 @@
     linear_fwd(c, prev, 1, c->params + c->fc.w_off, c->params + c->fc.b_off, feat, n, 2048, c->H, 1, 0);
 }
 
-static bool forward_impala_bf16(mi_ctx* c, const InputSrc& src, int n, int soff, float* feat, bool train) {
+static bool forward_impala_bf16(mi_ctx* c, const InputSrc& src, int n, float* feat, const FwdOpts& o) {
+    const int soff = o.soff; const bool train = o.train;
     const bool fused_tail = !train && n <= 256 && c->rollout_tail;
+    const bool fused_step = fused_tail && o.step && o.step_fused && !c->step_split && c->H == 256 && c->A + 1 <= 16 && !c->gru_on;
     const float* prev = nullptr;
     for (int b = 0; b < 3; ++b) {
         const Block k = block_view(c, b, soff);
@@ -707,9 +709,19 @@
             const unsigned short* bk[10]; const float* bb[10];
             for (int q = 0; q < 10; ++q) { bk[q] = c->banks + c->convs[5 + q].bank_f; bb[q] = c->params + c->convs[5 + q].b_off; }
             const Block k3 = block_view(c, 2, soff);
-            { const double px2 = (double)n * 32 * 32, px3 = (double)n * 16 * 16;
-              ProfScope ps(c, PC_RESBLOCK + (int)CS_32_32_16, n, 2.0 * (px2 * 16 + px3 / 4 * 32), px2 * 18.0 * 16 * 32 + 5.0 * px3 * 18.0 * 32 * 32 + 4.0 * (px3 / 4) * 18.0 * 32 * 32);
-              launch_rollout_tail_bf16(prev, k3.P2, n, bk, bb, CUR(c)); }
+            { const double px2 = (double)n * 32 * 32, px3 = (double)n * 16 * 16, H = c->H, O = c->A + 1;
+              double bytes = 2.0 * (px2 * 16 + px3 / 4 * 32), flops = px2 * 18.0 * 16 * 32 + 5.0 * px3 * 18.0 * 32 * 32 + 4.0 * (px3 / 4) * 18.0 * 32 * 32;
+              if (fused_step) {
+                  bytes += 2.0 * n * 2048 + 2.0 * 2048 * H + 4.0 * n * H + 4.0 * ((double)n * H + (double)n * O + H * O);
+                  flops += 2.0 * n * 2048 * H + 2.0 * n * H * O;
+              }
+              ProfScope ps(c, PC_RESBLOCK + (int)CS_32_32_16, n, bytes, flops);
+              if (fused_step) {
+                  launch_rollout_step_bf16(prev, k3.P2, n, bk, bb, c->fc_wf, c->params + c->fc.b_off, feat, c->params + c->wh_off, c->params + c->bh_off,
+                                           c->A, c->lse, *o.step, CUR(c));
+                  *o.step_fused = true;
+              } else launch_rollout_tail_bf16(prev, k3.P2, n, bk, bb, CUR(c)); }
+            if (fused_step) return true;
             prev = k3.P2;
             break;
         }
@@ -750,7 +762,7 @@
     float* const feat = c->feat + (size_t)o.soff * c->H;
     if (c->cfg.arch != MI_ARCH_IMPALA) forward_mlp(c, src, n, o.soff, feat);
     else if (!c->bf) forward_impala_fp32(c, src, n, o.soff, feat);
-    else if (!forward_impala_bf16(c, src, n, o.soff, feat, o.train)) return;
+    else if (!forward_impala_bf16(c, src, n, feat, o)) return;
     if (o.recurrent && c->gru_on) net_gru(c, n, o.soff);
     if (o.heads) net_heads(c, n, o.soff);
 }
@@ -970,6 +982,11 @@
     return false;
 }
 
+static void heads_sample_step(mi_ctx* c, const float* hin, int n, const StepHead& s, hipStream_t st) {
+    launch_heads_sample(hin, c->params + c->wh_off, c->params + c->bh_off, n, c->H, c->A, s.u, s.seed, s.ctr, s.act, s.logp, s.value, s.pack, s.hout,
+                        s.rd, s.rew_dst, s.done_dst, st, s.done_ctr, s.host_flag, s.ticket, c->lse);
+}
+
 int mi_policy_step(mi_ctx* c, int32_t t, uint64_t seed, const float* u, int64_t* act_out, float* logp_out, float* value_out) {
     ARG(c, "null"); JOIN(c); ARG(t >= 0 && t <= c->T, "t out of range");
     const int E = c->E;
@@ -1001,12 +1018,13 @@
     const float* du;
     if (int r = upload_u(c, u, c->stream, 0, E, &du)) return r;
     c->prof.phase = 0;
-    net_forward(c, src, E, {.recurrent = true, .heads = false});
     const bool last = (t == c->T);
-    launch_heads_sample(c->feat, c->params + c->wh_off, c->params + c->bh_off, E, c->H, c->A, du, seed, (unsigned long long)t * E,
-                        last ? nullptr : c->act + (size_t)t * E, last ? nullptr : c->logp + (size_t)t * E, c->value + (size_t)t * E,
-                        c->h_pack, nullptr, have_rd ? c->h_rd : nullptr, have_rd ? c->rew + (size_t)(t - 1) * E : nullptr,
-                        have_rd ? c->done + (size_t)(t - 1) * E : nullptr, c->stream, c->d_done_ctr, c->h_flag, ++c->roll_ticket, c->lse);
+    const StepHead sh{du, seed, (unsigned long long)t * E, last ? nullptr : c->act + (size_t)t * E, last ? nullptr : c->logp + (size_t)t * E,
+                      c->value + (size_t)t * E, c->h_pack, nullptr, have_rd ? c->h_rd : nullptr, have_rd ? c->rew + (size_t)(t - 1) * E : nullptr,
+                      have_rd ? c->done + (size_t)(t - 1) * E : nullptr, c->d_done_ctr, c->h_flag, ++c->roll_ticket};
+    bool fused = false;
+    net_forward(c, src, E, {.recurrent = true, .heads = false, .step = &sh, .step_fused = &fused});
+    if (!fused) heads_sample_step(c, c->feat, E, sh, c->stream);
     HIPC(hipGetLastError()); NETCHK(c);
     if (!wait_ticket(c->h_flag, c->roll_ticket, [&] { return hipStreamQuery(c->stream) != hipErrorNotReady; })) HIPC(hipStreamSynchronize(c->stream));
     unpack_step(c->h_pack, E, last, act_out, logp_out, value_out);
@@ -1052,7 +1070,12 @@
     const float* du;
     if (int r = upload_u(c, j.u, st, e0, ng, &du)) return r;
     InputSrc src{obs_ring(c), nullptr, (long long)j.t * E + e0};
-    net_forward(c, src, ng, {.heads = false, .soff = e0});
+    const size_t o = (size_t)j.t * E + e0;
+    const StepHead sh{du, j.seed, (unsigned long long)j.t * E + e0, j.last ? nullptr : c->act + o, j.last ? nullptr : c->logp + o, c->value + o,
+                      c->h_pack + 3 * e0, nullptr, j.have_rd ? h_rd : nullptr, j.have_rd ? c->rew + o - E : nullptr, j.have_rd ? c->done + o - E : nullptr,
+                      c->d_done_ctr + 1 + g, c->h_flag + 1 + g, j.ticket};
+    bool fused = false;
+    net_forward(c, src, ng, {.heads = false, .soff = e0, .step = &sh, .step_fused = &fused});
     const float* hin = c->feat + (size_t)e0 * c->H;
     if (c->gru_on) {
         const size_t H = c->H;
@@ -1061,11 +1084,7 @@
                         j.last ? nullptr : slot + (size_t)E * H, ng, c->H, st);
         hin = c->h_state + (size_t)e0 * H;
     }
-    const size_t o = (size_t)j.t * E + e0;
-    launch_heads_sample(hin, c->params + c->wh_off, c->params + c->bh_off, ng, c->H, c->A, du, j.seed, (unsigned long long)j.t * E + e0,
-                        j.last ? nullptr : c->act + o, j.last ? nullptr : c->logp + o, c->value + o, c->h_pack + 3 * e0, nullptr,
-                        j.have_rd ? h_rd : nullptr, j.have_rd ? c->rew + o - E : nullptr, j.have_rd ? c->done + o - E : nullptr, st,
-                        c->d_done_ctr + 1 + g, c->h_flag + 1 + g, j.ticket, c->lse);
+    if (!fused) heads_sample_step(c, hin, ng, sh, st);
     HIPC(hipGetLastError());
     if (const char* lf = mi_launch_failed_take()) return fail(-4, lf);
     return 0;
@@ -1832,4 +1851,4 @@
     }
 }
 
-int mi_debug_flags(mi_ctx* c, int32_t flags) { ARG(c, "null"); JOIN(c); c->rollout_tail = !(flags & 1); c->no_pull = (flags & 4) != 0; c->side_on = !(flags & 16); return 0; }
+int mi_debug_flags(mi_ctx* c, int32_t flags) { ARG(c, "null"); JOIN(c); c->rollout_tail = !(flags & 1); c->step_split = (flags & 2) != 0; c->no_pull = (flags & 4) != 0; c->side_on = !(flags & 16); return 0; }
diff --git a/train-procgen-pytorch_amd/csrc/engine_ctx.h b/train-procgen-pytorch_amd/csrc/engine_ctx.h
--- a/train-procgen-pytorch_amd/csrc/engine_ctx.h
+++ b/train-procgen-pytorch_amd/csrc/engine_ctx.h
@@ -106,7 +106,7 @@
     float* d_u = nullptr; float* d_lp = nullptr;
     unsigned short* banks = nullptr; BankDesc* d_bank_desc = nullptr; int n_banks = 0;
     unsigned short* c1_bank = nullptr;
-    unsigned short *fc_wp = nullptr, *fc_wt = nullptr;
+    unsigned short *fc_wp = nullptr, *fc_wt = nullptr, *fc_wf = nullptr;
     bool fc_packed_valid = false;
     float *d_pack = nullptr, *h_pack = nullptr, *h_rd = nullptr, *d_rd = nullptr;
     unsigned *d_done_ctr = nullptr, *h_flag = nullptr, roll_ticket = 0;
@@ -128,6 +128,7 @@
     bool side_on = true;
     struct SideJob { bool armed; LossArgs a; SegTab st; int mode; float* ring; float* fsr; float* log; } side = {};
     bool rollout_tail = true;
+    bool step_split = false;
     float *fs_colmax = nullptr, fs_grad_coef = 0.f; int *fs_arg = nullptr, fs_G = 0;
     long long *fs_keys = nullptr, *fs_keys_local = nullptr; int32_t *d_gpos = nullptr, *h_gpos = nullptr; int gpos_n = -1; bool fs_global_pending = false, fs_global_apply = false;
     ncclComm_t comm = nullptr, comm_grad = nullptr; int comm_world = 1, comm_rank = 0; hipStream_t comm_stream = nullptr; hipEvent_t ev_ar_ready = nullptr, ev_ar_done = nullptr;
@@ -152,7 +153,7 @@
 MI_INTERNAL void to_ref_layout(const TensorDesc& t, const float* dev, float* ref);
 MI_INTERNAL std::vector<uint16_t> host_to_bf16(const float* x, size_t n);
 struct InputSrc { const void* base; const int32_t* idx; long long first; };
-struct FwdOpts { bool recurrent = false; bool heads = true; bool train = false; int soff = 0; };
+struct FwdOpts { bool recurrent = false; bool heads = true; bool train = false; int soff = 0; const StepHead* step = nullptr; bool* step_fused = nullptr; };
 MI_INTERNAL void net_forward(mi_ctx* c, const InputSrc& src, int n, const FwdOpts& o);
 MI_INTERNAL void linear_fwd(mi_ctx* c, const float* X, int relu_x, const float* W, const float* b, float* Y, int n, int in, int out, int relu_out, int x_bf16 = 0);
 MI_INTERNAL void linear_dgrad(mi_ctx* c, const float* dY, const float* W, const float* mask, float* dX, int n, int in, int out, int x_bf16 = 0);
diff --git a/train-procgen-pytorch_amd/csrc/heads.hip b/train-procgen-pytorch_amd/csrc/heads.hip
--- a/train-procgen-pytorch_amd/csrc/heads.hip
+++ b/train-procgen-pytorch_amd/csrc/heads.hip
@@ -230,13 +230,7 @@
         const float* f = s_f + el * 260;
         float acc = 0.f;
         int k = 0;
-        if (H == 256) {
-#pragma unroll 8
-            for (; k < 256; k += 4) {
-                const f32x4 fv = *(const f32x4*)(f + k), ww = *(const f32x4*)(w + k);
-                acc += fv.x * ww.x + fv.y * ww.y + fv.z * ww.z + fv.w * ww.w;
-            }
-        }
+        if (H == 256) { acc = head_dot256(f, w); k = 256; }
         for (; k + 4 <= H; k += 4) {
             const f32x4 fv = *(const f32x4*)(f + k), ww = *(const f32x4*)(w + k);
             acc += fv.x * ww.x + fv.y * ww.y + fv.z * ww.z + fv.w * ww.w;
@@ -247,65 +241,10 @@
     }
     __syncthreads();
     __shared__ __attribute__((aligned(16))) float s_t[16 * 16];
-    const bool lane_on = o < A;
-    auto row = [&](float term, float (&v)[16]) {
-        __builtin_amdgcn_wave_barrier();
-        s_t[el * 16 + o] = term;
-        __builtin_amdgcn_wave_barrier();
-        const f32x4 a0 = *(const f32x4*)(s_t + el * 16), a1 = *(const f32x4*)(s_t + el * 16 + 4);
-        const f32x4 a2 = *(const f32x4*)(s_t + el * 16 + 8), a3 = *(const f32x4*)(s_t + el * 16 + 12);
-        v[0] = a0.x; v[1] = a0.y; v[2] = a0.z; v[3] = a0.w; v[4] = a1.x; v[5] = a1.y; v[6] = a1.z; v[7] = a1.w;
-        v[8] = a2.x; v[9] = a2.y; v[10] = a2.z; v[11] = a2.w; v[12] = a3.x; v[13] = a3.y; v[14] = a3.z; v[15] = a3.w;
-    };
-    auto group_sum = [&](float term) {
-        float v[16];
-        row(term, v);
-        float t = 0.f;
-#pragma unroll
-        for (int k = 0; k < 16; ++k) if (k < A) t += v[k];
-        return t;
-    };
-    const float z = lane_on ? s_z[el * 17 + o] : 0.f;
-    float mx;
-    {
-        float v[16];
-        row(z, v);
-        mx = v[0];
-#pragma unroll
-        for (int k = 1; k < 16; ++k) if (k < A) mx = fmaxf(mx, v[k]);
-    }
-    const float s1 = group_sum(lane_on ? expf(z - mx) : 0.f);
-    const float lse1 = mx + logf(s1);
-    float lp = z - lse1;
-    const float s2 = group_sum(lane_on ? expf(lp) : 0.f);
-    lp -= logf(s2);
-    const float pr = lane_on ? expf(lp) : 0.f;
-    float cdf = 0.f;
-    {
-        float v[16];
-        row(pr, v);
-#pragma unroll
-        for (int k = 0; k < 16; ++k) if (k < A) cdf += (k <= o) ? v[k] : 0.f;
-    }
     const float uu = (e < n) ? (u ? u[e] : philox_uniform(seed, ctr + e)) : 0.f;
-    const float mark = (lane_on && cdf <= uu) ? (float)(o + 1) : 0.f;
-    float sel = 0.f;
-    {
-        float v[16];
-        row(mark, v);
-#pragma unroll
-        for (int k = 0; k < 16; ++k) if (k < A) sel = fmaxf(sel, v[k]);
-    }
-    int a_sel = (int)sel;
-    if (a_sel > A - 1) a_sel = A - 1;
-    float lp_pick;
-    {
-        float v[16];
-        row(lp, v);
-        lp_pick = v[0];
-#pragma unroll
-        for (int k = 1; k < 16; ++k) lp_pick = (k == a_sel) ? v[k] : lp_pick;
-    }
+    const HeadPick hp = head_sample16(s_t + el * 16, o, A, o < A ? s_z[el * 17 + o] : 0.f, uu);
+    const int a_sel = hp.act;
+    const float lp_pick = hp.logp, lse1 = hp.lse;
     if (o == 0 && e < n) {
         const float lp_sel = lp_pick, val = LSE ? lse1 : s_z[el * 17 + A];
         if (rd) { rew_dst[e] = rwd; done_dst[e] = dn; }
diff --git a/train-procgen-pytorch_amd/csrc/policy_math.h b/train-procgen-pytorch_amd/csrc/policy_math.h
--- a/train-procgen-pytorch_amd/csrc/policy_math.h
+++ b/train-procgen-pytorch_amd/csrc/policy_math.h
@@ -25,6 +25,79 @@
     for (int a = 0; a < MAXA; ++a) if (a < A) p[a] /= s3;
 }
 
+typedef float pm_f32x4 __attribute__((ext_vector_type(4)));
+__device__ __forceinline__ float head_dot256(const float* f, const float* w) {
+    float acc = 0.f;
+#pragma unroll 8
+    for (int k = 0; k < 256; k += 4) {
+        const pm_f32x4 fv = *(const pm_f32x4*)(f + k), ww = *(const pm_f32x4*)(w + k);
+        acc += __builtin_fmaf(fv.w, ww.w, __builtin_fmaf(fv.z, ww.z, __builtin_fmaf(fv.x, ww.x, fv.y * ww.y)));
+    }
+    return acc;
+}
+struct HeadPick { int act; float logp, lse; };
+__device__ __forceinline__ HeadPick head_sample16(float* t16, int o, int A, float z, float uu) {
+    const bool lane_on = o < A;
+    auto row = [&](float term, float (&v)[16]) {
+        __builtin_amdgcn_wave_barrier();
+        t16[o] = term;
+        __builtin_amdgcn_wave_barrier();
+        const pm_f32x4 a0 = *(const pm_f32x4*)(t16), a1 = *(const pm_f32x4*)(t16 + 4);
+        const pm_f32x4 a2 = *(const pm_f32x4*)(t16 + 8), a3 = *(const pm_f32x4*)(t16 + 12);
+        v[0] = a0.x; v[1] = a0.y; v[2] = a0.z; v[3] = a0.w; v[4] = a1.x; v[5] = a1.y; v[6] = a1.z; v[7] = a1.w;
+        v[8] = a2.x; v[9] = a2.y; v[10] = a2.z; v[11] = a2.w; v[12] = a3.x; v[13] = a3.y; v[14] = a3.z; v[15] = a3.w;
+    };
+    auto group_sum = [&](float term) {
+        float v[16];
+        row(term, v);
+        float t = 0.f;
+#pragma unroll
+        for (int k = 0; k < 16; ++k) if (k < A) t += v[k];
+        return t;
+    };
+    if (!lane_on) z = 0.f;
+    float mx;
+    {
+        float v[16];
+        row(z, v);
+        mx = v[0];
+#pragma unroll
+        for (int k = 1; k < 16; ++k) if (k < A) mx = fmaxf(mx, v[k]);
+    }
+    const float s1 = group_sum(lane_on ? expf(z - mx) : 0.f);
+    const float lse1 = mx + logf(s1);
+    float lp = z - lse1;
+    const float s2 = group_sum(lane_on ? expf(lp) : 0.f);
+    lp -= logf(s2);
+    const float pr = lane_on ? expf(lp) : 0.f;
+    float cdf = 0.f;
+    {
+        float v[16];
+        row(pr, v);
+#pragma unroll
+        for (int k = 0; k < 16; ++k) if (k < A) cdf += (k <= o) ? v[k] : 0.f;
+    }
+    const float mark = (lane_on && cdf <= uu) ? (float)(o + 1) : 0.f;
+    float sel = 0.f;
+    {
+        float v[16];
+        row(mark, v);
+#pragma unroll
+        for (int k = 0; k < 16; ++k) if (k < A) sel = fmaxf(sel, v[k]);
+    }
+    int a_sel = (int)sel;
+    if (a_sel > A - 1) a_sel = A - 1;
+    float lp_pick;
+    {
+        float v[16];
+        row(lp, v);
+        lp_pick = v[0];
+#pragma unroll
+        for (int k = 1; k < 16; ++k) lp_pick = (k == a_sel) ? v[k] : lp_pick;
+    }
+    return HeadPick{a_sel, lp_pick, lse1};
+}
+
 __device__ __forceinline__ void philox_round(uint32_t* c, uint32_t* k) {
     const uint32_t M0 = 0xD2511F53u, M1 = 0xCD9E8D57u;
     const uint32_t hi0 = __umulhi(M0, c[0]), lo0 = M0 * c[0];
diff --git a/train-procgen-pytorch_amd/csrc/rollout_bf16.hip b/train-procgen-pytorch_amd/csrc/rollout_bf16.hip
--- a/train-procgen-pytorch_amd/csrc/rollout_bf16.hip
+++ b/train-procgen-pytorch_amd/csrc/rollout_bf16.hip
@@ -1,5 +1,6 @@
 #include "common.h"
 #include "device_util.h"
+#include "policy_math.h"
 #include <mutex>
 
 __device__ __forceinline__ unsigned rt_relu2(unsigned w) { const unsigned neg = (w >> 15) & 0x00010001u; return w & ~(neg * 0xFFFFu); }
@@ -23,6 +24,8 @@
 static_assert(KB2_ELEMS <= X16_ELEMS && KB3_ELEMS <= IN_ELEMS && 2 * X8_ELEMS <= X16_ELEMS, "region reuse");
 static_assert(LDS_ELEMS * 2 <= 160 * 1024, "LDS");
 constexpr int KW = (W_ELEMS / 8 + NT - 1) / NT;
+constexpr int FC_X = R_IN, FC_FEAT = FC_X + 2048, FC_WH = FC_FEAT + 2 * 256, FC_Z = FC_WH + 2 * 16 * 260, FC_T = FC_Z + 2 * 32, FC_END = FC_T + 2 * 16;
+static_assert(FC_END <= IN_ELEMS && FC_FEAT % 8 == 0 && FC_WH % 8 == 0 && FC_T % 8 == 0, "fc / head phase region");
 }
 
 struct RolloutTailArgs {
@@ -32,6 +35,11 @@
     const unsigned short* bank[10];
     const float* bias[10];
 };
+struct RolloutStepArgs {
+    const unsigned short* fc_wf; const float* fc_b; float* feat;
+    const float *Wh, *bh; int A, lse;
+    StepHead s;
+};
 
 struct KoffTab { int v[5]; __device__ __forceinline__ int operator()(int m) const { return v[m]; } };
 template <int P> struct KoffC { __device__ __forceinline__ constexpr int operator()(int m) const { return ((m / 3) * P + (m % 3)) * 48; } };
@@ -74,7 +82,8 @@
     return acc;
 }
 
-__global__ __launch_bounds__(rt::NT) void rollout_tail_bf16_kernel(RolloutTailArgs a) {
+template <bool STEP>
+__device__ __forceinline__ void rt_body(const RolloutTailArgs& a, const RolloutStepArgs& h) {
     using namespace rt;
     extern __shared__ __attribute__((aligned(16))) unsigned short smem_h[];
     unsigned short* s_in = smem_h + R_IN;
@@ -255,6 +264,28 @@
             __syncthreads();
         }
 
+        unsigned short* s_fx = s_in;
+        rt_u32x4 wf[2][16];
+        const unsigned short* fcw = STEP ? h.fc_wf + ((long long)wave * 2 * 64 * 64 + lane) * 8 : nullptr;
+        auto fc_fetch = [&](int u, rt_u32x4 (&r)[16]) {
+            const unsigned short* p = fcw + ((u >> 2) * 64 + (u & 3) * 16) * 64 * 8;
+#pragma unroll
+            for (int s = 0; s < 16; ++s) r[s] = *(const rt_u32x4*)(p + s * 64 * 8);
+        };
+        f32x4 whr[2];
+        float rwd = 0.f, dn = 0.f, uu = 0.f;
+        if constexpr (STEP) {
+            fc_fetch(0, wf[0]);
+#pragma unroll
+            for (int j = 0; j < 2; ++j) {
+                const int k = tid + j * NT, r = k >> 6, kk = (k & 63) * 4;
+                whr[j] = r <= h.A ? *(const f32x4*)(h.Wh + (long long)r * 256 + kk) : (f32x4){0.f, 0.f, 0.f, 0.f};
+            }
+            if (tid == 0) {
+                if (h.s.rd) { rwd = h.s.rd[img]; dn = h.s.rd[a.n + img]; }
+                if (h.s.u) uu = h.s.u[img];
+            }
+        }
         {
             const bool on = wave < 8;
             const int tile = (wave & 7) >> 1, nb = wave & 1;
@@ -285,14 +316,85 @@
                     for (int r = 0; r < 4; ++r) v[r] = acc[r] + bq[r] + mi_bf16x4_lane(sk, r);
                     const uint2 raw = mi_pk_bf16x4(v);
                     if (k2 < 9) *(uint2*)(s_x8 + cen) = raw;
-                    else *(uint2*)(a.y + ((long long)img * 64 + pl) * 32 + nb * 16 + kq * 4) = raw;
+                    else {
+                        *(uint2*)(a.y + ((long long)img * 64 + pl) * 32 + nb * 16 + kq * 4) = raw;
+                        if constexpr (STEP) *(uint2*)(s_fx + pl * 32 + nb * 16 + kq * 4) = (uint2){rt_relu2(raw.x), rt_relu2(raw.y)};
+                    }
                 }
                 if (k2 < 9) bank_step(k2);
                 __syncthreads();
             }
         }
+        if constexpr (STEP) {
+            float* s_feat = (float*)(smem_h + FC_FEAT);
+            float* s_wh = (float*)(smem_h + FC_WH);
+            float* s_z = (float*)(smem_h + FC_Z);
+            float* s_t = (float*)(smem_h + FC_T);
+#pragma unroll
+            for (int j = 0; j < 2; ++j) { const int k = tid + j * NT, r = k >> 6, kk = (k & 63) * 4; if (r <= h.A) *(f32x4*)(s_wh + r * 260 + kk) = whr[j]; }
+            f32x4 part[2][4];
+#pragma unroll
+            for (int u = 0; u < 8; ++u) {
+                if (u + 1 < 8) fc_fetch(u + 1, wf[(u + 1) & 1]);
+                __builtin_amdgcn_sched_barrier(0);
+                f32x4 acc = {0.f, 0.f, 0.f, 0.f};
+#pragma unroll
+                for (int s = 0; s < 16; ++s) {
+                    const rt_u32x4 xa = *(const rt_u32x4*)(s_fx + (u & 3) * 512 + s * 32 + kq * 8);
+                    acc = MFMA_BF16(__builtin_bit_cast(bf16x8, xa), __builtin_bit_cast(bf16x8, wf[u & 1][s]), acc);
+                }
+                part[u >> 2][u & 3] = acc;
+                __builtin_amdgcn_sched_barrier(0);
+            }
+            if (lane < 16) {
+#pragma unroll
+                for (int ct = 0; ct < 2; ++ct) {
+                    const int col = wave * 32 + ct * 16 + i;
+                    const float v = ((part[ct][0][0] + part[ct][1][0]) + (part[ct][2][0] + part[ct][3][0])) + h.fc_b[col];
+                    const float f = v > 0.f ? v : 0.f;
+                    h.feat[(long long)img * 256 + col] = f;
+                    s_feat[col] = f;
+                }
+            }
+            __syncthreads();
+            if (tid < 16) {
+                const int o = tid, A = h.A;
+                float z = 0.f;
+                if (o <= A) { z = head_dot256(s_feat, s_wh + o * 260) + h.bh[o]; s_z[o] = z; }
+                if (!h.s.u) uu = philox_uniform(h.s.seed, h.s.ctr + img);
+                uu = __shfl(uu, 0, 64);
+                const HeadPick hp = head_sample16(s_t, o, A, z, uu);
+                if (o == 0) {
+                    const float val = h.lse ? hp.lse : s_z[A];
+                    if (h.s.rd) { h.s.rew_dst[img] = rwd; h.s.done_dst[img] = dn; }
+                    if (h.s.act) h.s.act[img] = hp.act;
+                    if (h.s.logp) h.s.logp[img] = hp.logp;
+                    if (h.s.value) h.s.value[img] = val;
+                    if (h.s.pack) { h.s.pack[img * 3] = (float)hp.act; h.s.pack[img * 3 + 1] = hp.logp; h.s.pack[img * 3 + 2] = val; }
+                    if (h.s.hout) for (int k = 0; k <= A; ++k) h.s.hout[(long long)img * (A + 1) + k] = s_z[k];
+                }
+            }
+            break;
+        }
     }
-}
+    if constexpr (STEP) {
+        if (h.s.host_flag) {
+            __builtin_amdgcn_fence(__ATOMIC_RELEASE, "workgroup");
+            __syncthreads();
+            if (threadIdx.x < 64) __threadfence_system();
+            if (threadIdx.x == 0) {
+                const unsigned old = atomicAdd(h.s.done_ctr, 1u);
+                if (old == gridDim.x - 1) {
+                    *h.s.done_ctr = 0;
+                    __threadfence_system();
+                    __hip_atomic_store(h.s.host_flag, h.s.ticket, __ATOMIC_RELEASE, __HIP_MEMORY_SCOPE_SYSTEM);
+                }
+            }
+        }
+    }
+}
+__global__ __launch_bounds__(rt::NT) void rollout_tail_bf16_kernel(RolloutTailArgs a) { rt_body<false>(a, RolloutStepArgs{}); }
+__global__ __launch_bounds__(rt::NT) void rollout_step_bf16_kernel(RolloutTailArgs a, RolloutStepArgs h) { rt_body<true>(a, h); }
 
 void launch_rollout_tail_bf16(const void* x, void* y, int n, const unsigned short* const* bank, const float* const* bias, hipStream_t st) {
     if (n <= 0) return;
@@ -303,3 +405,16 @@
     for (int k = 0; k < 10; ++k) { a.bank[k] = bank[k]; a.bias[k] = bias[k]; }
     hipLaunchKernelGGL(rollout_tail_bf16_kernel, dim3(n < 256 ? n : 256), dim3(rt::NT), rt::LDS_ELEMS * 2, st, a);
 }
+void launch_rollout_step_bf16(const void* x, void* y, int n, const unsigned short* const* bank, const float* const* bias,
+                              const unsigned short* fc_wf, const float* fc_b, float* feat, const float* Wh, const float* bh, int A,
+                              int value_from_logits, const StepHead& s, hipStream_t st) {
+    if (n <= 0) return;
+    if (n > 256 || A + 1 > 16) { mi_launch_fail("rollout_step_bf16: n <= 256 and A + 1 <= 16 only"); return; }
+    static std::once_flag attr;
+    std::call_once(attr, [] { hipFuncSetAttribute((const void*)rollout_step_bf16_kernel, hipFuncAttributeMaxDynamicSharedMemorySize, rt::LDS_ELEMS * 2); });
+    RolloutTailArgs a{};
+    a.x = (const unsigned short*)x; a.y = (unsigned short*)y; a.n = n;
+    for (int k = 0; k < 10; ++k) { a.bank[k] = bank[k]; a.bias[k] = bias[k]; }
+    RolloutStepArgs h{fc_wf, fc_b, feat, Wh, bh, A, value_from_logits, s};
+    hipLaunchKernelGGL(rollout_step_bf16_kernel, dim3(n), dim3(rt::NT), rt::LDS_ELEMS * 2, st, a, h);
+}
```
